# wangkenpu/rsrgan

Hardware: AMD Instinct MI355X
Metric: GAN train frames/sec (G+D step), 257-dim LPS->40-dim MFCC (higher is better)
Workload: dtype f32

## Files before the change

include/rsrgan.h:

```cpp
#ifndef RSRGAN_H_
#define RSRGAN_H_

#include <stddef.h>
#include <stdint.h>

#ifdef __cplusplus
extern "C" {
#endif

typedef enum rsrgan_status {
  RSRGAN_OK = 0,
  RSRGAN_ERR_INVALID = -1,
  RSRGAN_ERR_HIP = -2,
  RSRGAN_ERR_NO_DEVICE = -3,
  RSRGAN_ERR_STATE = -4
} rsrgan_status;

enum { RSRGAN_G_LSTM = 0, RSRGAN_G_RES_LSTM_L = 1, RSRGAN_G_RES_LSTM_BASE = 2,
       RSRGAN_G_DNN = 3,
       RSRGAN_G_RCED = 4,
       RSRGAN_G_BNLSTM = 5 ,
       RSRGAN_G_RES_LSTM_I = 6  };
enum { RSRGAN_D_LSTM = 0, RSRGAN_D_DNN = 1  };
enum { RSRGAN_NET_G = 0, RSRGAN_NET_D = 1 };
// ... 50 lines not shown
};

typedef struct rsrgan_handle_s* rsrgan_handle;

int rsrgan_default_cfg(int32_t g_type, rsrgan_cfg* cfg);

int rsrgan_create(const rsrgan_cfg* cfg, uint64_t seed, rsrgan_handle* out);
int rsrgan_destroy(rsrgan_handle h);
const char* rsrgan_last_error(void);

int rsrgan_set_scalar(rsrgan_handle h, int32_t which, double v);
int rsrgan_get_scalar(rsrgan_handle h, int32_t which, double* v);

int rsrgan_num_tensors(rsrgan_handle h, int32_t net);
int rsrgan_tensor_info(rsrgan_handle h, int32_t net, int32_t idx,
                       char* name, int32_t name_cap,
                       int32_t* rows, int32_t* cols, int64_t* dense_offset);
int64_t rsrgan_param_count(rsrgan_handle h, int32_t net);

int rsrgan_get_params(rsrgan_handle h, int32_t net, int32_t what, float* dense, void* stream);
int rsrgan_set_params(rsrgan_handle h, int32_t net, int32_t what, const float* dense, void* stream);
int rsrgan_get_grads(rsrgan_handle h, int32_t net, float* dense, void* stream);

int rsrgan_forward_g(rsrgan_handle h, const float* x, const int32_t* lengths, int32_t T,
                     float* y, void* stream);

int rsrgan_g_state_floats(rsrgan_handle h, int32_t* n);
int rsrgan_g_state_reset(rsrgan_handle h, const int32_t* row_mask, void* stream);
int rsrgan_g_state_get(rsrgan_handle h, float* dst, void* stream);
int rsrgan_g_state_set(rsrgan_handle h, const float* src, void* stream);
int rsrgan_forward_g_stream(rsrgan_handle h, const float* x, const int32_t* lengths, int32_t T,
                            float* y, void* stream);

int rsrgan_d_step(rsrgan_handle h, const float* x, const float* labels, const int32_t* lengths,
                  int32_t T, const float* noise_real, const float* noise_fake,
                  float* out_losses, int32_t train, void* stream);

int rsrgan_g_step(rsrgan_handle h, const float* x, const float* labels, const int32_t* lengths,
                  int32_t T, const float* noise_fake, float* out_losses,
                  int32_t train, int32_t reuse_g_forward, void* stream);

int rsrgan_d_backward(rsrgan_handle h, const float* x, const float* labels, const int32_t* lengths,
                      int32_t T, const float* noise_real, const float* noise_fake,
                      float* out_losses, void* stream);
int rsrgan_g_backward(rsrgan_handle h, const float* x, const float* labels, const int32_t* lengths,
                      int32_t T, const float* noise_fake, float* out_losses,
                      int32_t reuse_g_forward, void* stream);
int rsrgan_apply(rsrgan_handle h, int32_t net, void* stream);
int rsrgan_grad_buffer(rsrgan_handle h, int32_t net, float** ptr, int64_t* count);
int rsrgan_grad_bucket_count(rsrgan_handle h, int32_t net);
int rsrgan_grad_bucket_info(rsrgan_handle h, int32_t net, int32_t i, int64_t* offset, int64_t* count);
int rsrgan_grad_bucket_wait(rsrgan_handle h, int32_t net, int32_t i, void* stream);

int rsrgan_profile_begin(rsrgan_handle h);
int rsrgan_profile_read(rsrgan_handle h, int32_t* launches, double* total_us, double* alg_flops);
int rsrgan_profile_read_kind(rsrgan_handle h, int32_t kind, int32_t* launches, double* total_us, double* alg_flops);

int rsrgan_device_status(rsrgan_handle h, int32_t* code);

int rsrgan_device_bytes(rsrgan_handle h, int64_t* bytes);

int rsrgan_set_dropout(rsrgan_handle h, float keep_prob, uint64_t seed);

int rsrgan_profile_launches(rsrgan_handle h, int64_t* n);
int rsrgan_op_launch_floor(int32_t n, int32_t mode, double* us_per_launch, void* stream);

int rsrgan_op_gemm(const float* A, int32_t lda, int32_t a_kcontig,
                   const float* B, int32_t ldb, int32_t b_kcontig,
                   float* C, int32_t ldc, int32_t M, int32_t N, int32_t K,
                   const float* bias, int32_t act, float alpha, int32_t accumulate, void* stream);

int rsrgan_op_gemm2(const float* A, int32_t lda, int32_t a_kcontig, const float* A2, int32_t lda2, int32_t M1,
                    const float* B, int32_t ldb, int32_t b_kcontig, float* C, int32_t ldc, int32_t M, int32_t N, int32_t K,
                    const float* bias, int32_t act, float alpha, int32_t accumulate,
                    int32_t map_rows_per, int64_t map_outer, int64_t map_inner, int32_t workers, int32_t force_cfg, void* stream);
#define RSRGAN_OP_NOT_APPLICABLE 1
int rsrgan_op_gemm_batch(int32_t nb, const float* const* A, int32_t lda, const float* const* A2, int32_t lda2, int32_t M1,
                         const float* const* B, int32_t ldb, float* const* C, int32_t ldc, int32_t M, int32_t N, int32_t K,
                         int32_t accumulate, int32_t workers, void* stream);
int rsrgan_op_gemm16_batch(int32_t n, const float* const* A, int32_t lda, const float* const* A2, int32_t lda2, int32_t M1,
                           const float* const* B, int32_t ldb, float* const* C, int32_t ldc, int32_t M, int32_t N, int32_t K,
                           int32_t accumulate, void* stream);
int rsrgan_op_gemm_last_plan(int32_t out[8]);
int rsrgan_op_lstm_colsums(int32_t nb, const float* const* dz, const float* const* cprev, const float* const* ccur, float* const* db,
                           float* const* dwi, float* const* dwf, float* const* dwo, int32_t rows, int32_t H, void* stream);
int rsrgan_op_colsum(const float* a, int32_t lda, const float* b, int32_t ldb, float* out, int32_t rows, int32_t cols, int32_t tall,
                     void* stream);
int rsrgan_op_bnl_fold(const float* Wx, const float* Wh, const float* const bn[12], const float* bias, int32_t P, int32_t H, float* KxT,
                       int32_t ldI, float* KhT, int32_t ldP, float* bias_f, float* ca, float* cb, void* stream);

int rsrgan_op_conv_fwd(const float* in, int32_t ldc_in, int32_t C, const float* F, int32_t ldf, int32_t flip, const float* bias, int32_t relu,
                       const float* mask, float* out, int32_t ldc_out, int32_t N, int32_t R, int32_t S, int32_t W, int32_t fw, void* stream);
int rsrgan_op_conv_wgrad(const float* in, int32_t ldc_in, int32_t C, const float* d, int32_t ldc_d, int32_t N, float* dW, int32_t ldw, float* db,
                         float* ws, int64_t ws_floats, int32_t R_max, int32_t R, int32_t S, int32_t W, int32_t fw, void* stream);
int64_t rsrgan_op_conv_ws_floats(int32_t C, int32_t R_max, int32_t S, int32_t W, int32_t fw);
int rsrgan_op_conv_supported(int32_t C, int32_t N, int32_t S, int32_t W, int32_t fw);
int rsrgan_op_conv_last_plan(int32_t out[40]);

int rsrgan_op_bn_forward(const float* z, int32_t ldz, float* y, int32_t ldy, int32_t rows, int32_t cols, int32_t calls,
                         float* const* vars, float* stat, int32_t ldc, int32_t training, int32_t relu, float* scratch,
                         int64_t scratch_floats, void* stream);
int rsrgan_op_bn_backward(float* dy, int32_t ldd, const float* y, int32_t ldy, const float* z, int32_t ldz, int32_t rows, int32_t cols,
                          int32_t calls, const float* stat, int32_t ldc, float* dbeta, float* dgamma, int32_t accumulate, int32_t relu,
                          float* sums, float* scratch, int64_t scratch_floats, void* stream);
int rsrgan_op_bn_seq_forward(const float* z, int32_t ldz, float* y, int32_t ldy, int32_t rows, int32_t cols, float* const* vars,
                             float* stat, int32_t ldc, int32_t training, int32_t relu, float alpha, int32_t Bp, int32_t Bt,
                             float* scratch, int64_t scratch_floats, void* stream);
int rsrgan_op_bn_seq_backward(float* dy, int32_t ldd, const float* y, int32_t ldy, const float* z, int32_t ldz, int32_t rows,
                              int32_t cols, const float* stat, int32_t ldc, float* dbeta, float* dgamma, int32_t accumulate,
                              int32_t relu, float alpha, int32_t Bp, int32_t Bt, float* sums, float* scratch, int64_t scratch_floats,
                              void* stream);
int rsrgan_op_bn_commit(int32_t n, float* const* vars, const float* const* stat, const int32_t* dims, int32_t single, void* stream);
int rsrgan_op_bn_last_plan(int32_t out[16]);

int rsrgan_feat_batch(const float* raw, int64_t raw_rows, const int32_t* offsets, int32_t B, int32_t T, int32_t D, int32_t left,
                      int32_t right, const double* mean, const double* stddev, float* out, int32_t* lengths, void* stream);
int rsrgan_feat_frames(const float* pool, int64_t pool_rows, const int32_t* picks, int32_t N, int32_t D, int32_t left, int32_t right,
                       const double* mean, const double* stddev, float* out, void* stream);
int rsrgan_feat_stream(const float* fresh, int64_t fresh_rows, const int32_t* table, float* hist, int32_t B, int32_t H, int32_t T, int32_t D,
                       int32_t left, int32_t right, const double* mean, const double* stddev, float* out, int32_t* lengths, void* stream);
int rsrgan_feat_denorm(const float* y, const int32_t* lengths, int32_t B, int32_t T, int32_t D, const double* mean, const double* stddev,
                       double* out, void* stream);
int rsrgan_feat_decode(const uint8_t* blob, int64_t blob_bytes, const int64_t* seg, const float* scale, const int32_t* offsets, int32_t B,
                       int32_t D, const double* mean, const double* stddev, float* out, int64_t out_rows, void* stream);
int rsrgan_feat_wave(const void* pcm, int32_t kind, int64_t n_samples, const int64_t* seg, const int32_t* offsets, int32_t B, int32_t N,
                     int32_t S, int32_t P, float preemph, const float* window, const float* twiddle, float* out, int64_t out_rows,
                     void* stream);
int rsrgan_feat_mfcc(const void* pcm, int32_t kind, int64_t n_samples, const int64_t* seg, const int32_t* offsets, int32_t B, int32_t N,
                     int32_t S, int32_t P, float preemph, const float* window, const float* twiddle, const int32_t* mel_seg,
                     const float* mel_w, int32_t nnz, int32_t M, const float* dct, int32_t C, float* out, int64_t out_rows, void* stream);
int rsrgan_feat_wave_frames(int32_t P);
int rsrgan_wave_reverb(const void* pcm, int32_t kind, int64_t n_samples, const int64_t* seg, const float* rir, int64_t n_taps,
                       const int64_t* rir_seg, const float* noise, int64_t n_noise, const int64_t* noise_seg, const float* noise_pow,
                       const int32_t* sel, const float* snr, int32_t B, int32_t R, int32_t V, int32_t C, const float* twiddle, int32_t flags,
                       float* out, int64_t out_samples, const int64_t* out_seg, float* gains, void* work, int64_t work_bytes, void* stream);
int64_t rsrgan_wave_reverb_work(int32_t B, int64_t n_max, int64_t L_max, int32_t C);

int rsrgan_hist(int32_t n, const float* const* x, const int64_t* dims, double* out, void* stream);
int rsrgan_hist_limits(double* out, int32_t* n);
int rsrgan_d_logits(rsrgan_handle h, float* real, float* fake, int32_t* T, void* stream);
int rsrgan_d_logits_hist(rsrgan_handle h, double* out, void* stream);

int rsrgan_op_segan_sizes(int32_t kind, const int64_t* dims, int64_t out[12]);
int rsrgan_op_segan_conv2(int32_t op, const void* const* ptrs, const int64_t* dims, const float* fl, void* stream);
int rsrgan_op_segan_conv1(int32_t op, const void* const* ptrs, const int64_t* dims, const float* fl, void* stream);
int rsrgan_op_segan_colred(int32_t mode, const void* const* ptrs, const int64_t* dims, const float* fl, void* stream);
int rsrgan_op_segan_last_plan(int32_t out[8]);
int rsrgan_op_segan_vbn(int32_t op, const void* const* ptrs, const int64_t* dims, const float* fl, void* stream);
int rsrgan_op_segan_elem(int32_t op, const void* const* ptrs, const int64_t* dims, const float* fl, void* stream);
int rsrgan_op_segan_dhead(int32_t op, const void* const* ptrs, const int64_t* dims, const float* fl, void* stream);

int rsrgan_op_chunks(const int64_t* tensors, int32_t n_tensors, int32_t* out, int64_t out_ints, int32_t* n_chunks);
int rsrgan_op_update(int32_t op, const void* const* ptrs, const int64_t* dims, const float* fl, void* stream);
int rsrgan_op_step_elem(int32_t op, const void* const* ptrs, const int64_t* dims, const float* fl, void* stream);
int rsrgan_op_layout(int32_t op, const void* const* ptrs, const int64_t* dims, const float* fl, void* stream);

typedef struct rsrgan_segan_cfg {
  int32_t batch_size;
  int32_t input_len;
  int32_t output_dim;
  int32_t n_layers;
  int32_t g_depths[16];
  int32_t d_depths[16];
  int32_t g_kwidth;
  int32_t d_kwidth;
  int32_t g_prelu;
  float   lrelu_alpha;
  float   vbn_eps;
  float   rms_decay;
  float   rms_eps;
} rsrgan_segan_cfg;
typedef struct rsrgan_segan_handle_s* rsrgan_segan_handle;
enum { RSRGAN_SEGAN_G_LR = 0, RSRGAN_SEGAN_D_LR = 1, RSRGAN_SEGAN_L1_LAMBDA = 2 };
int rsrgan_segan_default_cfg(rsrgan_segan_cfg* cfg);
int rsrgan_segan_create(const rsrgan_segan_cfg* cfg, uint64_t seed, rsrgan_segan_handle* out);
int rsrgan_segan_destroy(rsrgan_segan_handle h);
int rsrgan_segan_set_scalar(rsrgan_segan_handle h, int32_t which, double v);
int rsrgan_segan_num_tensors(rsrgan_segan_handle h, int32_t net);
int rsrgan_segan_tensor_info(rsrgan_segan_handle h, int32_t net, int32_t idx, char* name, int32_t name_cap, int32_t* rows, int32_t* cols,
                             int64_t* dense_offset);
int64_t rsrgan_segan_param_count(rsrgan_segan_handle h, int32_t net);
int rsrgan_segan_get_params(rsrgan_segan_handle h, int32_t net, int32_t what, float* dense, void* stream);
int rsrgan_segan_set_params(rsrgan_segan_handle h, int32_t net, int32_t what, const float* dense, void* stream);
int rsrgan_segan_forward_g(rsrgan_segan_handle h, const float* x, const float* z, float* y, void* stream);
int rsrgan_segan_d_backward(rsrgan_segan_handle h, const float* x, const float* labels, const float* z, const float* noise_ref,
                            const float* noise_real, const float* noise_fake, float* out_losses, int32_t train, void* stream);
int rsrgan_segan_g_backward(rsrgan_segan_handle h, const float* x, const float* labels, const float* z, const float* noise_ref,
                            const float* noise_fake, float* out_losses, int32_t train, void* stream);
int rsrgan_segan_grad_buffer(rsrgan_segan_handle h, int32_t net, float** ptr, int64_t* count);
int rsrgan_segan_apply(rsrgan_segan_handle h, int32_t net, void* stream);

int rsrgan_version(void);

#ifdef __cplusplus
}
#endif
#endif
```

rsrgan_amd/_lib.py:

```python
from __future__ import annotations

import ctypes as C
import os

_HERE = os.path.dirname(os.path.abspath(__file__))
LIB_PATH = os.path.join(_HERE, "lib", "librsrgan_hip.so")

G_TYPES = {"lstm": 0, "res_lstm_l": 1, "res_lstm_base": 2, "dnn": 3, "rced": 4, "bnlstm": 5, "res_lstm_i": 6}
FLAG_BATCH_NORM = 32
FLAG_INFER = 64
D_TYPES = {"lstm": 0, "dnn": 1}
NET_G, NET_D = 0, 1
SCALARS = {"g_learning_rate": 0, "d_learning_rate": 1, "mse_lambda": 2, "d_real": 3, "d_fake": 4,
           "l2_scale": 5, "clip_norm": 6, "adam_step": 7, "adam_step_d": 8}
WHAT = {"variables": 0, "adam_m": 1, "adam_v": 2, "ema": 3}

SYMBOLS = ["rsrgan_default_cfg", "rsrgan_create", "rsrgan_destroy", "rsrgan_last_error", "rsrgan_set_scalar",
           "rsrgan_get_scalar", "rsrgan_num_tensors", "rsrgan_tensor_info", "rsrgan_param_count",
           "rsrgan_get_params", "rsrgan_set_params", "rsrgan_get_grads", "rsrgan_forward_g",
           "rsrgan_g_state_floats", "rsrgan_g_state_reset", "rsrgan_g_state_get", "rsrgan_g_state_set", "rsrgan_forward_g_stream",
           "rsrgan_d_step",
           "rsrgan_g_step", "rsrgan_d_backward", "rsrgan_g_backward", "rsrgan_apply", "rsrgan_grad_buffer",
           "rsrgan_grad_bucket_count", "rsrgan_grad_bucket_info", "rsrgan_grad_bucket_wait",
           "rsrgan_profile_begin", "rsrgan_profile_read", "rsrgan_profile_read_kind", "rsrgan_profile_launches", "rsrgan_op_launch_floor", "rsrgan_device_status", "rsrgan_device_bytes", "rsrgan_set_dropout",
           "rsrgan_op_gemm", "rsrgan_op_gemm2", "rsrgan_op_gemm_batch", "rsrgan_op_gemm16_batch", "rsrgan_op_gemm_last_plan",
           "rsrgan_op_lstm_colsums", "rsrgan_op_colsum", "rsrgan_op_bnl_fold", "rsrgan_version",
           "rsrgan_op_conv_fwd", "rsrgan_op_conv_wgrad", "rsrgan_op_conv_ws_floats", "rsrgan_op_conv_supported", "rsrgan_op_conv_last_plan",
           "rsrgan_op_bn_forward", "rsrgan_op_bn_backward", "rsrgan_op_bn_commit", "rsrgan_op_bn_last_plan",
           "rsrgan_op_bn_seq_forward", "rsrgan_op_bn_seq_backward", "rsrgan_feat_batch", "rsrgan_feat_frames",
           "rsrgan_feat_stream", "rsrgan_feat_denorm", "rsrgan_feat_decode", "rsrgan_feat_wave", "rsrgan_feat_mfcc", "rsrgan_feat_wave_frames",
           "rsrgan_wave_reverb", "rsrgan_wave_reverb_work",
           "rsrgan_hist", "rsrgan_hist_limits", "rsrgan_d_logits", "rsrgan_d_logits_hist",
           "rsrgan_op_segan_sizes", "rsrgan_op_segan_conv2", "rsrgan_op_segan_conv1", "rsrgan_op_segan_colred", "rsrgan_op_segan_last_plan",
           "rsrgan_op_segan_vbn", "rsrgan_op_segan_elem", "rsrgan_op_segan_dhead",
           "rsrgan_op_chunks", "rsrgan_op_update", "rsrgan_op_step_elem", "rsrgan_op_layout",
           "rsrgan_segan_default_cfg", "rsrgan_segan_create", "rsrgan_segan_destroy", "rsrgan_segan_set_scalar",
           "rsrgan_segan_num_tensors", "rsrgan_segan_tensor_info", "rsrgan_segan_param_count", "rsrgan_segan_get_params",
           "rsrgan_segan_set_params", "rsrgan_segan_forward_g", "rsrgan_segan_d_backward", "rsrgan_segan_g_backward",
           "rsrgan_segan_grad_buffer", "rsrgan_segan_apply"]


class RsrganCfg(C.Structure):
    _fields_ = [("batch_size", C.c_int32), ("max_frames", C.c_int32), ("input_dim", C.c_int32),
                ("output_dim", C.c_int32), ("g_type", C.c_int32), ("g_layers", C.c_int32), ("g_cells", C.c_int32),
                ("g_proj", C.c_int32), ("d_type", C.c_int32), ("d_layers", C.c_int32), ("d_cells", C.c_int32),
                ("d_proj", C.c_int32), ("l2_scale", C.c_float), ("clip_norm", C.c_float), ("adam_beta1", C.c_float),
                ("adam_beta2", C.c_float), ("adam_eps", C.c_float), ("ema_decay", C.c_float),
                ("lrelu_alpha", C.c_float), ("forget_bias", C.c_float), ("cross_validation", C.c_int32),
                ("flags", C.c_int32), ("d_joint_off", C.c_int32), ("d_joint_dim", C.c_int32), ("g_splice", C.c_int32)]


class SeganCfg(C.Structure):
    _fields_ = [("batch_size", C.c_int32), ("input_len", C.c_int32), ("output_dim", C.c_int32), ("n_layers", C.c_int32),
                ("g_depths", C.c_int32 * 16), ("d_depths", C.c_int32 * 16), ("g_kwidth", C.c_int32), ("d_kwidth", C.c_int32),
                ("g_prelu", C.c_int32), ("lrelu_alpha", C.c_float), ("vbn_eps", C.c_float), ("rms_decay", C.c_float),
                ("rms_eps", C.c_float)]


class RsrganError(RuntimeError):
    pass


_lib = None


def load():
    global _lib
    if _lib is not None:
        return _lib
    if not os.path.exists(LIB_PATH):
        raise ImportError("%s is missing: build it with `python -c 'import __graft_entry__ as g; g.build()'` "
                          "(hipcc --offload-arch=gfx950); rsrgan_amd has no CPU fallback" % LIB_PATH)
    lib = C.CDLL(LIB_PATH)
    p, i32, i64, f32, vp = C.c_void_p, C.c_int32, C.c_int64, C.c_float, C.c_void_p
    lib.rsrgan_last_error.restype = C.c_char_p
    lib.rsrgan_default_cfg.argtypes = [i32, C.POINTER(RsrganCfg)]
    lib.rsrgan_create.argtypes = [C.POINTER(RsrganCfg), C.c_uint64, C.POINTER(vp)]
    lib.rsrgan_destroy.argtypes = [vp]
    lib.rsrgan_set_scalar.argtypes = [vp, i32, C.c_double]
    lib.rsrgan_get_scalar.argtypes = [vp, i32, C.POINTER(C.c_double)]
    lib.rsrgan_num_tensors.argtypes = [vp, i32]
    lib.rsrgan_tensor_info.argtypes = [vp, i32, i32, C.c_char_p, i32, C.POINTER(i32), C.POINTER(i32), C.POINTER(i64)]
    lib.rsrgan_param_count.argtypes = [vp, i32]
    lib.rsrgan_param_count.restype = i64
    lib.rsrgan_get_params.argtypes = [vp, i32, i32, p, vp]
    lib.rsrgan_set_params.argtypes = [vp, i32, i32, p, vp]
    lib.rsrgan_get_grads.argtypes = [vp, i32, p, vp]
    lib.rsrgan_forward_g.argtypes = [vp, p, p, i32, p, vp]
    lib.rsrgan_g_state_floats.argtypes = [vp, C.POINTER(i32)]
    lib.rsrgan_g_state_reset.argtypes = [vp, p, vp]
    lib.rsrgan_g_state_get.argtypes = [vp, p, vp]
    lib.rsrgan_g_state_set.argtypes = [vp, p, vp]
    lib.rsrgan_forward_g_stream.argtypes = [vp, p, p, i32, p, vp]
    lib.rsrgan_d_step.argtypes = [vp, p, p, p, i32, p, p, p, i32, vp]
    lib.rsrgan_g_step.argtypes = [vp, p, p, p, i32, p, p, i32, i32, vp]
    lib.rsrgan_d_backward.argtypes = [vp, p, p, p, i32, p, p, p, vp]
    lib.rsrgan_g_backward.argtypes = [vp, p, p, p, i32, p, p, i32, vp]
    lib.rsrgan_apply.argtypes = [vp, i32, vp]
    lib.rsrgan_grad_buffer.argtypes = [vp, i32, C.POINTER(p), C.POINTER(i64)]
    lib.rsrgan_grad_bucket_count.argtypes = [vp, i32]
    lib.rsrgan_grad_bucket_info.argtypes = [vp, i32, i32, C.POINTER(i64), C.POINTER(i64)]
    lib.rsrgan_grad_bucket_wait.argtypes = [vp, i32, i32, vp]
    lib.rsrgan_profile_begin.argtypes = [vp]
    lib.rsrgan_profile_read.argtypes = [vp, C.POINTER(i32), C.POINTER(C.c_double), C.POINTER(C.c_double)]
    lib.rsrgan_profile_read_kind.argtypes = [vp, i32, C.POINTER(i32), C.POINTER(C.c_double), C.POINTER(C.c_double)]
    lib.rsrgan_device_status.argtypes = [vp, C.POINTER(i32)]
    lib.rsrgan_device_bytes.argtypes = [vp, C.POINTER(i64)]
    lib.rsrgan_set_dropout.argtypes = [vp, f32, C.c_uint64]
    lib.rsrgan_profile_launches.argtypes = [vp, C.POINTER(i64)]
    lib.rsrgan_op_launch_floor.argtypes = [i32, i32, C.POINTER(C.c_double), vp]
    lib.rsrgan_op_gemm.argtypes = [p, i32, i32, p, i32, i32, p, i32, i32, i32, i32, p, i32, f32, i32, vp]
    pp = C.POINTER(C.c_void_p)
    lib.rsrgan_op_gemm2.argtypes = [p, i32, i32, p, i32, i32, p, i32, i32, p, i32, i32, i32, i32, p, i32, f32, i32, i32, i64, i64, i32, i32, vp]
    lib.rsrgan_op_gemm_batch.argtypes = [i32, pp, i32, pp, i32, i32, pp, i32, pp, i32, i32, i32, i32, i32, i32, vp]
    lib.rsrgan_op_gemm16_batch.argtypes = [i32, pp, i32, pp, i32, i32, pp, i32, pp, i32, i32, i32, i32, i32, vp]
    lib.rsrgan_op_gemm_last_plan.argtypes = [C.POINTER(i32)]
    lib.rsrgan_op_lstm_colsums.argtypes = [i32, pp, pp, pp, pp, pp, pp, pp, i32, i32, vp]
    lib.rsrgan_op_colsum.argtypes = [p, i32, p, i32, p, i32, i32, i32, vp]
    lib.rsrgan_op_bnl_fold.argtypes = [p, p, pp, p, i32, i32, p, i32, p, i32, p, p, p, vp]
    lib.rsrgan_op_conv_fwd.argtypes = [p, i32, i32, p, i32, i32, p, i32, p, p, i32, i32, i32, i32, i32, i32, vp]
    lib.rsrgan_op_conv_wgrad.argtypes = [p, i32, i32, p, i32, i32, p, i32, p, p, i64, i32, i32, i32, i32, i32, vp]
    lib.rsrgan_op_conv_ws_floats.argtypes = [i32, i32, i32, i32, i32]
    lib.rsrgan_op_conv_ws_floats.restype = i64
    lib.rsrgan_op_conv_supported.argtypes = [i32, i32, i32, i32, i32]
    lib.rsrgan_op_conv_last_plan.argtypes = [C.POINTER(i32)]
    lib.rsrgan_op_bn_forward.argtypes = [p, i32, p, i32, i32, i32, i32, pp, p, i32, i32, i32, p, i64, vp]
    lib.rsrgan_op_bn_backward.argtypes = [p, i32, p, i32, p, i32, i32, i32, i32, p, i32, p, p, i32, i32, p, p, i64, vp]
    lib.rsrgan_op_bn_seq_forward.argtypes = [p, i32, p, i32, i32, i32, pp, p, i32, i32, i32, f32, i32, i32, p, i64, vp]
    lib.rsrgan_op_bn_seq_backward.argtypes = [p, i32, p, i32, p, i32, i32, i32, p, i32, p, p, i32, i32, f32, i32, i32, p, p, i64, vp]
    lib.rsrgan_feat_batch.argtypes = [p, i64, p, i32, i32, i32, i32, i32, p, p, p, p, vp]
    lib.rsrgan_feat_frames.argtypes = [p, i64, p, i32, i32, i32, i32, p, p, p, vp]
    lib.rsrgan_feat_stream.argtypes = [p, i64, p, p, i32, i32, i32, i32, i32, i32, p, p, p, p, vp]
    lib.rsrgan_feat_denorm.argtypes = [p, p, i32, i32, i32, p, p, p, vp]
    lib.rsrgan_feat_decode.argtypes = [p, i64, p, p, p, i32, i32, p, p, p, i64, vp]
    lib.rsrgan_feat_wave.argtypes = [p, i32, i64, p, p, i32, i32, i32, i32, f32, p, p, p, i64, vp]
    lib.rsrgan_feat_mfcc.argtypes = [p, i32, i64, p, p, i32, i32, i32, i32, f32, p, p, p, p, i32, i32, p, i32, p, i64, vp]
    lib.rsrgan_feat_wave_frames.argtypes = [i32]
    lib.rsrgan_wave_reverb.argtypes = [p, i32, i64, p, p, i64, p, p, i64, p, p, p, p, i32, i32, i32, i32, p, i32, p, i64, p, p, p, i64, vp]
    lib.rsrgan_wave_reverb_work.argtypes = [i32, i64, i64, i32]
    lib.rsrgan_wave_reverb_work.restype = i64
    lib.rsrgan_hist.argtypes = [i32, pp, C.POINTER(i64), p, vp]
    lib.rsrgan_hist_limits.argtypes = [C.POINTER(C.c_double), C.POINTER(i32)]
    lib.rsrgan_d_logits.argtypes = [vp, p, p, C.POINTER(i32), vp]
    lib.rsrgan_d_logits_hist.argtypes = [vp, p, vp]
    lib.rsrgan_op_bn_commit.argtypes =[i32, pp, pp, C.POINTER(i32), i32, vp]
    lib.rsrgan_op_bn_last_plan.argtypes = [C.POINTER(i32)]
    lib.rsrgan_op_segan_sizes.argtypes = [i32, C.POINTER(i64), C.POINTER(i64)]
    for f in (lib.rsrgan_op_segan_conv2, lib.rsrgan_op_segan_conv1, lib.rsrgan_op_segan_colred, lib.rsrgan_op_segan_vbn, lib.rsrgan_op_segan_elem,
              lib.rsrgan_op_segan_dhead, lib.rsrgan_op_update, lib.rsrgan_op_step_elem, lib.rsrgan_op_layout):
        f.argtypes = [i32, C.POINTER(vp), C.POINTER(i64), C.POINTER(C.c_float), vp]
    lib.rsrgan_op_segan_last_plan.argtypes = [C.POINTER(i32)]
    lib.rsrgan_op_chunks.argtypes = [C.POINTER(i64), i32, C.POINTER(i32), i64, C.POINTER(i32)]
    lib.rsrgan_segan_default_cfg.argtypes = [C.POINTER(SeganCfg)]
    lib.rsrgan_segan_create.argtypes = [C.POINTER(SeganCfg), C.c_uint64, C.POINTER(vp)]
    lib.rsrgan_segan_destroy.argtypes = [vp]
    lib.rsrgan_segan_set_scalar.argtypes = [vp, i32, C.c_double]
    lib.rsrgan_segan_num_tensors.argtypes = [vp, i32]
    lib.rsrgan_segan_tensor_info.argtypes = [vp, i32, i32, C.c_char_p, i32, C.POINTER(i32), C.POINTER(i32), C.POINTER(i64)]
    lib.rsrgan_segan_param_count.argtypes = [vp, i32]
    lib.rsrgan_segan_param_count.restype = i64
    lib.rsrgan_segan_get_params.argtypes = [vp, i32, i32, p, vp]
    lib.rsrgan_segan_set_params.argtypes = [vp, i32, i32, p, vp]
    lib.rsrgan_segan_forward_g.argtypes = [vp, p, p, p, vp]
    lib.rsrgan_segan_d_backward.argtypes = [vp, p, p, p, p, p, p, p, i32, vp]
    lib.rsrgan_segan_g_backward.argtypes = [vp, p, p, p, p, p, p, i32, vp]
    lib.rsrgan_segan_grad_buffer.argtypes = [vp, i32, C.POINTER(p), C.POINTER(i64)]
    lib.rsrgan_segan_apply.argtypes = [vp, i32, vp]
    _lib = lib
    return lib


OP_NOT_APPLICABLE = 1
GEMM_CLASSES = {0: "none", 1: "gemm16", 2: "n32", 3: "k_gemm", 4: "k_gemm_s", 5: "gemm16_batch", 6: "k_gemm_batch", 7: "k_gemm_s_batch"}
GEMM_PLAN_FIELDS = ("cls", "bm", "bn", "W", "n_dp", "fixup", "splits", "Ur")
GEMM_FORMS = [("k_gemm", 128, 128), ("k_gemm", 96, 128), ("k_gemm", 128, 96), ("k_gemm", 256, 64), ("k_gemm", 256, 32),
              ("k_gemm_s", 256, 256), ("k_gemm_s", 128, 256), ("k_gemm_s", 256, 128)]
CONV_FAMILIES = {0: "none", 1: "fwd", 2: "fwd4", 3: "wgrad", 4: "wgrad4"}
CONV_FWD_BRANCHES = {1: "whole", 2: "main", 3: "rem"}
CONV_WGRAD_BRANCHES = {1: "k2", 2: "rows", 3: "search"}
CONV_PLAN_FIELDS = ("family", "a0", "a1", "a2", "branch", "TW", "FB", "gx", "gy", "gz", "lds", "DH", "fpg", "groups", "nstrips", "nkg",
                    "PS", "waves", "gmax")
BN_ROUTES = {0: "none", 1: "small", 2: "sliced", 3: "narrow"}
BN_PLAN_FIELDS = ("route", "backward", "calls", "launches", "slices", "per", "pgx", "pgy", "egrid", "q", "R")
SEGAN_OPS = {"conv2": ("conv2_fwd", "conv2_wgrad", "tconv2"), "conv1": ("conv1_fwd", "conv1_wgrad", "tconv1"),
             "colred": ("sum", "dalpha", "moments", "vbn_bwd"), "vbn": ("coef", "apply", "bwd_coef", "bwd_apply"),
             "elem": ("pad_rows", "prep_tconv", "prep_tconv_many", "interleave", "act_fwd", "act_bwd", "copy_cols", "build_joint1", "sum_all",
                      "lsgan", "l1", "rmsprop"),
             "dhead": ("fwd", "bwd")}
UPDATE_OPS = ("sumsq", "dw_reduce", "l2", "apply_sgd", "apply_adam")
STEP_ELEM_OPS = ("lsgan", "dhead", "mse", "g_total", "l2_total", "adam_tick", "dropout_fwd", "dropout_bwd", "lrelu_bwd")
LAYOUT_OPS = ("pack_tm", "unpack_bm", "stage_inputs", "build_d_input", "add_noise_rows", "transpose", "transpose_many", "swizzle_many", "im2col",
              "col2im", "expand_c4", "gstate", "window_len", "zero_many", "fill", "build_joint", "slice_cols", "pad_copy", "copy_f")
DYN_SLOTS = {"g_lr": 0, "d_lr": 1, "lambda": 2, "d_real": 3, "d_fake": 4, "l2": 5, "clip": 6, "beta1": 7, "beta2": 8, "eps": 9, "ema": 10,
             "adam_lrt": 11, "adam_lrt_d": 12}
DYN_COUNT = 16
SEGAN_PLAN_FIELDS = ("vec", "mode", "chunk", "chunks_per", "grid")
BN_VARS = ("beta", "gamma", "moving_mean", "moving_variance", "renorm_mean", "renorm_mean_weight", "renorm_stddev", "renorm_stddev_weight")


def ptr_table(ptrs):
    return (C.c_void_p * max(len(ptrs), 1))(*[None if q is None else q for q in ptrs])


_hist_limits = None


def hist_limits():
    global _hist_limits
    if _hist_limits is None:
        import numpy as np
        lib = load()
        n = C.c_int32()
        check(lib.rsrgan_hist_limits(None, C.byref(n)))
        buf = (C.c_double * n.value)()
        check(lib.rsrgan_hist_limits(buf, C.byref(n)))
        _hist_limits = np.frombuffer(buf, np.float64).copy()
        _hist_limits.setflags(write=False)
    return _hist_limits


def check(rc):
    if rc != 0:
        raise RsrganError("librsrgan_hip error %d: %s" % (rc, load().rsrgan_last_error().decode()))
```

rsrgan_amd/csrc/capi_ops.cpp:

```cpp
#include "capi_common.h"

extern "C" {

int rsrgan_op_launch_floor(int32_t n, int32_t mode, double* us_per_launch, void* stream) {
  if (n <= 0 || !us_per_launch) { set_error("op_launch_floor: bad argument"); return RSRGAN_ERR_INVALID; }
  static float* buf = nullptr;
  if (!buf && hipMalloc((void**)&buf, 2 * 65536 * 4 * sizeof(float)) != hipSuccess) { set_error("hipMalloc failed"); return RSRGAN_ERR_HIP; }
  hipStream_t s = nullptr;
  hipGraph_t g = nullptr; hipGraphExec_t ge = nullptr;
  hipEvent_t e0 = nullptr, e1 = nullptr;
  int rc = RSRGAN_ERR_HIP;
  do {
    if (hipStreamCreateWithFlags(&s, hipStreamNonBlocking) != hipSuccess) break;
    if (hipMemsetAsync(buf, 0, 2 * 65536 * 4 * sizeof(float), s) != hipSuccess) break;
    if (hipStreamBeginCapture(s, hipStreamCaptureModeThreadLocal) != hipSuccess) break;
    launch_floor_chain(buf, buf + 65536 * 4, n, mode, s);
    if (hipStreamEndCapture(s, &g) != hipSuccess) break;
    if (hipGraphInstantiate(&ge, g, nullptr, nullptr, 0) != hipSuccess) break;
    if (hipEventCreate(&e0) != hipSuccess || hipEventCreate(&e1) != hipSuccess) break;
    if (hipGraphLaunch(ge, s) != hipSuccess) break;
    if (hipEventRecord(e0, s) != hipSuccess || hipGraphLaunch(ge, s) != hipSuccess || hipEventRecord(e1, s) != hipSuccess) break;
    if (hipEventSynchronize(e1) != hipSuccess) break;
    float ms = 0.f;
    if (hipEventElapsedTime(&ms, e0, e1) != hipSuccess) break;
// ... 568 lines not shown
      }
      if (op == 1) launch_prep_tconv(FP(0), (int)d[1], (int)d[2], (int)d[3], (int)d[4], (int)d[5], FP(1), (int)d[6], s);
      else {
        PrepTconvBatch pb(s);
        for (int j = 0; j < n; ++j) { const int64_t* q = d + 1 + 6 * j; pb.add(FP(2 * j), (int)q[0], (int)q[1], (int)q[2], (int)q[3], (int)q[4], FP(2 * j + 1), (int)q[5]); }
        pb.flush();
      }
      break;
    }
    case 3: {
      OP_DIM("Q0", d[0], 1); OP_DIM("Q1", d[1], 1); OP_DIM("pl", d[4], 0); OP_DIM("B", d[5], 1); OP_DIM("Lt", d[6], 1); OP_DIM("C", d[7], 1); OP_MUL4("C", d[7]);
      for (int e = 0; e < 2; ++e) {
        const int64_t i0 = (((e - d[4]) % 2) + 2) % 2, cnt = d[6] > i0 ? (d[6] - i0 + 1) / 2 : 0;
        OP_REFUSE(d[2 + e] != i0, WHO ": i0%d = %lld is not the first position of parity class %d under pl = %lld", e, (long long)d[2 + e], e, (long long)d[4]);
        OP_REFUSE(d[e] < cnt, WHO ": Q%d = %lld below the %lld positions of its class", e, (long long)d[e], (long long)cnt);
      }
      OP_REFUSE(d[5] * d[6] * d[7] > ((int64_t)1 << 30), WHO ": B x Lt x C above the entry's 2^30");
      OP_PTR("T0", ptrs[0], 16); OP_PTR("T1", ptrs[1], 16); OP_OPT("bias", ptrs[2], 16); OP_PTR("T", ptrs[3], 16);
      launch_interleave(FP(0), FP(1), (int)d[0], (int)d[1], (int)d[2], (int)d[3], (int)d[4], FP(2), FP(3), (int)d[5], (int)d[6], (int)d[7], s);
      break;
    }
    case 4: {
      OP_DIM("C", d[0], 1); OP_DIM("coff", d[2], 0); OP_DIM("rows", d[3], 1); OP_LD("ldo", d[1], d[2] + d[0]);
      OP_REFUSE(d[3] * d[1] > ((int64_t)1 << 30), WHO ": rows x ldo above the entry's 2^30");
      OP_PTR("z", ptrs[0], 4); OP_OPT("alpha", ptrs[1], 4); OP_PTR("out", ptrs[2], 4);
      launch_act_fwd(FP(0), (int)d[0], FP(1), fl[0], FP(2), (int)d[1], (int)d[2], (size_t)d[3], s);
      break;
    }
    case 5: {
      OP_DIM("C", d[2], 1); OP_DIM("coff", d[1], 0); OP_DIM("rows", d[3], 1); OP_LD("ldy", d[0], d[1] + d[2]);
      OP_REFUSE(d[3] * d[0] > ((int64_t)1 << 30), WHO ": rows x ldy above the entry's 2^30");
      OP_PTR("dy", ptrs[0], 4); OP_PTR("z", ptrs[1], 4); OP_OPT("alpha", ptrs[2], 4); OP_OPT("extra", ptrs[3], 4); OP_PTR("dz", ptrs[4], 4);
      launch_act_bwd(FP(0), (int)d[0], (int)d[1], FP(1), (int)d[2], FP(2), fl[0], FP(3), FP(4), (size_t)d[3], s);
      break;
    }
    case 6: {
      OP_DIM("C", d[4], 1); OP_DIM("rows", d[5], 1); OP_DIM("soff", d[1], 0); OP_DIM("doff", d[3], 0); OP_FLAG("accumulate", d[6]);
      OP_LD("lds", d[0], d[1] + d[4]); OP_LD("ldd", d[2], d[3] + d[4]);
      OP_REFUSE(d[5] * std::max(d[0], d[2]) > ((int64_t)1 << 30), WHO ": rows x ld above the entry's 2^30");
      OP_PTR("src", ptrs[0], 4); OP_PTR("dst", ptrs[1], 4);
      launch_copy_cols(FP(0), (int)d[0], (int)d[1], FP(1), (int)d[2], (int)d[3], (int)d[4], (size_t)d[5], d[6] != 0, s);
      break;
    }
    case 7: {
      OP_DIM("Lx", d[0], 1); OP_DIM("U", d[1], 1); OP_DIM("B", d[2], 1);
      OP_REFUSE(d[2] * (d[0] + d[1]) > ((int64_t)1 << 30), WHO ": B x (Lx + U) above the entry's 2^30");
      OP_PTR("x", ptrs[0], 4); OP_PTR("tail", ptrs[1], 4); OP_OPT("noise", ptrs[2], 4); OP_PTR("joint", ptrs[3], 4);
      launch_build_joint1(FP(0), (int)d[0], FP(1), (int)d[1], FP(2), FP(3), (int)d[2], s);
      break;
    }
    case 8: {
      OP_DIM("rows", d[0], 1); OP_DIM("cols", d[1], 1); OP_LD("ld", d[2], d[1]);
      OP_REFUSE(d[0] * d[2] > ((int64_t)1 << 30), WHO ": rows x ld above the entry's 2^30");
      OP_PTR("src", ptrs[0], 4); OP_PTR("out", ptrs[1], 4); OP_PTR("scratch", ptrs[2], 4);
      launch_sum_all(FP(0), (int)d[0], (int)d[1], (int)d[2], FP(1), FP(2), s);
      break;
    }
    case 9: {
      OP_DIM("B", d[0], 1); OP_DIM("P", d[3], 1);
      OP_REFUSE(d[1] < 0 || d[1] > 1, WHO ": mode = %lld outside 0 (D-run) .. 1 (G-run)", (long long)d[1]);
      OP_REFUSE(d[2] < 0 || d[2] >= d[3], WHO ": fake_pass = %lld outside [0, P = %lld)", (long long)d[2], (long long)d[3]);
      OP_REFUSE(d[0] * d[3] > (1 << 24), WHO ": P x B above the entry's 2^24");
      OP_PTR("logits", ptrs[0], 4); OP_OPT("dlogits", ptrs[1], 4); OP_PTR("loss3", ptrs[2], 4);
      launch_segan_lsgan(FP(0), (int)d[0], (int)d[1], (int)d[2], (int)d[3], FP(1), FP(2), s);
      break;
    }
    case 10: {
      OP_DIM("n", d[0], 1); OP_FLAG("accumulate", d[1]);
      OP_PTR("G", ptrs[0], 4); OP_PTR("labels", ptrs[1], 4); OP_PTR("lambda", ptrs[2], 4); OP_OPT("dG", ptrs[3], 4); OP_PTR("loss3", ptrs[4], 4);
      launch_segan_l1(FP(0), FP(1), (int)d[0], FP(2), FP(3), d[1] != 0, FP(4), s);
      break;
    }
    default: {
      OP_DIM("n", d[0], 1);
      OP_PTR("w", ptrs[0], 4); OP_PTR("g", ptrs[1], 4); OP_PTR("ms", ptrs[2], 4); OP_PTR("lr", ptrs[3], 4);
      launch_rmsprop(FP(0), FP(1), FP(2), FP(3), fl[0], fl[1], (size_t)d[0], s);
      break;
    }
  }
  OP_LAUNCHED(WHO);
}
#undef WHO

#define WHO "op_segan_dhead"
int rsrgan_op_segan_dhead(int32_t op, const void* const* ptrs, const int64_t* dims, const float* fl, void* stream) {
  (void)fl;
  OP_TABLES(0);
  OP_REFUSE(op < 0 || op > 1, WHO ": op = %d outside 0 (dhead_fwd), 1 (dhead_bwd)", op);
  const int64_t* d = dims;
  OP_DIM("R", d[0], 1); OP_DIM("Ld", d[1], 1); OP_DIM("C", d[2], 1); OP_DIM("k", d[3], 1); OP_DIM("ldfc", d[4], 1);
  OP_REFUSE(d[0] * d[1] * d[2] > ((int64_t)1 << 28) || d[3] * d[2] > (1 << 24), WHO ": R x Ld x C above the entry's 2^28");
  if (op == 0) {
    const char* names[6] = {"h", "W", "wfc", "bfc", "conv_out", "logits"};
    for (int i = 0; i < 6; ++i) OP_PTR(names[i], ptrs[i], 4);
    launch_dhead_fwd(FP(0), (int)d[0], (int)d[1], (int)d[2], (int)d[3], FP(1), FP(2), (int)d[4], FP(3), FP(4), FP(5), (hipStream_t)stream);
  } else {
    const char* names[9] = {"dlogit", "h", "conv_out", "W", "wfc", "dW", "dwfc", "dbfc", "dh"};
    for (int i = 0; i < 9; ++i) { if (i >= 5 && i <= 7) OP_OPT(names[i], ptrs[i], 4); else OP_PTR(names[i], ptrs[i], 4); }
    OP_REFUSE((!ptrs[5]) != (!ptrs[6]) || (!ptrs[5]) != (!ptrs[7]), WHO ": dW, dwfc and dbfc must all be given or all be null");
    launch_dhead_bwd(FP(0), (int)d[0], (int)d[1], (int)d[2], (int)d[3], FP(1), FP(2), FP(3), FP(4), (int)d[4], FP(5), FP(6), FP(7), FP(8), (hipStream_t)stream);
  }
  OP_LAUNCHED(WHO);
}
#undef WHO

#define OP_BP(rows_name, rows, Bp, Bt) do { \
    OP_REFUSE((Bp) < 0 || (Bp) > (1 << 20), WHO ": Bp = %lld outside 0 .. 2^20", (long long)(Bp)); \
    if ((Bp) > 0) { \
      OP_REFUSE((Bt) < 1 || (Bt) > (Bp), WHO ": Bt = %lld outside 1 .. Bp = %lld", (long long)(Bt), (long long)(Bp)); \
      OP_REFUSE((rows) % (Bp), WHO ": %s = %lld is not divisible by Bp = %lld", rows_name, (long long)(rows), (long long)(Bp)); \
    } } while (0)
static const int64_t g_up_max_tensors = 4096;

static int up_tensors_ok(const char* who, const int64_t* tensors, int64_t n, int64_t buf_floats) {
  OP_REFUSE(!tensors, "%s: null pointer (tensors)", who);
  OP_REFUSE(n < 1 || n > g_up_max_tensors, "%s: n_tensors = %lld outside 1 .. %lld", who, (long long)n, (long long)g_up_max_tensors);
  for (int64_t i = 0; i < n; ++i) {
    const int64_t off = tensors[3 * i], fl = tensors[3 * i + 1], l2 = tensors[3 * i + 2];
    OP_REFUSE(off < 0 || (off & 3), "%s: offset %lld of tensor %lld is negative or not a multiple of 4", who, (long long)off, (long long)i);
    OP_REFUSE(fl < 1 || (fl & 3), "%s: length %lld of tensor %lld is below 1 or not a multiple of 4", who, (long long)fl, (long long)i);
    OP_REFUSE(off > ((int64_t)1 << 30) || fl > ((int64_t)1 << 30), "%s: tensor %lld reaches beyond 2^30 floats", who, (long long)i);
    OP_REFUSE(l2 < 0 || l2 > 1, "%s: l2 flag %lld of tensor %lld is neither 0 nor 1", who, (long long)l2, (long long)i);
    OP_REFUSE(buf_floats >= 0 && off + fl > buf_floats, "%s: tensor %lld ends at %lld, beyond the buffer's %lld floats", who, (long long)i,
              (long long)(off + fl), (long long)buf_floats);
  }
  return RSRGAN_OK;
}
static void up_table(const int64_t* tensors, int n, ChunkTableHost& h) {
  std::vector<int64_t> off(n), fl(n);
  std::vector<int> l2(n);
  for (int i = 0; i < n; ++i) { off[i] = tensors[3 * i]; fl[i] = tensors[3 * i + 1]; l2[i] = (int)tensors[3 * i + 2]; }
  chunk_table_host(off.data(), fl.data(), l2.data(), n, h);
}

#define WHO "op_chunks"
int rsrgan_op_chunks(const int64_t* tensors, int32_t n_tensors, int32_t* out, int64_t out_ints, int32_t* n_chunks) {
  return guard(WHO, [&]() -> int {
    OP_REFUSE(!n_chunks, WHO ": null pointer (n_chunks)");
    if (int rc = up_tensors_ok(WHO, tensors, n_tensors, -1)) return rc;
    ChunkTableHost h;
    up_table(tensors, n_tensors, h);
    *n_chunks = (int32_t)h.tensor.size();
    if (!out) return RSRGAN_OK;
    const int64_t need = 3 * (int64_t)h.tensor.size() + 3 * (int64_t)n_tensors;
    OP_REFUSE(out_ints < need, WHO ": out of %lld ints below the table's %lld", (long long)out_ints, (long long)need);
    for (const std::vector<int>* v : {&h.tensor, &h.off, &h.len, &h.t_first, &h.t_count, &h.t_l2})
      for (int x : *v) *out++ = x;
    return RSRGAN_OK;
  });
}
#undef WHO

#define WHO "op_update"
int rsrgan_op_update(int32_t op, const void* const* ptrs, const int64_t* dims, const float* fl, void* stream) {
  (void)fl;
  return guard(WHO, [&]() -> int {
    OP_TABLES(0);
    OP_REFUSE(op < 0 || op > 4, WHO ": op = %d outside 0 (sumsq), 1 (dw_reduce), 2 (l2), 3 (apply_sgd), 4 (apply_adam)", op);
    const int64_t* d = dims;
    const int64_t nt = d[0], buf_floats = d[1], partial_floats = d[2];
    OP_DIM("buf_floats", buf_floats, 4);
    if (int rc = up_tensors_ok(WHO, d + 6, nt, buf_floats)) return rc;
    ChunkTableHost h;
    up_table(d + 6, (int)nt, h);
    const int nc = (int)h.tensor.size();
    OP_REFUSE(partial_floats < nc, WHO ": partial of %lld floats below the table's %d chunks", (long long)partial_floats, nc);
    static const char* const names[5][7] = {{"g", "partial"}, {"ws", "g", "partial"}, {"w", "g", "l2_scale", "partial"},
                                            {"w", "g", "ema", "partial", "dyn"}, {"w", "g", "m", "v", "ema", "partial", "dyn"}};
    static const int align[5][7] = {{16, 4}, {16, 16, 4}, {16, 16, 4, 4}, {16, 16, -16, 4, 4}, {16, 16, 16, 16, -16, 4, 4}};
    static const int np[5] = {2, 3, 4, 5, 7};
    for (int i = 0; i < np[op]; ++i) {
      if (align[op][i] < 0) OP_OPT(names[op][i], ptrs[i], -align[op][i]); else OP_PTR(names[op][i], ptrs[i], align[op][i]);
    }
    std::vector<long long> src;
    if (op == 1) {
      const int64_t stride = d[3], ntiles = d[4], ws_floats = d[5];
      OP_DIM("stride", stride, 4); OP_MUL4("stride", stride); OP_DIM("ws_floats", ws_floats, 4);
      OP_REFUSE(ntiles < 1 || ntiles > 64, WHO ": ntiles = %lld outside 1 .. 64", (long long)ntiles);
      for (int64_t i = 0; i < nt; ++i) {
        const int64_t so = d[6 + 3 * nt + i], n = d[6 + 3 * i + 1];
        OP_REFUSE(so < -1 || (so >= 0 && (so & 3)), WHO ": src %lld of tensor %lld is neither -1 nor a non-negative multiple of 4", (long long)so, (long long)i);
        OP_REFUSE(so >= 0 && so + n > stride, WHO ": tensor %lld at src %lld does not fit a record of stride %lld", (long long)i, (long long)so, (long long)stride);
        OP_REFUSE(so >= 0 && (ntiles - 1) * stride + so + n > ws_floats, WHO ": ws of %lld floats below tensor %lld's last record", (long long)ws_floats, (long long)i);
        src.push_back(so);
      }
    }
    if (op == 4) OP_REFUSE(d[3] != DYN_ADAM_LRT && d[3] != DYN_ADAM_LRT_D, WHO ": lrt_slot = %lld is neither %d (G) nor %d (D)", (long long)d[3], (int)DYN_ADAM_LRT, (int)DYN_ADAM_LRT_D);
    hipStream_t s = (hipStream_t)stream;
    std::vector<int> host;
    for (const std::vector<int>* v : {&h.tensor, &h.off, &h.len, &h.t_first, &h.t_count, &h.t_l2}) host.insert(host.end(), v->begin(), v->end());
    int* dev = nullptr;
    long long* dsrc = nullptr;
    HIPC(hipMalloc((void**)&dev, host.size() * sizeof(int)));
    struct Free { int*& a; long long*& b; ~Free() { if (a) (void)hipFree(a); if (b) (void)hipFree(b); } } fr{dev, dsrc};
    HIPC(hipMemcpy(dev, host.data(), host.size() * sizeof(int), hipMemcpyHostToDevice));
    if (op == 1) {
      HIPC(hipMalloc((void**)&dsrc, src.size() * sizeof(long long)));
      HIPC(hipMemcpy(dsrc, src.data(), src.size() * sizeof(long long), hipMemcpyHostToDevice));
    }
    ChunkTable ct{};
    ct.tensor = dev; ct.off = dev + nc; ct.len = dev + 2 * nc;
    ct.t_first = dev + 3 * nc; ct.t_count = dev + 3 * nc + nt; ct.t_l2 = dev + 3 * nc + 2 * nt;
    ct.n_chunks = nc; ct.n_tensors = (int)nt;
    switch (op) {
      case 0: launch_sumsq(FP(0), ct, FP(1), s); break;
      case 1: launch_dw_reduce(FP(0), (size_t)d[3], (int)d[4], dsrc, FP(1), ct, FP(2), s); break;
      case 2: launch_l2(FP(0), FP(1), ct, FP(2), FP(3), s); break;
      case 3: launch_apply_sgd(FP(0), FP(1), FP(2), ct, FP(3), FP(4), s); break;
      default: launch_apply_adam(FP(0), FP(1), FP(2), FP(3), FP(4), ct, FP(5), FP(6), s, (int)d[3]); break;
    }
    OP_LAUNCH_OK(WHO);
    HIPC(hipStreamSynchronize(s));
    return RSRGAN_OK;
  });
}
#undef WHO

#define WHO "op_step_elem"
int rsrgan_op_step_elem(int32_t op, const void* const* ptrs, const int64_t* dims, const float* fl, void* stream) {
  OP_REFUSE(!ptrs, WHO ": null table (ptrs)");
  OP_REFUSE(op < 0 || op > 8, WHO ": op = %d outside 0 .. 8", op);
  OP_REFUSE(op != 3 && !dims, WHO ": null table (dims)");
  OP_REFUSE((op == 0 || op >= 5) && !fl, WHO ": null table (fl: the clip bounds, the betas, keep or alpha)");
  const int64_t* d = dims;
  hipStream_t s = (hipStream_t)stream;
  switch (op) {
    case 0: {
      OP_DIM("T", d[0], 1); OP_DIM("Nd", d[1], 1); OP_LD("ldl", d[3], 1); OP_FLAG("clip_on", d[4]);
      OP_REFUSE(d[2] < 0 || d[2] > d[1], WHO ": n_real = %lld outside 0 .. Nd = %lld", (long long)d[2], (long long)d[1]);
      OP_REFUSE(d[0] * d[1] > (1 << 24), WHO ": T x Nd above the entry's 2^24");
      OP_BP("Nd", d[1], d[5], d[6]); OP_BP("n_real", d[2], d[5], d[6]);
      OP_PTR("logits", ptrs[0], 4); OP_OPT("dlogits", ptrs[1], 4); OP_PTR("t_real", ptrs[2], 4); OP_PTR("t_fake", ptrs[3], 4); OP_PTR("loss3", ptrs[4], 4);
      launch_lsgan(FP(0), (int)d[3], FP(1), (int)d[0], (int)d[1], (int)d[2], FP(2), FP(3), FP(4), s, d[4] != 0, fl[0], fl[1], (int)d[5], (int)d[6]);
      break;
    }
    case 1: {
      OP_DIM("T", d[0], 1); OP_DIM("Nd", d[1], 1); OP_DIM("dR", d[3], 1); OP_MUL4("dR", d[3]);
      OP_REFUSE(d[3] + 3 > 64, WHO ": dR = %lld above 60 (k_dhead2 sums 3 + dR <= 64 quantities)", (long long)d[3]);
      OP_REFUSE(d[2] < 0 || d[2] > d[1], WHO ": n_real = %lld outside 0 .. Nd = %lld", (long long)d[2], (long long)d[1]);
      OP_REFUSE(d[0] * d[1] > (1 << 24), WHO ": T x Nd above the entry's 2^24");
      OP_FLAG("want_grads", d[8]); OP_FLAG("want_wgrads", d[9]);
      OP_LD("ldt", d[4], d[3]); OP_MUL4("ldt", d[4]); OP_LD("ldw", d[5], 1); OP_LD("ldl", d[6], 1);
      if (d[8]) { OP_LD("ldo", d[7], d[3]); OP_MUL4("ldo", d[7]); }
      OP_BP("Nd", d[1], d[10], d[11]); OP_BP("n_real", d[2], d[10], d[11]);
      static const char* const names[12] = {"top", "w", "b", "logits", "dlogits", "dout", "gw", "gb", "t_real", "t_fake", "loss3", "part"};
      for (int i = 0; i < 12; ++i) {
        const bool wanted = i < 4 || i > 7 || (i < 6 ? d[8] != 0 : d[9] != 0);
        const int align = (i == 0 || i == 5) ? 16 : 4;
        if (wanted) OP_PTR(names[i], ptrs[i], align); else OP_OPT(names[i], ptrs[i], align);
      }
      const int64_t need = (d[0] * d[1] + 63) / 64 * (DH_MAXR + 3);
      OP_REFUSE(d[12] < need, WHO ": part of %lld floats below ceil(T x Nd / 64) x %d = %lld", (long long)d[12], DH_MAXR + 3, (long long)need);
      DHeadArgs a{};
      a.top = FP(0); a.ldt = (int)d[4]; a.w = FP(1); a.ldw = (int)d[5]; a.b = FP(2);
      a.logits = FP(3); a.ldl = (int)d[6]; a.dlogits = FP(4); a.dout = FP(5); a.ldo = (int)d[7]; a.gw = FP(6); a.gb = FP(7);
      a.T = (int)d[0]; a.Nd = (int)d[1]; a.n_real = (int)d[2]; a.dR = (int)d[3]; a.t_real = FP(8); a.t_fake = FP(9); a.loss3 = FP(10); a.part = FP(11);
      a.want_grads = (int)d[8]; a.want_wgrads = (int)d[9]; a.Bp = (int)d[10]; a.Bt = (int)d[11];
      launch_dhead(a, s);
      break;
    }
    case 2: {
      OP_DIM("rows", d[0], 1); OP_DIM("D", d[1], 1); OP_LD("ld", d[2], d[1]); OP_FLAG("accumulate", d[3]);
      OP_REFUSE(d[0] * d[2] > ((int64_t)1 << 30), WHO ": rows x ld above the entry's 2^30");
      OP_BP("rows", d[0], d[4], d[5]);
      OP_REFUSE(d[6] < 1024, WHO ": scratch of %lld floats below launch_mse's 1024", (long long)d[6]);
      OP_PTR("y", ptrs[0], 4); OP_PTR("lab", ptrs[1], 4); OP_OPT("dy", ptrs[2], 4); OP_PTR("lambda", ptrs[3], 4); OP_PTR("loss", ptrs[4], 4); OP_PTR("scratch", ptrs[5], 4);
      launch_mse(FP(0), FP(1), (int)d[2], FP(2), (int)d[0], (int)d[1], FP(3), d[3] != 0, FP(4), FP(5), s, (int)d[4], (int)d[5]);
      break;
    }
    case 3:
      OP_PTR("l4", ptrs[0], 4); OP_PTR("lambda", ptrs[1], 4);
      launch_g_total(FP(0), FP(1), s);
      break;
    case 4:
      OP_DIM("n", d[0], 1);
      OP_PTR("partial", ptrs[0], 4); OP_PTR("l2_scale", ptrs[1], 4); OP_PTR("out", ptrs[2], 4);
      launch_l2_total(FP(0), (int)d[0], FP(1), FP(2), s);
      break;
    case 5: {
      const bool g = d[0] == DYN_G_LR && d[1] == DYN_ADAM_LRT, dd = d[0] == DYN_D_LR && d[1] == DYN_ADAM_LRT_D;
      OP_REFUSE(!g && !dd, WHO ": slots (%lld, %lld) are neither (%d, %d) (G) nor (%d, %d) (D)", (long long)d[0], (long long)d[1], (int)DYN_G_LR,
                (int)DYN_ADAM_LRT, (int)DYN_D_LR, (int)DYN_ADAM_LRT_D);
      OP_REFUSE(!(fl[0] >= 0.f && fl[0] < 1.f) || !(fl[1] >= 0.f && fl[1] < 1.f), WHO ": beta1 = %g or beta2 = %g outside [0, 1)", (double)fl[0], (double)fl[1]);
      OP_PTR("dyn", ptrs[0], 4); OP_PTR("t", ptrs[1], 4);
      launch_adam_tick(FP(0), (int*)ptrs[1], (double)fl[0], (double)fl[1], s, (int)d[0], (int)d[1]);
      break;
    }
    case 6: case 7: case 8: {
      OP_DIM("rows", d[0], 1); OP_DIM("cols", d[1], 1); OP_LD("ld", d[2], d[1]);
      OP_REFUSE(d[0] * d[2] > ((int64_t)1 << 30), WHO ": rows x ld above the entry's 2^30");
      if (op != 8) OP_REFUSE(!(fl[0] > 0.f && fl[0] <= 1.f), WHO ": keep = %g outside (0, 1]", (double)fl[0]);
      if (op == 6) OP_REFUSE(d[4] < 0 || d[4] > (1 << 24), WHO ": thr = %lld outside 0 .. 2^24", (long long)d[4]);
      OP_PTR(op == 8 ? "h" : "y", ptrs[0], 4);
      if (op != 6) OP_PTR("d", ptrs[1], 4);
      if (op == 6) launch_dropout_fwd(FP(0), (size_t)d[0], (int)d[1], (int)d[2], (unsigned long long)d[3], (unsigned)d[4], fl[0], s);
      else if (op == 7) launch_dropout_bwd(FP(0), FP(1), (size_t)d[0], (int)d[1], (int)d[2], fl[0], s);
      else launch_lrelu_bwd(FP(0), FP(1), (size_t)d[0], (int)d[1], (int)d[2], fl[0], s);
      break;
    }
  }
  OP_LAUNCHED(WHO);
}
#undef WHO

#define OP_JOB_NAME(buf, name, j) char buf[48]; snprintf(buf, sizeof(buf), "%s of job %d", name, (int)(j))
#define WHO "op_layout"
int rsrgan_op_layout(int32_t op, const void* const* ptrs, const int64_t* dims, const float* fl, void* stream) {
  OP_REFUSE(!ptrs || !dims, WHO ": null table (ptrs or dims)");
  OP_REFUSE(op < 0 || op > 18, WHO ": op = %d outside 0 .. 18", op);
  OP_REFUSE(op == 14 && !fl, WHO ": null table (fl: the fill value)");
  const int64_t* d = dims;
  const int64_t lim = (int64_t)1 << 30;
  hipStream_t s = (hipStream_t)stream;
  switch (op) {
    case 0: case 1: {
      OP_DIM("B", d[0], 1); OP_DIM("T", d[1], 1); OP_DIM("D", d[2], 1); OP_LD("ld", d[3], d[2]);
      OP_REFUSE(d[0] * d[1] * d[3] > lim || d[0] > 65535, WHO ": B x T x ld above the entry's 2^30, or B above the grid's 65535");
      if (op == 1) OP_REFUSE(d[4] < 0 || d[4] > d[0], WHO ": Bt = %lld outside 0 (all rows) .. B = %lld", (long long)d[4], (long long)d[0]);
      OP_PTR("src", ptrs[0], 4); OP_PTR("dst", ptrs[1], 4);
      if (op == 0) launch_pack_tm(FP(0), FP(1), (int)d[0], (int)d[1], (int)d[2], (int)d[3], s);
      else launch_unpack_bm(FP(0), (int)d[3], FP(1), (int)d[0], (int)d[1], (int)d[2], s, (int)d[4]);
      break;
    }
    case 2: {
      OP_DIM("B", d[0], 1); OP_DIM("T", d[1], 1);
      OP_REFUSE(d[0] > 65535, WHO ": B = %lld above the grid's 65535", (long long)d[0]);
      OP_REFUSE(d[2] < 0 || d[2] > d[0], WHO ": Bt = %lld outside 0 (all rows) .. B = %lld", (long long)d[2], (long long)d[0]);
      StageJobs j{};
      j.B = (int)d[0]; j.T = (int)d[1]; j.Bt = (int)d[2];
      for (int k = 0; k < 2; ++k) {
        if (!ptrs[2 * k]) continue;
        OP_JOB_NAME(ns, "src", k); OP_JOB_NAME(nd, "dst", k); OP_JOB_NAME(nD, "D", k); OP_JOB_NAME(nl, "ld", k);
        OP_PTR(ns, ptrs[2 * k], 4); OP_PTR(nd, ptrs[2 * k + 1], 4);
        OP_DIM(nD, d[3 + 2 * k], 1); OP_LD(nl, d[4 + 2 * k], d[3 + 2 * k]);
        OP_REFUSE(d[0] * d[1] * d[4 + 2 * k] > lim, WHO ": B x T x ld of pack %d above the entry's 2^30", k);
        j.pack[k] = StagePack{FP(2 * k), FP(2 * k + 1), (int)d[3 + 2 * k], (int)d[4 + 2 * k]};
      }
      for (int k = 0; k < 4; ++k) {
        if (!ptrs[4 + 2 * k]) continue;
        OP_JOB_NAME(ns, "copy src", k); OP_JOB_NAME(nd, "copy dst", k); OP_JOB_NAME(nn, "n", k);
        OP_PTR(ns, ptrs[4 + 2 * k], 4); OP_PTR(nd, ptrs[5 + 2 * k], 4); OP_DIM(nn, d[7 + k], 1);
        j.copy[k] = StageCopy{ptrs[4 + 2 * k], (void*)ptrs[5 + 2 * k], (int)d[7 + k]};
      }
      launch_stage_inputs(j, s);
      break;
    }
    case 3: {
      OP_DIM("B", d[0], 1); OP_DIM("T", d[1], 1); OP_DIM("D", d[2], 1); OP_LD("ld", d[3], d[2]); OP_FLAG("with_real", d[4]);
      OP_REFUSE(2 * d[0] * d[1] * d[3] > lim, WHO ": 2 B x T x ld above the entry's 2^30");
      if (d[4]) OP_PTR("lab", ptrs[0], 4); else OP_OPT("lab", ptrs[0], 4);
      OP_PTR("y", ptrs[1], 4); OP_OPT("nr", ptrs[2], 4); OP_OPT("nf", ptrs[3], 4); OP_PTR("xd", ptrs[4], 4);
      launch_build_d_input(FP(0), FP(1), FP(2), FP(3), FP(4), (int)d[0], (int)d[1], (int)d[2], (int)d[3], d[4] != 0, s);
      break;
    }
    case 4: {
      OP_DIM("B", d[0], 1); OP_DIM("T", d[1], 1); OP_DIM("D", d[2], 1); OP_LD("ld", d[3], d[2]); OP_DIM("Ns", d[4], 1); OP_DIM("row0", d[5], 0);
      OP_REFUSE(d[5] + d[0] > d[4], WHO ": rows [row0 = %lld, row0 + B = %lld) outside Ns = %lld", (long long)d[5], (long long)(d[5] + d[0]), (long long)d[4]);
      OP_REFUSE(d[4] * d[1] * d[3] > lim, WHO ": Ns x T x ld above the entry's 2^30");
      OP_PTR("src", ptrs[0], 4); OP_OPT("noise", ptrs[1], 4); OP_PTR("dst", ptrs[2], 4);
      launch_add_noise_rows(FP(0), FP(1), FP(2), (int)d[0], (int)d[1], (int)d[2], (int)d[3], (int)d[4], (int)d[5], s);
      break;
    }
    case 5: {
      OP_DIM("R", d[2], 1); OP_DIM("C", d[3], 1); OP_LD("lds", d[0], d[3]); OP_LD("ldd", d[1], d[2]);
      OP_REFUSE(d[2] * d[0] > lim || d[3] * d[1] > lim || d[2] > (65535 << 5), WHO ": R x lds or C x ldd above the entry's 2^30, or R above the grid's 65535 tiles");
      OP_PTR("src", ptrs[0], 4); OP_PTR("dst", ptrs[1], 4);
// ... 159 lines not shown
```

rsrgan_amd/csrc/kernels.h:

```cpp
#pragma once
#include <hip/hip_runtime.h>
#include <stdint.h>

#include <vector>

#include "switches.h"

namespace rsr {

constexpr int MAXJ = 8;

struct Place { int x0, nx, sb, se, nb, w; };
constexpr int JOBMAP_MAX = 768;
struct JobMap { int valid; unsigned char job[JOBMAP_MAX]; };
struct PlanItem { int ncol, nrow; double cost; int mult; };
int plan_places(int n, const PlanItem* items, Place* out);

enum { DYN_G_LR = 0, DYN_D_LR = 1, DYN_LAMBDA = 2, DYN_D_REAL = 3, DYN_D_FAKE = 4, DYN_L2 = 5, DYN_CLIP = 6,
       DYN_B1 = 7, DYN_B2 = 8, DYN_EPS = 9, DYN_EMA = 10, DYN_ADAM_LRT = 11, DYN_ADAM_LRT_D = 12, DYN_COUNT = 16 };

struct FwdGateJob {
  const float* x;
  const float* KxT;
  const float* m;
// ... 211 lines not shown
                         hipStream_t s, float* ws, size_t ws_floats);
void launch_gemm2(const float* A, int lda, const float* A2, int lda2, int M1, bool a_kc, const float* B, int ldb, bool b_kc,
                  float* C, int ldc, int M, int N, int K, const float* bias, int act, float alpha, bool accumulate,
                  hipStream_t s, float* ws, size_t ws_floats);
constexpr int GEMM_MAXB = 4;
bool launch_gemm_batch(int nb, const float* const* A, int lda, const float* const* A2, int lda2, int M1, const float* const* B, int ldb,
                       float* const* C, int ldc, int M, int N, int K, bool accumulate, hipStream_t s, float* ws, size_t ws_floats);
void launch_gemm(const float* A, int lda, bool a_kc, const float* B, int ldb, bool b_kc,
                 float* C, int ldc, int M, int N, int K,
                 const float* bias, int act, float alpha, bool accumulate, hipStream_t s,
                 float* splitk_ws = nullptr, size_t splitk_ws_floats = 0);

struct StagePack { const float* src; float* dst; int D, ld; };
struct StageCopy { const void* src; void* dst; int n; };
struct StageJobs { StagePack pack[2]; StageCopy copy[4]; int B, T; int Bt; };
void launch_stage_inputs(const StageJobs& j, hipStream_t s);
void launch_pack_tm(const float* src_bm, float* dst_tm, int B, int T, int D, int ld, hipStream_t s);
void launch_unpack_bm(const float* src_tm, int ld, float* dst_bm, int B, int T, int D, hipStream_t s, int Bt = 0);
void launch_build_d_input(const float* lab_tm, const float* y_tm, const float* noise_r, const float* noise_f,
                          float* xd, int B, int T, int D, int ld, bool with_real, hipStream_t s);
void launch_add_noise_rows(const float* src_tm, const float* noise, float* dst, int B, int T, int D, int ld,
                           int Ns, int row0, hipStream_t s);
void launch_transpose(const float* src, int lds, float* dst, int ldd, int R, int C, hipStream_t s);
void launch_fill(float* p, size_t n, float v, hipStream_t s);
struct SwizzleJob { const float* src; float* dst; int ld, gates, H, C, c0, K1, I, P, kx, nct, nkb, blk_base; };
struct SwizzleList { int n; SwizzleJob j[24]; };
void launch_swizzle_many(SwizzleList& sl, hipStream_t s);
inline size_t swizzle_floats(int nct, int nkb) { return (size_t)nct * nkb * 256; }
struct TransposeJob { const float* src; float* dst; int lds, ldd, R, C, blk_base; };
struct TransposeList { int n; TransposeJob j[16]; };
void launch_transpose_many(TransposeList& tl, hipStream_t s);
size_t conv_prep_floats(int S, int fw, int C);
void launch_conv_prep(const float* F, int ldf_src, int S, int fw, int Cin, int Cout, bool flip, float* Ft, hipStream_t s);
bool conv_fwd_supported(int C, int N, int S, int W, int fw);
void launch_conv_fwd(const float* in, int ldc_in, int C, const float* Ft, const float* bias, bool relu, float* out, int ldc_out, int N,
                     int R, int S, int W, int fw, hipStream_t s,
                     const float* mask = nullptr );
bool conv_wgrad_supported(int C, int N, int S, int W, int fw);
size_t conv_wgrad_ws_floats(int C, int R, int S, int W, int fw);
void launch_conv_wgrad(const float* in, int ldc_in, int C, const float* d, int ldc_d, int N, float* dW, int ldw, float* ws, int R, int S,
                       int W, int fw, hipStream_t s,
                       float* db = nullptr );
enum { CONV_FAM_NONE = 0, CONV_FAM_FWD = 1 , CONV_FAM_FWD4 = 2 ,
       CONV_FAM_WGRAD = 3 , CONV_FAM_WGRAD4 = 4  };
enum { CONV_BR_WHOLE = 1, CONV_BR_MAIN = 2, CONV_BR_REM = 3, CONV_BR_WG_K2 = 1, CONV_BR_WG_ROWS = 2, CONV_BR_WG_SEARCH = 3 };
struct ConvLaunchRecord {
  int family, a0, a1, a2;
  int branch, TW, FB, gx, gy, gz, lds;
  int DH, fpg, groups, nstrips, nkg, PS, waves, gmax;
};
struct ConvPlanRecord { int n; ConvLaunchRecord l[2]; };
extern thread_local ConvPlanRecord g_conv_last_plan;
void launch_im2col(const float* src, size_t row_stride, int ldc, int C, int S, int W, int kh, int kw, float* col, int ldk, size_t M,
                   hipStream_t s);
void launch_expand_c4(const float* src, int ld_src, int n, float* dst, size_t rows, hipStream_t s);
void launch_col2im(const float* dcol, int ldk, int C, int S, int W, int kh, int kw, float* dst, int ldc, size_t M, hipStream_t s);
struct GStateLayer { float *c, *mst; int H, P, ldP, off; };
struct GStateArgs { GStateLayer L[GP_MAXL]; int nl, SF, rows, dir; float* state; size_t slot; const int* mask; };
void launch_gstate(const GStateArgs& a, hipStream_t s);
void launch_window_len(const int* len, int* dst, int n, int t0, int Tw, hipStream_t s);
struct ZeroList { int n; float* p[32]; unsigned len[32]; };
void launch_zero_many(const ZeroList& zl, hipStream_t s);
struct ColsumsBatch { const float* dz[4]; const float* cprev[4]; const float* ccur[4]; float* db[4]; float* dwi[4]; float* dwf[4]; float* dwo[4]; int n; };
void launch_lstm_colsums_batch(const ColsumsBatch& bt, int rows, int H, float* scratch, hipStream_t s);
void launch_lstm_colsums(const float* dz, const float* cprev, const float* ccur, float* db, float* dwi, float* dwf, float* dwo,
                         int rows, int H, float* scratch , hipStream_t s);
void launch_lrelu_bwd(const float* hval, float* d, size_t rows, int cols, int ld, float alpha, hipStream_t s);
void launch_dropout_fwd(float* y, size_t rows, int cols, int ld, unsigned long long key, unsigned thr, float keep, hipStream_t s);
void launch_dropout_bwd(const float* y, float* d, size_t rows, int cols, int ld, float keep, hipStream_t s);
void launch_colsum_tall(const float* a, int lda, float* out, int rows, int cols, float* scratch, size_t scratch_floats, hipStream_t s);

struct BnVars {
  float *beta, *gamma;
  float *mm, *mv, *rm, *rmw, *rs, *rsw;
};
constexpr int BN_STAT_ROWS = 6;
void launch_bn_forward(const float* z, int ldz, float* y, int ldy, int rows, int cols, const BnVars& v, float* stat, int ldc, bool training,
                       bool relu, float* scratch, size_t scratch_floats, hipStream_t s, int calls = 1);
void launch_bn_backward(float* dy, int ldd, const float* y, int ldy, const float* z, int ldz, int rows, int cols, const float* stat, int ldc,
                        float* dbeta, float* dgamma, bool accumulate, bool relu, float* sums, float* scratch, size_t scratch_floats,
                        hipStream_t s, int calls = 1);
void launch_bn_commit(int cols, const BnVars& v, const float* stat, int ldc, int times, hipStream_t s);
struct BnCommit { BnVars v; const float* stat; int cols, ldc, times0, times1; };
struct BnCommitList { int n; BnCommit e[24]; };
void launch_bn_commit_many(const BnCommitList& cl, hipStream_t s);
enum { BN_ROUTE_NONE = 0, BN_ROUTE_SMALL = 1, BN_ROUTE_SLICED = 2, BN_ROUTE_NARROW = 3 };
struct BnPlanRecord { int route, backward, calls, launches, slices, per, pgx, pgy, egrid, q, R; };
extern thread_local BnPlanRecord g_bn_last_plan;
int bn_seq_count(int rows, int Bp, int Bt);
void launch_bn_seq_forward(const float* z, int ldz, float* y, int ldy, int rows, int cols, const BnVars& v, float* stat, int ldc, bool training,
                           bool act, float alpha, int Bp, int Bt, float* scratch, size_t scratch_floats, hipStream_t s);
void launch_bn_seq_backward(float* dy, int ldd, const float* y, int ldy, const float* z, int ldz, int rows, int cols, const float* stat, int ldc,
                            float* dbeta, float* dgamma, bool accumulate, bool act, float alpha, int Bp, int Bt, float* sums, float* scratch,
                            size_t scratch_floats, hipStream_t s);
void launch_bn_seq_fold(float* W, int ldw, int K, int cols, const BnVars& v, float* bias, hipStream_t s);
void launch_feat_batch(const float* raw, long long raw_rows, const int* offsets, int B, int T, int D, int left, int right, const double* mean,
                       const double* stddev, float* out, int* lengths, hipStream_t s);
void launch_feat_frames(const float* pool, long long pool_rows, const int* picks, int N, int D, int left, int right, const double* mean,
                        const double* stddev, float* out, hipStream_t s);
void launch_feat_stream(const float* fresh, long long fresh_rows, const int* table, float* hist, int B, int H, int T, int D, int left, int right,
                        const double* mean, const double* stddev, float* out, int* lengths, hipStream_t s);
void launch_feat_denorm(const float* y, const int* lengths, int B, int T, int D, const double* mean, const double* stddev, double* out,
                        hipStream_t s);
void launch_feat_decode(const uint8_t* blob, long long blob_bytes, const long long* seg, const float* scale, const int* offsets, int B, int D,
                        const double* mean, const double* stddev, float* out, long long out_rows, hipStream_t s);
int wave_frames(int P);
void launch_feat_wave(const void* pcm, int kind, long long n_samples, const long long* seg, const int* offsets, int B, int N, int S, int P,
                      float preemph, const float* window, const float* twiddle, float* out, long long out_rows, hipStream_t s);
size_t mfcc_lds_bytes(int N, int S, int P, int M, int C, int nnz);
void launch_feat_mfcc(const void* pcm, int kind, long long n_samples, const long long* seg, const int* offsets, int B, int N, int S, int P,
                      float preemph, const float* window, const float* twiddle, const int* mel_seg, const float* mel_w, int nnz, int M,
                      const float* dct, int C, float* out, long long out_rows, hipStream_t s);
struct RevArgs {
  const void* pcm; int kind; long long n_samples; const long long* seg;
  const float* rir; long long n_taps; const long long* rir_seg;
  const float* noise; long long n_noise; const long long* noise_seg; const float* noise_pow;
  const int* sel; const float* snr; int B, R, V; uint32_t C; const float* twiddle; int flags;
  float* out; long long out_samples; const long long* out_seg; float* gains;
  unsigned char* work; unsigned long long slot;
};
size_t reverb_work_bytes(int B, long long n_max, long long L_max, int C);
void launch_wave_reverb(const RevArgs& a, size_t work_bytes, hipStream_t s);
constexpr int HIST_MAX_TENSORS = 16;
constexpr int hist_nl() {
  int k = 0;
  for (double v = 1e-12; v < 1e20; v *= 1.1) ++k;
  return 2 * (k + 1) + 1;
}
constexpr int HIST_NL = hist_nl();
constexpr int HIST_REC = 5 + HIST_NL;
struct HistView { const float* x; long long ld, cs; unsigned rows, cols; int clip; };
const std::vector<double>& hist_limits();
bool launch_hist(int n, const HistView* views, float clip_lo, float clip_hi, double* out, hipStream_t s);
void launch_logits_dense(const float* logits, int frame_rows, int B, int T, float* out, bool clip, float clip_lo, float clip_hi, hipStream_t s);
void launch_colsum(const float* a, int lda, const float* b, int ldb, float* out, int rows, int cols,
                   float* scratch , hipStream_t s);

constexpr int DH_MAXR = 64;
struct DHeadArgs {
  const float* top; int ldt; const float* w; int ldw; const float* b;
  float* logits; int ldl; float* dlogits; float* dout; int ldo; float* gw; float* gb;
  int T, Nd, n_real, dR; const float* t_real; const float* t_fake; float* loss3; float* part; int want_grads, want_wgrads;
  int Bp, Bt;
};
void launch_dhead(const DHeadArgs& a, hipStream_t s);
void launch_lsgan(const float* logits, int ldl, float* dlogits, int T, int Nd, int n_real,
                  const float* target_real, const float* target_fake, float* loss3, hipStream_t s,
                  bool clip_on = false, float clip_lo = 0.f, float clip_hi = 0.f, int Bp = 0, int Bt = 0);
void launch_build_joint(const float* x, int ldx, int off, int dim, const float* tail, int ldt, int Dt, float* joint, int ldj,
                        int row0, int R, hipStream_t s);
void launch_slice_cols(const float* src, int lds, int off, float* dst, int ldd, int R, int C, hipStream_t s);
void launch_mse(const float* y, const float* lab, int ld, float* dy, int rows, int D, const float* lambda,
                bool accumulate, float* loss_out, float* scratch , hipStream_t s, int Bp = 0, int Bt = 0);
void launch_g_total(float* l4 , const float* lambda, hipStream_t s);
void launch_copy_f(const float* src, float* dst, int n, hipStream_t s);

struct ChunkTable {
  const int* tensor;
  const int* off;
  const int* len;
  const int* t_first;
  const int* t_count;
  const int* t_l2;
  int n_chunks, n_tensors;
};
void launch_sumsq(const float* g, const ChunkTable& ct, float* partial, hipStream_t s);
void launch_dw_reduce(const float* ws, size_t stride, int ntiles, const long long* src, float* g, const ChunkTable& ct, float* partial, hipStream_t s);
void launch_l2(const float* w, float* g, const ChunkTable& ct, const float* l2_scale, float* partial, hipStream_t s);
void launch_l2_total(const float* partial, int n_chunks, const float* l2_scale, float* out, hipStream_t s);
void launch_apply_sgd(float* w, const float* g, float* ema, const ChunkTable& ct, const float* partial,
                      const float* dyn, hipStream_t s);
void launch_apply_adam(float* w, const float* g, float* m, float* v, float* ema, const ChunkTable& ct,
                       const float* partial, const float* dyn, hipStream_t s, int lrt_slot = DYN_ADAM_LRT);
void launch_adam_tick(float* dyn, int* t, double b1, double b2, hipStream_t s, int lr_slot = DYN_G_LR, int lrt_slot = DYN_ADAM_LRT);
void launch_pad_copy(const float* dense, float* padded, int rows, int cols, int ld, bool to_padded, hipStream_t s);

}
```

rsrgan_amd/csrc/kernels.hip:

```cpp
#include <algorithm>
#include <cstdlib>

#include "kernels.h"

namespace rsr {

typedef float f32x4 __attribute__((ext_vector_type(4)));

__device__ __forceinline__ float sigmoid_(float x) { return 1.0f / (1.0f + expf(-x)); }

#ifdef RSR_TRACE
__device__ unsigned long long g_trace[8192 * 16];
#define TR_BEGIN() do { if (threadIdx.x == 0 && blockIdx.x < 8192) { unsigned long long* t_ = g_trace + (size_t)blockIdx.x * 16; \
    t_[0] = __builtin_amdgcn_s_memrealtime(); t_[1] = __builtin_amdgcn_s_memtime(); \
    t_[14] = __builtin_amdgcn_s_getreg(4 | (0 << 6) | (31 << 11)); t_[15] = __builtin_amdgcn_s_getreg(20 | (0 << 6) | (3 << 11)); \
    for (int i_ = 2; i_ < 14; ++i_) t_[i_] = 0; } } while (0)
#define TR_ID(ptr) do { if (threadIdx.x == 0 && blockIdx.x < 8192) g_trace[(size_t)blockIdx.x * 16 + 12] = (unsigned long long)(size_t)(ptr); } while (0)
#define TR(i) do { if (threadIdx.x == 0 && blockIdx.x < 8192) g_trace[(size_t)blockIdx.x * 16 + (i)] = __builtin_amdgcn_s_memtime(); } while (0)
#define TR_END() do { if (threadIdx.x == 0 && blockIdx.x < 8192) { g_trace[(size_t)blockIdx.x * 16 + 9] = __builtin_amdgcn_s_memtime(); \
    g_trace[(size_t)blockIdx.x * 16 + 13] = __builtin_amdgcn_s_memrealtime(); } } while (0)
#else
#define TR_BEGIN() do { } while (0)
#define TR_ID(ptr) do { } while (0)
#define TR(i) do { } while (0)
// ... 1496 lines not shown
    const float lr_ = n_real > 0 ? sr / cr : 0.f;
    const float lf_ = (Nd - n_real) > 0 ? sf / cf : 0.f;
    loss3[0] = lr_; loss3[1] = lf_; loss3[2] = lr_ + lf_;
  }
}
void launch_lsgan(const float* logits, int ldl, float* dlogits, int T, int Nd, int n_real,
                  const float* t_real, const float* t_fake, float* loss3, hipStream_t s, bool clip_on, float clip_lo, float clip_hi,
                  int Bp, int Bt) {
  hipLaunchKernelGGL(k_lsgan, dim3(1), dim3(1024), 0, s, logits, ldl, dlogits, T, Nd, n_real, t_real, t_fake, loss3,
                     clip_on ? 1 : 0, clip_lo, clip_hi, Bp, Bt);
}

__global__ __launch_bounds__(64) void k_dhead1(const DHeadArgs a) {
  __shared__ float wsh[DH_MAXR + 1];
  const int lane = threadIdx.x;
  const int rows = a.T * a.Nd, dR = a.dR;
  if (lane < dR) wsh[lane] = a.w[(size_t)lane * a.ldw];
  if (lane == 0) wsh[DH_MAXR] = a.b[0];
  __syncthreads();
  const int r = blockIdx.x * 64 + lane;
  const bool on = r < rows;
  const float tr = *a.t_real, tf = *a.t_fake;
  const int nr_ = a.Bp > 0 ? a.n_real / a.Bp * a.Bt : a.n_real, nf_ = a.Bp > 0 ? (a.Nd - a.n_real) / a.Bp * a.Bt : a.Nd - a.n_real;
  const float cr = (float)a.T * (float)nr_, cf = (float)a.T * (float)nf_;
  float x[DH_MAXR];
  float logit = wsh[DH_MAXR];
  const float* xr = a.top + (size_t)(on ? r : 0) * a.ldt;
#pragma unroll
  for (int c = 0; c < DH_MAXR; c += 4) {
    float4 v = make_float4(0.f, 0.f, 0.f, 0.f);
    if (c < dR) v = *reinterpret_cast<const float4*>(xr + c);
    x[c] = v.x; x[c + 1] = v.y; x[c + 2] = v.z; x[c + 3] = v.w;
  }
#pragma unroll
  for (int c = 0; c < DH_MAXR; ++c) if (c < dR) logit += x[c] * wsh[c];
  const bool real = on && (r % a.Nd) < a.n_real;
  const bool valid = a.Bp <= 0 || ((r % a.Nd) % a.Bp) < a.Bt;
  const float d = valid ? logit - (real ? tr : tf) : 0.f;
  float sr = (on && real) ? d * d : 0.f, sf = (on && !real) ? d * d : 0.f;
  const float dl = on ? 2.f * d / (real ? cr : cf) : 0.f;
  if (on) {
    a.logits[(size_t)r * a.ldl] = logit;
    if (a.want_grads) {
      a.dlogits[(size_t)r * a.ldl] = dl;
      float* o = a.dout + (size_t)r * a.ldo;
#pragma unroll
      for (int c = 0; c < DH_MAXR; c += 4)
        if (c < dR) *reinterpret_cast<float4*>(o + c) = make_float4(dl * wsh[c], dl * wsh[c + 1], dl * wsh[c + 2], dl * wsh[c + 3]);
    }
  }
  auto wsum = [&](float v) { for (int o = 32; o > 0; o >>= 1) v += __shfl_down(v, o, 64); return v; };
  float* part = a.part + (size_t)blockIdx.x * (DH_MAXR + 3);
  sr = wsum(sr); sf = wsum(sf);
  if (lane == 0) { part[0] = sr; part[1] = sf; }
  if (a.want_wgrads) {
    const float sd = wsum(dl);
    if (lane == 0) part[2] = sd;
#pragma unroll
    for (int c = 0; c < DH_MAXR; ++c)
      if (c < dR) { const float v = wsum(x[c] * dl); if (lane == 0) part[3 + c] = v; }
  }
}
__global__ __launch_bounds__(1024) void k_dhead2(const DHeadArgs a, int nblocks) {
  __shared__ float tot[DH_MAXR + 3];
  const int q = threadIdx.x >> 4, j = threadIdx.x & 15;
  const int nq = a.want_wgrads ? 3 + a.dR : 2;
  float s = 0.f;
  if (q < nq)
    for (int b = j; b < nblocks; b += 16) s += a.part[(size_t)b * (DH_MAXR + 3) + q];
  s += __shfl_xor(s, 8); s += __shfl_xor(s, 4); s += __shfl_xor(s, 2); s += __shfl_xor(s, 1);
  if (q < nq && j == 0) {
    tot[q] = s;
    if (a.want_wgrads) {
      if (q == 2) a.gb[0] = s;
      if (q >= 3) a.gw[(size_t)(q - 3) * a.ldw] = s;
    }
  }
  __syncthreads();
  if (threadIdx.x == 0) {
    const int nr_ = a.Bp > 0 ? a.n_real / a.Bp * a.Bt : a.n_real, nf_ = a.Bp > 0 ? (a.Nd - a.n_real) / a.Bp * a.Bt : a.Nd - a.n_real;
    const float cr = (float)a.T * (float)nr_, cf = (float)a.T * (float)nf_;
    const float lr_ = a.n_real > 0 ? tot[0] / cr : 0.f;
    const float lf_ = (a.Nd - a.n_real) > 0 ? tot[1] / cf : 0.f;
    a.loss3[0] = lr_; a.loss3[1] = lf_; a.loss3[2] = lr_ + lf_;
  }
}
void launch_dhead(const DHeadArgs& a, hipStream_t s) {
  const int rows = a.T * a.Nd, nb = (rows + 63) / 64;
  hipLaunchKernelGGL(k_dhead1, dim3(nb), dim3(64), 0, s, a);
  hipLaunchKernelGGL(k_dhead2, dim3(1), dim3(1024), 0, s, a, nb);
}

__global__ void k_build_joint(const float* __restrict__ x, int ldx, int off, int dim, const float* __restrict__ tail, int ldt, int Dt,
                              float* __restrict__ joint, int ldj, int row0, int R) {
  const int W = dim + Dt;
  const size_t total = (size_t)R * W;
  for (size_t i = (size_t)blockIdx.x * blockDim.x + threadIdx.x; i < total; i += (size_t)gridDim.x * blockDim.x) {
    const int r = (int)(i / W), c = (int)(i % W);
    joint[(size_t)(row0 + r) * ldj + c] = c < dim ? x[(size_t)r * ldx + off + c] : tail[(size_t)r * ldt + (c - dim)];
  }
}
void launch_build_joint(const float* x, int ldx, int off, int dim, const float* tail, int ldt, int Dt, float* joint, int ldj,
                        int row0, int R, hipStream_t s) {
  const size_t total = (size_t)R * (dim + Dt);
  const int blocks = (int)min((size_t)2048, (total + 255) / 256);
  hipLaunchKernelGGL(k_build_joint, dim3(blocks), dim3(256), 0, s, x, ldx, off, dim, tail, ldt, Dt, joint, ldj, row0, R);
}
__global__ void k_slice_cols(const float* __restrict__ src, int lds_, int off, float* __restrict__ dst, int ldd, int R, int C) {
  const size_t total = (size_t)R * C;
  for (size_t i = (size_t)blockIdx.x * blockDim.x + threadIdx.x; i < total; i += (size_t)gridDim.x * blockDim.x) {
    const int r = (int)(i / C), c = (int)(i % C);
    dst[(size_t)r * ldd + c] = src[(size_t)r * lds_ + off + c];
  }
}
void launch_slice_cols(const float* src, int lds_, int off, float* dst, int ldd, int R, int C, hipStream_t s) {
  const size_t total = (size_t)R * C;
  const int blocks = (int)min((size_t)2048, (total + 255) / 256);
  hipLaunchKernelGGL(k_slice_cols, dim3(blocks), dim3(256), 0, s, src, lds_, off, dst, ldd, R, C);
}

constexpr int MSE_BLOCKS = 256;
__global__ __launch_bounds__(256) void k_mse1(const float* __restrict__ y, const float* __restrict__ lab, int ld,
                                              float* __restrict__ dy, int rows, int D, const float* __restrict__ lambda,
                                              int accumulate, float* __restrict__ scratch, int Bp, int Bt) {
  __shared__ float red[16];
  const size_t total = (size_t)rows * D;
  const int rows_eff = Bp > 0 ? rows / Bp * Bt : rows;
  const float scale = dy ? (*lambda) / (float)rows_eff : 0.f;
  float s = 0.f;
  for (size_t i = (size_t)blockIdx.x * blockDim.x + threadIdx.x; i < total; i += (size_t)gridDim.x * blockDim.x) {
    const size_t r = i / D; const int c = (int)(i % D);
    const size_t o = r * ld + c;
    const bool valid = Bp <= 0 || (int)(r % Bp) < Bt;
    const float d = valid ? y[o] - lab[o] : 0.f;
    s += d * d;
    if (dy) dy[o] = (accumulate ? dy[o] : 0.f) + scale * d;
  }
  s = block_sum_1024(s, red);
  if (threadIdx.x == 0) scratch[blockIdx.x] = s;
}
__global__ void k_mse2(const float* __restrict__ scratch, int rows, float* __restrict__ out) {
  if (threadIdx.x == 0) {
    float s = 0.f;
    for (int i = 0; i < MSE_BLOCKS; ++i) s += scratch[i];
    *out = 0.5f * s / (float)rows;
  }
}
void launch_mse(const float* y, const float* lab, int ld, float* dy, int rows, int D, const float* lambda,
                bool accumulate, float* loss_out, float* scratch, hipStream_t s, int Bp, int Bt) {
  hipLaunchKernelGGL(k_mse1, dim3(MSE_BLOCKS), dim3(256), 0, s, y, lab, ld, dy, rows, D, lambda, accumulate ? 1 : 0, scratch, Bp, Bt);
  hipLaunchKernelGGL(k_mse2, dim3(1), dim3(64), 0, s, scratch, Bp > 0 ? rows / Bp * Bt : rows, loss_out);
}

__global__ void k_g_total(float* l4, const float* lambda) {
  if (threadIdx.x == 0) l4[3] = l4[0] + (*lambda) * l4[1] + l4[2];
}
void launch_g_total(float* l4, const float* lambda, hipStream_t s) {
  hipLaunchKernelGGL(k_g_total, dim3(1), dim3(64), 0, s, l4, lambda);
}
__global__ void k_copy_f(const float* src, float* dst, int n) {
  const int i = blockIdx.x * blockDim.x + threadIdx.x;
  if (i < n) dst[i] = src[i];
}
void launch_copy_f(const float* src, float* dst, int n, hipStream_t s) {
  hipLaunchKernelGGL(k_copy_f, dim3((n + 255) / 256), dim3(256), 0, s, src, dst, n);
}


__global__ __launch_bounds__(256) void k_sumsq(const float* __restrict__ g, ChunkTable ct, float* __restrict__ partial) {
  __shared__ float red[16];
  const int c = blockIdx.x;
  const float* p = g + ct.off[c];
  const int n = ct.len[c];
  float s = 0.f;
  for (int i = threadIdx.x * 4; i < n; i += 1024) {
    const float4 v = *reinterpret_cast<const float4*>(p + i);
    s += (v.x * v.x + v.y * v.y) + (v.z * v.z + v.w * v.w);
  }
  s = block_sum_1024(s, red);
  if (threadIdx.x == 0) partial[c] = s;
}
void launch_sumsq(const float* g, const ChunkTable& ct, float* partial, hipStream_t s) {
  hipLaunchKernelGGL(k_sumsq, dim3(ct.n_chunks), dim3(256), 0, s, g, ct, partial);
}

__global__ __launch_bounds__(256) void k_dw_reduce(const float* __restrict__ ws, size_t stride, int ntiles, const long long* __restrict__ src,
                                                   float* __restrict__ g, ChunkTable ct, float* __restrict__ partial) {
  __shared__ float red[16];
  const int c = blockIdx.x;
  const int t = ct.tensor[c];
  const int off = ct.off[c], n = ct.len[c];
  const long long so = src[t];
  float s = 0.f;
  if (so < 0) {
    for (int i = threadIdx.x * 4; i < n; i += 1024) {
      const float4 v = *reinterpret_cast<const float4*>(g + off + i);
      s += (v.x * v.x + v.y * v.y) + (v.z * v.z + v.w * v.w);
    }
  } else {
    const float* p = ws + so + (off - ct.off[ct.t_first[t]]);
    for (int i = threadIdx.x * 4; i < n; i += 1024) {
      float4 a = *reinterpret_cast<const float4*>(p + i);
      for (int r = 1; r < ntiles; ++r) {
        const float4 b = *reinterpret_cast<const float4*>(p + (size_t)r * stride + i);
        a.x += b.x; a.y += b.y; a.z += b.z; a.w += b.w;
      }
      *reinterpret_cast<float4*>(g + off + i) = a;
      s += (a.x * a.x + a.y * a.y) + (a.z * a.z + a.w * a.w);
    }
  }
  s = block_sum_1024(s, red);
  if (threadIdx.x == 0) partial[c] = s;
}
void launch_dw_reduce(const float* ws, size_t stride, int ntiles, const long long* src, float* g, const ChunkTable& ct, float* partial, hipStream_t s) {
  hipLaunchKernelGGL(k_dw_reduce, dim3(ct.n_chunks), dim3(256), 0, s, ws, stride, ntiles, src, g, ct, partial);
}

__global__ __launch_bounds__(256) void k_l2(const float* __restrict__ w, float* __restrict__ g, ChunkTable ct,
                                            const float* __restrict__ l2_scale, float* __restrict__ partial) {
  __shared__ float red[16];
  const int c = blockIdx.x;
  const bool on = ct.t_l2[ct.tensor[c]] != 0;
  const int off = ct.off[c], n = ct.len[c];
  const float sc = *l2_scale;
  float s = 0.f;
  if (on) {
    for (int i = threadIdx.x; i < n; i += 256) {
      const float v = w[off + i];
      s += v * v;
      g[off + i] += sc * v;
    }
  }
  s = block_sum_1024(s, red);
  if (threadIdx.x == 0) partial[c] = s;
}
void launch_l2(const float* w, float* g, const ChunkTable& ct, const float* l2_scale, float* partial, hipStream_t s) {
  hipLaunchKernelGGL(k_l2, dim3(ct.n_chunks), dim3(256), 0, s, w, g, ct, l2_scale, partial);
}
__global__ __launch_bounds__(1024) void k_l2_total(const float* __restrict__ partial, int n, const float* __restrict__ l2_scale, float* out) {
  __shared__ float red[16];
  float s = 0.f;
  for (int i = threadIdx.x; i < n; i += blockDim.x) s += partial[i];
  s = block_sum_1024(s, red);
  if (threadIdx.x == 0) *out = 0.5f * (*l2_scale) * s;
}
void launch_l2_total(const float* partial, int n, const float* l2_scale, float* out, hipStream_t s) {
  hipLaunchKernelGGL(k_l2_total, dim3(1), dim3(1024), 0, s, partial, n, l2_scale, out);
}

__device__ __forceinline__ float tensor_clip_scale(const ChunkTable& ct, const float* partial, int c, float clip, float* red) {
  const int t = ct.tensor[c];
  const int first = ct.t_first[t], cnt = ct.t_count[t];
  float s = 0.f;
  for (int i = threadIdx.x; i < cnt; i += blockDim.x) s += partial[first + i];
  s = block_sum_1024(s, red);
  if (!(clip > 0.f)) return 1.0f;
  const float inv = s > 0.f ? 1.0f / sqrtf(s) : __builtin_inff();
  return clip * fminf(inv, 1.0f / clip);
}

__global__ __launch_bounds__(256) void k_apply_sgd(float* __restrict__ w, const float* __restrict__ g, float* __restrict__ ema,
                                                   ChunkTable ct, const float* __restrict__ partial, const float* __restrict__ dyn) {
  __shared__ float red[16];
  const int c = blockIdx.x;
  const float scale = tensor_clip_scale(ct, partial, c, dyn[DYN_CLIP], red);
  const float lr = dyn[DYN_D_LR], dec = dyn[DYN_EMA];
  const int off = ct.off[c], n = ct.len[c];
  for (int i = threadIdx.x; i < n; i += 256) {
    const float nw = w[off + i] - lr * (g[off + i] * scale);
    w[off + i] = nw;
    if (ema) ema[off + i] = dec * ema[off + i] + (1.f - dec) * nw;
  }
}
void launch_apply_sgd(float* w, const float* g, float* ema, const ChunkTable& ct, const float* partial, const float* dyn, hipStream_t s) {
  hipLaunchKernelGGL(k_apply_sgd, dim3(ct.n_chunks), dim3(256), 0, s, w, g, ema, ct, partial, dyn);
}

__global__ __launch_bounds__(256) void k_apply_adam(float* __restrict__ w, const float* __restrict__ g, float* __restrict__ m,
                                                    float* __restrict__ v, float* __restrict__ ema, ChunkTable ct,
                                                    const float* __restrict__ partial, const float* __restrict__ dyn, int lrt_slot) {
  __shared__ float red[16];
  const int c = blockIdx.x;
  const float scale = tensor_clip_scale(ct, partial, c, dyn[DYN_CLIP], red);
  const float b1 = dyn[DYN_B1], b2 = dyn[DYN_B2], eps = dyn[DYN_EPS], lrt = dyn[lrt_slot], dec = dyn[DYN_EMA];
  const int off = ct.off[c], n = ct.len[c];
  for (int i = threadIdx.x; i < n; i += 256) {
    const float gg = g[off + i] * scale;
    const float mm = b1 * m[off + i] + (1.f - b1) * gg;
    const float vv = b2 * v[off + i] + (1.f - b2) * gg * gg;
    m[off + i] = mm; v[off + i] = vv;
    const float nw = w[off + i] - lrt * mm / (sqrtf(vv) + eps);
    w[off + i] = nw;
    if (ema) ema[off + i] = dec * ema[off + i] + (1.f - dec) * nw;
  }
}
void launch_apply_adam(float* w, const float* g, float* m, float* v, float* ema, const ChunkTable& ct,
                       const float* partial, const float* dyn, hipStream_t s, int lrt_slot) {
  hipLaunchKernelGGL(k_apply_adam, dim3(ct.n_chunks), dim3(256), 0, s, w, g, m, v, ema, ct, partial, dyn, lrt_slot);
}

__global__ void k_adam_tick(float* dyn, int* t, double b1, double b2, int lr_slot, int lrt_slot) {
  if (threadIdx.x == 0) {
    const int tt = *t + 1;
    *t = tt;
    dyn[lrt_slot] = (float)((double)dyn[lr_slot] * sqrt(1.0 - pow(b2, (double)tt)) / (1.0 - pow(b1, (double)tt)));
  }
}
void launch_adam_tick(float* dyn, int* t, double b1, double b2, hipStream_t s, int lr_slot, int lrt_slot) {
  hipLaunchKernelGGL(k_adam_tick, dim3(1), dim3(64), 0, s, dyn, t, b1, b2, lr_slot, lrt_slot);
}

__global__ void k_pad_copy(const float* __restrict__ dense_c, float* __restrict__ dense_m, float* __restrict__ padded,
                           int rows, int cols, int ld, int to_padded) {
  const size_t total = (size_t)rows * cols;
  for (size_t i = (size_t)blockIdx.x * blockDim.x + threadIdx.x; i < total; i += (size_t)gridDim.x * blockDim.x) {
    const size_t r = i / cols; const int c = (int)(i % cols);
    if (to_padded) padded[r * ld + c] = dense_c[i];
    else dense_m[i] = padded[r * ld + c];
  }
}
void launch_pad_copy(const float* dense, float* padded, int rows, int cols, int ld, bool to_padded, hipStream_t s) {
  const size_t total = (size_t)rows * cols;
  const int blocks = (int)min((size_t)1024, (total + 255) / 256);
  hipLaunchKernelGGL(k_pad_copy, dim3(blocks), dim3(256), 0, s, dense, const_cast<float*>(dense), padded, rows, cols, ld, to_padded ? 1 : 0);
}

}
```

rsrgan_amd/csrc/model.cpp:

```cpp
#include "model.h"

#include <cmath>
#include <cstdarg>
#include <cstdio>
#include <cstdlib>
#include <cstring>

namespace rsr {

static thread_local char g_err[512] = "";
void set_error(const char* fmt, ...) {
  va_list ap;
  va_start(ap, fmt);
  vsnprintf(g_err, sizeof(g_err), fmt, ap);
  va_end(ap);
}
const char* get_error() { return g_err; }

void Model::refresh_transposes(int net, hipStream_t s) {
  const ParamSet& ps = net == RSRGAN_NET_G ? G : D;
  auto& layers = net == RSRGAN_NET_G ? gl : dl;
  TransposeList tl{};
  auto add = [&](const float* src, int lds_, float* dst, int ldd, int R, int C) {
    if (tl.n == 16) { launch_transpose_many(tl, s); tl.n = 0; }
    tl.j[tl.n++] = TransposeJob{src, dst, lds_, ldd, R, C, 0};
  };
  if (net == RSRGAN_NET_G && bnl_infer()) { bnl_refresh_fold(s); return; }
  if (net == RSRGAN_NET_G && seq_bn_infer()) seq_bn_fold(s);
  for (auto& L : layers) {
    const float* K = ps.W(L.tK);
    const int H4 = 4 * L.H;
    add(K, H4, L.KxT, L.ldI, L.I, H4);
    add(K + (size_t)L.I * H4, H4, L.KhT, L.ldP, L.P, H4);
    if (L.has_proj) add(ps.W(L.tWp), L.ldP, L.WpT, L.ldH, L.H, L.P);
  }
  if (net == RSRGAN_NET_G && g_fc_out_wT && g_fc_out_w >= 0)
    add(G.W(g_fc_out_w), ldDout, g_fc_out_wT, pad4(gR), gR, Dout);
  launch_transpose_many(tl, s);
  if (!lazy_sw) refresh_swizzles(net, s);
  if (net == RSRGAN_NET_G)
    for (size_t l = 0; l < gconv.size(); ++l) {
      const ConvLayer& L = gconv[l];
      if (rc_ft_fwd[l]) launch_conv_prep(G.W(L.tW), L.ldCout, rcS, L.fw, L.Cin, L.Cout, false, rc_ft_fwd[l], s);
      if (rc_ft_bwd[l]) launch_conv_prep(G.W(L.tW), L.ldCout, rcS, L.fw, L.Cin, L.Cout, true, rc_ft_bwd[l], s);
    }
}

void Model::refresh_swizzles(int net, hipStream_t s) {
  if (net == RSRGAN_NET_G && bnl_infer()) return;
  const ParamSet& ps = net == RSRGAN_NET_G ? G : D;
  auto& layers = net == RSRGAN_NET_G ? gl : dl;
  {
    SwizzleList sl{};
    auto addz = [&](const SwizzleJob& j) {
      if (!j.dst) return;
      if (sl.n == 24) { launch_swizzle_many(sl, s); sl.n = 0; }
      sl.j[sl.n++] = j;
    };
    for (auto& L : layers) {
      const float* K = ps.W(L.tK);
      const int H4 = 4 * L.H, ncb = (L.H + 15) / 16, kbI = (L.ldI + L.ldP + 15) / 16, kbP = (L.ldP + 15) / 16, kbH = (L.ldH + 15) / 16, kb4 = (H4 + 15) / 16;
      addz(SwizzleJob{K, L.Wg_full, H4,    4,    L.H, 0,         0,   0,  L.I, L.P, L.ldI, 4 * ncb,            kbI, 0});
      addz(SwizzleJob{K, L.Wg_h,    H4,    4,    L.H, 0,         0,   0,  L.I, L.P, 0,     4 * ncb,            kbP, 0});
      addz(SwizzleJob{K, L.Kb_full, H4,    0,    0,   L.I + L.P, 0,   H4, 0,   0,   0,     (L.I + L.P + 15) / 16, kb4, 0});
      addz(SwizzleJob{K, L.Kb_rec,  H4,    0,    0,   L.P,       L.I, H4, 0,   0,   0,     (L.P + 15) / 16,    kb4, 0});
      if (L.has_proj) {
        const float* Wp = ps.W(L.tWp);
        addz(SwizzleJob{Wp, L.WpT_sw, L.ldP, 1,  L.P, 0,         0,   0,  L.H, 0,   16 * kbH, (L.P + 15) / 16, kbH, 0});
        addz(SwizzleJob{Wp, L.Wp_sw,  L.ldP, 0,  0,   L.H,       0,   L.P, 0,  0,   0,     ncb,                kbP, 0});
      }
    }
    launch_swizzle_many(sl, s);
  }
}

static inline int kb16(int ld) { return (ld + 15) >> 4; }

bool Model::bwd_b_splitk_ok(const BwdBJobs& jobs) const {
  if (!bwdb_ws || (cfg.flags & RSRGAN_FLAG_NO_SPLITK_B)) return false;
  BwdBJobs tmp = jobs;
  const size_t need = bwd_b_plan(tmp, nullptr);
  if (need > bwdb_ws_floats) return false;
  int blocks = 0;
  for (int i = 0; i < tmp.n; ++i) {
    if ((tmp.j[i].kpg + 1) / 2 > 12) return false;
    blocks += tmp.j[i].KG * tmp.j[i].ncg * tmp.j[i].nrg;
  }
  return blocks >= 96;
}

void Model::gemm(const float* A, int lda, bool a_kc, const float* B_, int ldb, bool b_kc, float* C, int ldc, int M, int N,
                 int K, const float* bias, int act, float alpha, bool accumulate, hipStream_t s) {
  launch_gemm(A, lda, a_kc, B_, ldb, b_kc, C, ldc, M, N, K, bias, act, alpha, accumulate, s,
              (side && s == side) ? gemm_ws2 : gemm_ws, gemm_ws_floats);
}

static void fill_gate(FwdGateJob& a, const LayerRun& R, int t, bool zx) {
  const LstmLayer& L = *R.L; const LstmStash& S = *R.S; const ParamSet& ps = *R.ps;
  const int H = L.H, H4 = 4 * H;
  const size_t r = (size_t)t * R.Ns + R.row0, rn = (size_t)(t + 1) * R.Ns + R.row0;
  a.x = zx ? nullptr : R.in + r * L.ldI;
  a.KxT = L.KxT; a.ldx = L.ldI; a.Wsw = zx ? L.Wg_h : L.Wg_full;
  a.m = S.mst + r * L.ldP; a.KhT = L.KhT; a.ldm = L.ldP;
  a.zx = zx ? S.gates + r * H4 : nullptr; a.bias = ps.W(L.tb);
  a.wf = ps.W(L.twf); a.wi = ps.W(L.twi); a.wo = ps.W(L.two);
  a.c_prev = S.c + r * H; a.c_out = S.c + rn * H;
  a.gates = S.gates + r * H4;
  a.h = S.h + r * L.ldH; a.ldh = L.ldH;
  a.len = R.len; a.t = t; a.N = R.N; a.H = H;
  a.nblk_c = (H + 15) / 16;
  if (L.has_proj) { a.np_m_out = nullptr; a.np_out = nullptr; a.np_res_in = nullptr; a.np_res_out = nullptr; }
  else {
    a.np_m_out = S.mst + rn * L.ldP; a.np_out = S.out ? S.out + r * L.ldP : nullptr;
    a.np_res_in = R.res_in ? R.res_in + r * L.ldP : nullptr;
    a.np_res_out = R.res_out ? R.res_out + r * L.ldP : nullptr;
  }
}
static void fill_proj(FwdProjJob& p, const LayerRun& R, int t) {
  const LstmLayer& L = *R.L; const LstmStash& S = *R.S;
  const size_t r = (size_t)t * R.Ns + R.row0, rn = (size_t)(t + 1) * R.Ns + R.row0;
  p.h = S.h + r * L.ldH; p.WpT = L.WpT; p.WpT_sw = L.WpT_sw; p.ldh = L.ldH;
  p.m_prev = S.mst + r * L.ldP; p.m_out = S.mst + rn * L.ldP; p.out = S.out + r * L.ldP;
  p.res_in = R.res_in ? R.res_in + r * L.ldP : nullptr;
  p.res_out = R.res_out ? R.res_out + r * L.ldP : nullptr;
  p.len = R.len; p.bias = nullptr; p.noise = nullptr;
  p.ldm = L.ldP; p.ldo = L.ldP; p.P = L.P; p.t = t; p.N = R.N;
  p.nblk_c = (L.P + 15) / 16;
  p.drop = R.drop; p.drop.tag += (unsigned long long)t;
}
static void fill_fc_fwd(FwdProjJob& p, const FcStage& F, int t) {
  p.h = F.in + (size_t)t * F.N * F.ld_in; p.WpT = F.WT; p.WpT_sw = nullptr; p.ldh = F.ld_in;
  p.m_prev = nullptr; p.m_out = F.y + (size_t)t * F.N * F.ldy; p.ldm = F.ldy;
  p.out = F.out2 + ((size_t)t * F.Ns2 + F.row02) * F.ld2; p.ldo = F.ld2;
  p.res_in = nullptr; p.res_out = nullptr; p.len = nullptr; p.bias = F.bias; p.noise = F.noise;
  p.P = F.D; p.t = t; p.N = F.N;
  p.nblk_c = (F.D + 15) / 16;
  p.drop = DropSpec{};
}
static void fill_fc_bwd(BwdBJob& b, const FcStage& F, int t) {
  b.dz = F.in + (size_t)t * F.N * F.ld_in; b.K = F.WT; b.Ksw = nullptr; b.H4 = F.ld_in;
  b.dx = F.y + (size_t)t * F.N * F.ldy; b.lddx = F.ldy; b.dmst = nullptr; b.len = nullptr;
  b.I = F.D; b.n_begin = 0; b.n_end = F.D; b.ldm = 0; b.t = t; b.N = F.N;
  b.dx_accumulate = F.accumulate ? 1 : 0;
  b.nblk_c = (F.D + 15) / 16;
}
static void fill_bwd_a(BwdAJob& a, const LayerRun& R, int t) {
  const LstmLayer& L = *R.L; const LstmStash& S = *R.S; const ParamSet& ps = *R.ps;
  const int H = L.H, H4 = 4 * H;
  const size_t r = (size_t)t * R.Ns + R.row0, rn = (size_t)(t + 1) * R.Ns + R.row0;
  a.dout = R.dout ? R.dout + r * L.ldP : nullptr;
  a.dmst = S.dmst + (size_t)R.row0 * L.ldP; a.Wp = L.has_proj ? ps.W(L.tWp) : nullptr; a.Wp_sw = L.has_proj ? L.Wp_sw : nullptr;
  a.dmt = S.dmt + r * L.ldP;
  a.gates = S.gates + r * H4;
  a.c_prev = S.c + r * H; a.c_cur = S.c + rn * H;
  a.wf = ps.W(L.twf); a.wi = ps.W(L.twi); a.wo = ps.W(L.two);
  a.dc = S.dc + (size_t)R.row0 * H; a.len = R.len; a.ldm = L.ldP; a.P = L.P; a.t = t; a.N = R.N; a.H = H;
  a.nblk_c = (H + bwd_a_cells() - 1) / bwd_a_cells();
  a.drop = R.drop; a.drop.tag += (unsigned long long)t;
}
static void fill_bwd_b(BwdBJob& b, const LayerRun& R, int t, bool with_dx) {
  const LstmLayer& L = *R.L; const LstmStash& S = *R.S; const ParamSet& ps = *R.ps;
  const int H4 = 4 * L.H;
  const size_t r = (size_t)t * R.Ns + R.row0;
  b.dz = S.gates + r * H4; b.K = ps.W(L.tK); b.Ksw = with_dx ? L.Kb_full : L.Kb_rec;
  b.dx = with_dx ? R.din + r * L.ldI : nullptr;
  b.dmst = S.dmst + (size_t)R.row0 * L.ldP; b.len = R.len;
  b.I = L.I; b.n_begin = with_dx ? 0 : L.I; b.n_end = L.I + L.P; b.lddx = L.ldI; b.ldm = L.ldP; b.t = t; b.N = R.N; b.H4 = H4;
  b.dx_accumulate = R.din_accumulate ? 1 : 0;
  b.nblk_c = (b.n_end - b.n_begin + 15) / 16;
}

int Model::gates_blocks(int H, int N) const { return job_blocks((H + 15) / 16, N, fwd_gates_rows()); }
int Model::proj_blocks(int P, int N) const { return job_blocks((P + 15) / 16, N); }
int Model::bwd_a_blocks(int H, int N) const { return job_blocks((H + bwd_a_cells() - 1) / bwd_a_cells(), N); }
static void run_gates(const FwdGateJobs& gj, int blocks, int kb, hipStream_t s) { launch_fwd_gates(gj, blocks, kb, s); }
static void run_proj(const FwdProjJobs& pj, int blocks, int kb, hipStream_t s) { launch_fwd_proj(pj, blocks, kb, s); }
static void run_bwd_a(const BwdAJobs& aj, int blocks, int kb, hipStream_t s) { launch_bwd_a(aj, blocks, kb, s); }
void Model::run_bwd_b_splitk(BwdBJobs& bj, hipStream_t s) { bwd_b_plan(bj, bwdb_ws); launch_bwd_b_splitk(bj, s); }

static void prof_ring_room(std::vector<hipEvent_t>& ev, int n, size_t step) {
  if ((size_t)(2 * n + 2) <= ev.size()) return;
  const size_t old = ev.size();
  ev.resize(old + step, nullptr);
  for (size_t i = old; i < ev.size(); ++i) (void)hipEventCreate(&ev[i]);
}
void Model::gates_launch(const FwdGateJobs& gj, int blocks, int kb, hipStream_t s) {
  if (!prof_on) { run_gates(gj, blocks, kb, s); return; }
  prof_ring_room(prof_ev, prof_n, 128);
  for (int i = 0; i < gj.n; ++i) {
    const FwdGateJob& J = gj.j[i];
    prof_flops += 2.0 * J.N * ((J.x ? J.ldx : 0) + J.ldm) * 4.0 * J.H;
// ... 711 lines not shown
```

rsrgan_amd/csrc/model.h:

```cpp
#pragma once
#include <hip/hip_runtime.h>
#include <stdint.h>
#include <string>
#include <unordered_map>
#include <functional>
#include <vector>

#include "../../include/rsrgan.h"
#include "kernels.h"

namespace rsr {

inline int pad4(int x) { return (x + 3) & ~3; }

struct TensorDesc {
  std::string name;
  int rows, cols, ld;
  int64_t off;
  int64_t dense_off;
  bool l2;
  bool trainable = true;
  bool is_vector;
  int xavier_fan_out = 0;
  float bias_init = 0.f;
// ... 214 lines not shown
  void persist_disable(int which);
  bool gp_fwd_on() const { return gp_gran1 && (gp_live & 1); }
  bool gpersist_shape(GPersistArgs& a, int T) const;
  int gp_np_nt = 0;
  bool gp_noproj = false;
  bool gpersist_args(GPersistArgs& a, int T) const;
  void gpersist_rearm();
  bool persist_forward_g(int T, hipStream_t s);
  float* g_state = nullptr;
  int g_state_sf = 0;
  bool g_carry = false;
  void gstate_xfer(int dir, int T, int rows, const int* mask, hipStream_t s);
  typedef std::function<void(hipStream_t)> StreamFn;
  bool persist_backward_g(const Chain& ch, int T, hipStream_t s, bool check_only = false, const StreamFn& pre = nullptr, const StreamFn& post = nullptr);
  std::vector<FcLayer> gfc, dfc;
  std::vector<float*> g_act, d_act;
  float *fc_dA = nullptr, *fc_dB = nullptr, *joint = nullptr, *dy_buf = nullptr;
  int ldJ = 0;
  int *adam_t_dev_d = nullptr;
  bool g_dnn() const { return cfg.g_type == RSRGAN_G_DNN || cfg.g_type == RSRGAN_G_RCED; }
  bool g_rced() const { return cfg.g_type == RSRGAN_G_RCED; }
  bool g_resi() const { return cfg.g_type == RSRGAN_G_RES_LSTM_I; }
  std::vector<BnlCell> bnl;
  bool g_bnl() const { return cfg.g_type == RSRGAN_G_BNLSTM; }
  int bnl_check(const rsrgan_cfg& c) const;
  void bnl_params();
  void bnl_alloc();
  void bnl_init(std::vector<float>& host, uint64_t seed) const;
  BnlLayer bnl_args(int l, bool train) const;
  void bnl_forward(int T, bool train, hipStream_t s);
  void bnl_backward(int T, float* dy, hipStream_t s);
  int bnl_step(const float* x, const float* labels, const int32_t* lengths, int T, float* out_losses, bool want_grads, hipStream_t s);
  bool bnl_infer() const { return g_bnl() && infer(); }
  void bnl_infer_layers();
  void bnl_refresh_fold(hipStream_t s);
  std::vector<ConvLayer> gconv;
  FcLayer rc_fc{};
  std::vector<float*> rc_act;
  float *rc_col = nullptr, *rc_dcol = nullptr, *rc_dA = nullptr, *rc_dB = nullptr;
  std::vector<float*> rc_cols;
  std::vector<float*> rc_ft_fwd, rc_ft_bwd;
  std::vector<char> rc_wgrad_implicit;
  float* rc_wg_ws = nullptr;
  float* rc_x4 = nullptr;
  bool rc_keep_cols = false;
  size_t scratch_floats = 0;
  int rcS = 0, rcW = 0;
  void g_frame_forward(int rows, hipStream_t s);
  void g_frame_backward(int rows, float* dy, hipStream_t s);
  void rced_forward(int rows, hipStream_t s);
  void rced_backward(int rows, float* dy, hipStream_t s);
  bool d_dnn() const { return cfg.d_type == RSRGAN_D_DNN && !(cfg.flags & RSRGAN_FLAG_INFER); }
  bool d_adam() const { return g_dnn(); }
  void fc_forward(const ParamSet& ps, const std::vector<FcLayer>& L, const std::vector<float*>& act, int rows, hipStream_t s, int calls = 1,
                  int call0 = 0);
  float keep_prob = 1.f;
  uint64_t drop_seed = 0, drop_run = 0;
  bool drop_training() const {
    return g_dnn() && keep_prob < 1.f && !cfg.cross_validation && !bn_eval_call && scal[RSRGAN_L2_SCALE] > 0.0;
  }
  uint64_t drop_key(int net, int layer, int call) const;
  unsigned long long* drop_ctr = nullptr;
  bool seq_drop_on() const { return !g_dnn() && keep_prob < 1.f && !cfg.cross_validation && !bn_eval_call; }
  unsigned drop_thr() const { return (unsigned)((double)keep_prob * 16777216.0); }
  float* fc_backward(const ParamSet& ps, const std::vector<FcLayer>& L, const std::vector<float*>& act, int rows, float* dtop,
                     bool want_wgrads, bool want_din, hipStream_t s, int calls = 1, int row0 = 0, int call0 = 0);
  bool bn_on() const { return (cfg.flags & RSRGAN_FLAG_BATCH_NORM) != 0; }
  bool bn_eval_call = false;
  bool bn_training() const { return bn_on() && !cfg.cross_validation && !bn_eval_call; }
  BnVars bn_vars(const ParamSet& ps, const FcLayer& F) const;
  BnVars bn_vars(const ParamSet& ps, const int (&tbn)[8]) const;
  void bn_commit_stack(const ParamSet& ps, const std::vector<FcLayer>& L, int times0, int times1, BnCommitList& cl);
  float* bn_sums = nullptr;
  bool seq_bn() const { return bn_on() && cfg.g_type == RSRGAN_G_LSTM; }
  int g_bn_t[8] = {-1, -1, -1, -1, -1, -1, -1, -1};
  float* g_z0 = nullptr;
  float* g_bn_stat = nullptr;
  float* g_bn_sums = nullptr;
  float* g_bn_scr = nullptr;
  bool g_fwd_bn_train = false;
  void g_fc_in_backward(float* d, int R, float* colsum_scratch, hipStream_t q);
  void seq_bn_commit(int times, hipStream_t s);
  bool seq_bn_infer() const { return seq_bn() && infer(); }
  float* g_bn_fold_b = nullptr;
  std::vector<float> g_w0_host;
  bool g_fc_in_unfolded = false;
  void seq_bn_fold(hipStream_t s);
  void d_dnn_forward_loss(int T, int Nd, int n_real, bool want_grads, float* loss3, hipStream_t s, int calls = 1, int call0 = 0);
  void bn_commit_run(bool with_d, hipStream_t s);
  int dnn_d_backward(const float* x, const float* labels, int T, float* out_losses, bool want_grads, hipStream_t s);
  int dnn_g_backward(const float* x, const float* labels, int T, float* out_losses, bool want_grads, bool reuse, hipStream_t s);

  float *dyn = nullptr;
  int *adam_t_dev = nullptr;
  float *losses = nullptr;
  float *tmp3 = nullptr;
  float *scratch = nullptr;
  double scal[RSRGAN_SCALAR_COUNT_] = {0};
  bool g_fwd_valid = false;
  int cur_T = 0;
  bool d_grads_ready = false, g_grads_ready = false;
  std::vector<void*> allocs;
  size_t alloc_bytes = 0;

  int init(const rsrgan_cfg& c, uint64_t seed);
  int check_cfg() const;
  void build_tables();
  void plan_rows();
  int alloc_params();
  int alloc_generator();
  void alloc_rced();
  int alloc_discriminator();
  int alloc_shared();
  int plan_persistent();
  int plan_dpersist();
  int plan_gpersist();
  int init_values(uint64_t seed);
  size_t frame_rows() const { return (size_t)Tmax * B; }
  int g_ldP() const { return g_dnn() ? 4 : pad4(gR); }
  int d_ldP() const { return d_dnn() ? 4 : pad4(dR); }
  bool res_sums() const { return cfg.g_type == RSRGAN_G_RES_LSTM_L || cfg.g_type == RSRGAN_G_RES_LSTM_I; }
  bool ema_on() const { return cfg.ema_decay > 0.f && !infer(); }
  template <typename T> T* alloc(size_t n);
  template <typename T> T* alloc_opt(size_t n);
  void* alloc_raw(size_t bytes, bool required);
  int alloc_status(const char* stage) const;
  bool alloc_fail = false;
  size_t alloc_fail_bytes = 0;
  void destroy();

  int prepare_batch(const float* x, const float* labels, const int32_t* lengths, int T, hipStream_t s, const float** nr = nullptr,
                    const float** nf = nullptr, hipStream_t early = nullptr);
  void g_forward(int T, hipStream_t s, Chain* extra = nullptr);
  void g_forward_head(int T, hipStream_t s);
  void g_forward_tail(int T, hipStream_t s);
  void d_logits(int N, int T, hipStream_t s);
  void d_backward_pass(int N, int T, bool want_wgrads, bool need_dx0, const float* dlog, hipStream_t s, bool head_done = false);
  bool d_head(int N, int T, int n_real, const float* t_real, const float* t_fake, float* loss3, bool want_grads, bool want_wgrads, hipStream_t s);
  void g_backward_pass(int T, float* dy, hipStream_t s);
  void g_fc_out_wgrads(const float* dy, int R, hipStream_t q);
  float* wire_g_bptt(Chain& ch, float* a, float* b);
  float* wire_d_bptt(Chain& ch, bool want_wgrads, float* din0, bool accumulate0);
  FcStage g_out_fc_stage(const float* nf, int Ns2, int row02);
  bool d_head_or_logits(int N, int T, int n_real, const float* t_fake, float* loss3, bool want_grads, bool want_wgrads, hipStream_t s);
  void g_loss_tail(bool l2, hipStream_t s);
  GRunPlan plan_g_run(int T, const float* nf, bool want_grads, bool reuse, hipStream_t s);
  void g_fc_side_pair(const GRunPlan& p, StreamFn& pre, StreamFn& post);
  bool g_run_forward(const GRunPlan& p, hipStream_t s);
  void g_run_d_forward(const GRunPlan& p, hipStream_t s);
  bool g_run_loss_head(const GRunPlan& p, hipStream_t s);
  bool g_run_backward(const GRunPlan& p, bool g_head, hipStream_t s);
  bool g_run_bptt_fused(const GRunPlan& p, hipStream_t s);
  void g_run_bwd_rest(const GRunPlan& p, hipStream_t s);
  void g_run_tail(const GRunPlan& p, hipStream_t s);
  int g_supervised_step(const float* x, const float* labels, const int32_t* lengths, int T, float* out_losses, bool want_grads, hipStream_t s);
  DRunPlan plan_d_run(int T, const float* nr, const float* nf, bool want_grads, hipStream_t s);
  void d_run_forward(const DRunPlan& p, hipStream_t s);
  void d_run_head_backward(const DRunPlan& p, hipStream_t s);
  bool g_forward_persist(int T, hipStream_t s);
  int d_backward(const float* x, const float* labels, const int32_t* lengths, int T, const float* nr, const float* nf,
                 float* out_losses, bool want_grads, hipStream_t s);
  int g_backward(const float* x, const float* labels, const int32_t* lengths, int T, const float* nf,
                 float* out_losses, bool want_grads, bool reuse, hipStream_t s);
  int apply(int net, hipStream_t s);
  void apply_body(int net, hipStream_t s);
  int apply_inlined = 0;
  void refresh_transposes(int net, hipStream_t s);
  void refresh_swizzles(int net, hipStream_t s);
  bool lazy_sw = false;

  void rnn_forward(std::vector<Chain>& chains, int T, hipStream_t s, const std::vector<int>* offsets = nullptr,
                   const std::vector<FcStage>* fcs = nullptr);
  void rnn_backward(std::vector<Chain>& chains, int T, hipStream_t s, const std::vector<int>* offsets = nullptr,
                    const std::vector<FcStage>* fcs = nullptr);
  void layer_wgrads(const LayerRun& R, int T, hipStream_t s);
  void chain_wgrads(const Chain& ch, int T, hipStream_t s, const StreamFn& between, const StreamFn& pre = nullptr, const StreamFn& post = nullptr);
  void layer_wgrads_gemms(const LayerRun& R, int t0, int t1, bool accumulate, hipStream_t s, bool do_dK = true, bool do_dWp = true);
  int trail_nrt() const;
  bool batch_wgrads(const Chain& ch, int T, hipStream_t s, bool dK_too, bool* dK_done, bool check_only = false);
  void layer_wgrads_colsums(const LayerRun& R, int T, hipStream_t s, float* scr);
  hipStream_t side = nullptr;
  struct GradBucket { int64_t off = 0, count = 0; hipEvent_t ev = nullptr; bool marked = false; };
  std::vector<GradBucket> gbk[2];
  bool fused_apply = false;
  bool defer_wgrads = false;
  int build_buckets();
  void mark_bucket(int net, int i, hipStream_t s);
  void finish_buckets(int net, hipStream_t s);
  bool prof_on = false;
  std::vector<hipEvent_t> prof_ev;
  int prof_n = 0;
  double prof_flops = 0.0;
  std::vector<hipEvent_t> prof_gp_ev;
  int prof_gp_n = 0;
  double prof_gp_flops = 0.0;
  std::vector<hipEvent_t> prof_gb_ev;
  int prof_gb_n = 0;
  int prof_fdt_n = 0;
  int prof_cnt[9] = {};
  double prof_gb_flops = 0.0;
  void gates_launch(const FwdGateJobs& gj, int blocks, int kb, hipStream_t s);
  int gates_blocks(int H, int N) const;
  int proj_blocks(int P, int N) const;
  int bwd_a_blocks(int H, int N) const;
  void run_bwd_b_splitk(BwdBJobs& bj, hipStream_t s);
  hipEvent_t ev_pool[16] = {};
  int ev_next = 0;
  float* gemm_ws2 = nullptr;
  float* dk_tmp = nullptr;
  size_t dk_tmp_per = 0;
  float* scratch2 = nullptr;
  bool overlap() const { return side != nullptr && (cfg.flags & RSRGAN_FLAG_OVERLAP) != 0; }
  Chain g_chain(int T);
  Chain d_chain(int N, int Ns, int row0);
  void gemm(const float* A, int lda, bool a_kc, const float* B, int ldb, bool b_kc, float* C, int ldc, int M, int N,
            int K, const float* bias, int act, float alpha, bool accumulate, hipStream_t s);
  bool supervised() const { return (cfg.flags & RSRGAN_FLAG_SUPERVISED) != 0; }
  bool infer() const { return (cfg.flags & RSRGAN_FLAG_INFER) != 0; }
  static constexpr int INFER_WINDOW = 64;
  int inf_W = 0;
  int* len_win = nullptr;
  int inf_t0 = 0, inf_slot = 0;
  bool inf_failed = false;
  bool infer_fallback_stash();
  void infer_forward(int T, hipStream_t s);
  void infer_window_launches(int t0, int Tw, hipStream_t s);
  void infer_state_to_slot0(hipStream_t s);
  bool wavefront() const { return (cfg.flags & RSRGAN_FLAG_WAVEFRONT) != 0; }
  float* g_fc_out_wT = nullptr;
  float* bwdb_ws = nullptr;
  size_t bwdb_ws_floats = 0;
  bool bwd_b_splitk_ok(const BwdBJobs& jobs) const;
  float* gemm_ws = nullptr;
  size_t gemm_ws_floats = 0;

  struct GraphSlot { int uses = 0; hipGraphExec_t exec = nullptr; };
  std::unordered_map<uint64_t, GraphSlot> graphs;
  hipStream_t main_s = nullptr;
  hipEvent_t ev_in = nullptr, ev_out = nullptr;
  hipEvent_t ev_last = nullptr; bool ev_last_set = false;
  float *noise_r_buf = nullptr, *noise_f_buf = nullptr;
  bool graphs_on() const { return (cfg.flags & RSRGAN_FLAG_GRAPH) != 0 && wavefront() && !overlap() && !prof_on && !g_dnn() && sw.graphs; }
  template <class F> void run_seg(uint64_t key, hipStream_t s, F&& body);
  void drop_graphs();
  hipStream_t enter(hipStream_t caller);
  void leave(hipStream_t caller, hipStream_t work);
  const float* stage_noise(const float* src, float* buf, hipStream_t s);
};

void set_error(const char* fmt, ...);
const char* get_error();

#define HIPC(expr)                                                                   \
  do {                                                                               \
    hipError_t e_ = (expr);                                                          \
    if (e_ != hipSuccess) {                                                          \
      rsr::set_error("%s failed: %s (%s:%d)", #expr, hipGetErrorString(e_), __FILE__, __LINE__); \
      return RSRGAN_ERR_HIP;                                                         \
    }                                                                                \
  } while (0)

}
```

rsrgan_amd/csrc/model_init.cpp:

```cpp
#include "model.h"

#include <algorithm>
#include <cmath>
#include <random>

namespace rsr {

int ParamSet::add(const std::string& name, int rows, int cols, bool is_vector) {
  TensorDesc d;
  d.name = name;
  d.rows = rows; d.cols = cols; d.ld = pad4(cols);
  d.off = padded; d.dense_off = dense;
  d.l2 = name.find("bias") == std::string::npos;
  d.is_vector = is_vector;
  padded += ((int64_t)rows * d.ld + 63) / 64 * 64;
  dense += (int64_t)rows * cols;
  t.push_back(d);
  return (int)t.size() - 1;
}

void* Model::alloc_raw(size_t bytes, bool required) {
  void* p = nullptr;
  if (hipMalloc(&p, bytes) != hipSuccess) {
    if (required && !alloc_fail) { alloc_fail = true; alloc_fail_bytes = bytes; }
// ... 494 lines not shown
  }
  if (!inf && switches().dk_pad && !gl.empty() && gl[0].has_proj && gl[0].I % 4 != 0 && gl[0].ldI % 4 == 0 && gl.size() <= (size_t)GEMM_MAXB) {
    dk_tmp_per = (size_t)(gl[0].ldI + gl[0].P) * 4 * gl[0].H;
    dk_tmp = alloc_opt<float>(dk_tmp_per * gl.size());
    if (!dk_tmp) dk_tmp_per = 0;
  }
  if (!gemm_ws2) side = nullptr;
  if (int rc = alloc_status("shared work space")) return rc;
  HIPC(hipMemset(drop_ctr, 0, 16));
  return RSRGAN_OK;
}

int Model::plan_persistent() {
  if (int rc = plan_dpersist()) return rc;
  if (int rc = plan_gpersist()) return rc;
  if (bnl_infer() && !gp_fwd_on()) {
    set_error("g_type bnlstm with RSRGAN_FLAG_INFER: no persistent forward plan for this configuration (batch_size=%d padded to %d rows, %d x %d / p%d; "
              "gpersist_plan's shapes, every workgroup of a row group resident at once, RSRGAN_GPERSIST / RSRGAN_PAD_ROWS not switched off), "
              "and a launch-per-phase forward of the folded cell is not built", Bt, B, cfg.g_layers, cfg.g_cells, cfg.g_proj);
    return RSRGAN_ERR_INVALID;
  }
  GPersistArgs ga{};
  if (sw.trail && dp_gran && (dp_live & 2) && gp_gran1 && gp_gran3 && !gp_noproj && (gp_live & 2) && B % 32 == 0 && gpersist_args(ga, gp_Tcap))
    trail_fits = resident_probe(gpersist_grid(ga) + ((dpersist_trail_grid((int)dl.size(), B) + 7) & ~7), GP_THREADS,
                                std::max(gpersist_lds_bytes(), dpersist_trail_lds_bytes()));
  lazy_sw = switches().lazy_swizzle && wavefront() && gp_gran1 && gp_gran3 && (gp_live & 3) == 3 && dp_gran && (dp_live & 3) == 3;
  if (sw.dpipe > 0 && trail_fits && side && !d_dnn() && dp_max_grid >= dpersist_grid((int)dl.size(), B)) {
    const size_t gb = dpersist_granule_bytes((int)dl.size(), B, Tmax) / 2;
    dp_gran2 = (unsigned long long*)alloc_opt<float>(gb / sizeof(float));
    dp_ctl2 = (unsigned*)alloc_opt<float>(16);
    if (dp_gran2 && dp_ctl2 && hipEventCreateWithFlags(&ev_dfree, hipEventDisableTiming) == hipSuccess &&
        hipEventCreateWithFlags(&ev_real, hipEventDisableTiming) == hipSuccess) {
      HIPC(ctl_reset(dp_ctl2));
      dpipe = true;
    }
  }
  return RSRGAN_OK;
}

int Model::plan_dpersist() {
  if (dp_live && !dl.empty() && dl.size() <= (size_t)DP_MAXL && B % 16 == 0) {
    const int nl_ = (int)dl.size();
    for (int rows : {2 * B, B}) {
      const int g_ = dpersist_grid(nl_, rows);
      if (g_ <= 128 && resident_probe(g_, 512, dpersist_lds_bytes())) { dp_max_grid = g_; break; }
    }
  }
  if (dp_max_grid <= 0) return RSRGAN_OK;
  dp_gran_bytes = dpersist_granule_bytes((int)dl.size(), 2 * B, Tmax);
  dp_gran = (unsigned long long*)alloc<float>(dp_gran_bytes / sizeof(float));
  dp_ctl = (unsigned*)alloc<float>(16);
  if (int rc = alloc_status("persistent discriminator rings")) return rc;
  HIPC(ctl_reset(dp_ctl));
  DPersistArgs pa{};
  pa.nl = (int)dl.size(); pa.N = 2 * B; pa.H = dl[0].H;
  for (size_t l = 0; l < dl.size(); ++l) { pa.L[l].I = dl[l].I; pa.L[l].P = dl[l].P; pa.L[l].ldP = dl[l].ldP; pa.L[l].ldI = dl[l].ldI; }
  bool shapes = switches().dw_inkernel && (dp_live & 2) && dpersist_dw_supported(pa) && !d_adam();
  for (auto& L : dl) shapes = shapes && L.has_proj && L.H == dl[0].H && L.ldH == dl[0].ldH;
  if (shapes && dpersist_grid(pa.nl, pa.N) == dp_max_grid) {
    const int nt = pa.N / 16;
    dw_stride = dpersist_dw_stride(pa);
    dw_ws = alloc_opt<float>((size_t)pa.nl * nt * dw_stride);
    dw_flag = (unsigned*)alloc_opt<float>(dpersist_dw_flag_bytes(pa.nl, pa.N, Tmax) / sizeof(float));
    std::vector<long long> src(D.t.size(), -1);
    const int IP = dl[0].I + dl[0].P, H4 = 4 * dl[0].H, H_ = dl[0].H;
    for (size_t l = 0; l < dl.size(); ++l) {
      const long long base = (long long)l * nt * (long long)dw_stride;
      src[dl[l].tK] = base; src[dl[l].tb] = base + (long long)IP * H4;
      const long long pp = base + (long long)(IP + 1) * H4;
      src[dl[l].twi] = pp; src[dl[l].twf] = pp + H_; src[dl[l].two] = pp + 2 * H_; src[dl[l].tWp] = pp + 3 * H_;
    }
    dw_src = (long long*)alloc_opt<float>(src.size() * 2);
    if (dw_ws && dw_flag && dw_src) HIPC(hipMemcpy(dw_src, src.data(), src.size() * sizeof(long long), hipMemcpyHostToDevice));
    else dw_ws = nullptr;
  }
  return RSRGAN_OK;
}

int Model::plan_gpersist() {
  const bool inf = infer();
  if (!gp_live || g_dnn() || (g_bnl() && !inf)) return RSRGAN_OK;
  auto ring = [&](size_t bytes) { return (unsigned long long*)alloc_opt<float>(bytes / sizeof(float)); };
  GPersistArgs ga{};
  gp_Tcap = std::min(Tmax, (int)GP_TMAX);
  gp_noproj = !gl.empty() && !gl[0].has_proj;
  if (gp_noproj) {
    bool fits = false;
    for (int nt : {2, 4}) {
      gp_np_nt = nt;
      if (gpersist_shape(ga, gp_Tcap) && resident_probe(gpersist_grid(ga), GP_THREADS, gpersist_np_lds_bytes())) { fits = true; break; }
    }
    if (!fits) { gp_np_nt = 0; return RSRGAN_OK; }
    gp_gran2_bytes = gpersist_np_gran2_bytes(ga);
    gp_gran2 = ring(gp_gran2_bytes);
    gp_ctl = (unsigned*)alloc_opt<float>(16);
    if (gp_np_nt == 2 && (gp_live & 2) && switches().gp_np_bwd && !inf) {
      gp_gran1 = ring(gpersist_np_gran1_bytes(ga));
      gp_gran3 = ring(gpersist_np_gran3_bytes(ga));
      if (!gp_gran1 || !gp_gran3) { gp_gran1 = gp_gran3 = nullptr; }
    }
    if (!gp_gran1) gp_gran1 = gp_gran2;
    if (gp_gran2 && gp_ctl) {
      HIPC(ctl_reset(gp_ctl));
      gpersist_rearm();
    } else { gp_gran1 = gp_gran2 = gp_gran3 = nullptr; gp_ctl = nullptr; }
  } else if (gpersist_args(ga, gp_Tcap) && resident_probe(gpersist_grid(ga), GP_THREADS, gpersist_lds_bytes())) {
    gp_gran1 = ring(gpersist_gran1_bytes(ga));
    gp_gran2_bytes = gpersist_gran2_bytes(ga);
    gp_gran2 = ring(gp_gran2_bytes);
    gp_ctl = (unsigned*)alloc_opt<float>(16);
    bool bwd_ok = (gp_live & 2) != 0 && !inf;
    for (auto& L : gl) bwd_ok = bwd_ok && L.P > 16;
    if (bwd_ok) gp_gran3 = ring(gpersist_gran3_bytes(ga));
    if (gp_gran1 && gp_gran2 && gp_ctl) {
      HIPC(ctl_reset(gp_ctl));
      gpersist_rearm();
    } else { gp_gran1 = gp_gran2 = nullptr; gp_ctl = nullptr; }
  }
  return RSRGAN_OK;
}

int Model::init_values(uint64_t seed) {
  const rsrgan_cfg& c = cfg;
  const bool inf = infer();
  std::mt19937_64 rng(seed);
  for (ParamSet* ps : {&G, &D}) {
    if (ps == &D && inf) continue;
    std::vector<float> host((size_t)ps->padded, 0.f);
    if (ps == &G && g_bnl()) bnl_init(host, seed);
    else for (auto& t : ps->t) {
      if (!t.l2 || t.const_init) {
        if (t.bias_init != 0.f)
          for (int cc = 0; cc < t.cols; ++cc) host[(size_t)t.off + cc] = t.bias_init;
        continue;
      }
      const double fan_in = t.is_vector ? t.cols : t.rows, fan_out = t.xavier_fan_out > 0 ? t.xavier_fan_out : t.cols;
      const double lim = std::sqrt(6.0 / (fan_in + fan_out));
      std::uniform_real_distribution<double> u(-lim, lim);
      for (int r = 0; r < t.rows; ++r)
        for (int cc = 0; cc < t.cols; ++cc) host[(size_t)t.off + (size_t)r * t.ld + cc] = (float)u(rng);
    }
    HIPC(hipMemcpy(ps->w, host.data(), host.size() * sizeof(float), hipMemcpyHostToDevice));
    if (ps->ema) HIPC(hipMemcpy(ps->ema, host.data(), host.size() * sizeof(float), hipMemcpyHostToDevice));
  }
  scal[RSRGAN_G_LEARNING_RATE] = 8e-5; scal[RSRGAN_D_LEARNING_RATE] = 1e-3; scal[RSRGAN_MSE_LAMBDA] = 10.0;
  scal[RSRGAN_D_REAL] = 1.0; scal[RSRGAN_D_FAKE] = 0.0; scal[RSRGAN_L2_SCALE] = c.l2_scale;
  scal[RSRGAN_CLIP_NORM] = c.clip_norm; scal[RSRGAN_ADAM_STEP] = 0;
  float hdyn[DYN_COUNT] = {0};
  hdyn[DYN_G_LR] = 8e-5f; hdyn[DYN_D_LR] = 1e-3f; hdyn[DYN_LAMBDA] = 10.f; hdyn[DYN_D_REAL] = 1.f; hdyn[DYN_D_FAKE] = 0.f;
  hdyn[DYN_L2] = c.l2_scale; hdyn[DYN_CLIP] = c.clip_norm; hdyn[DYN_B1] = c.adam_beta1; hdyn[DYN_B2] = c.adam_beta2;
  hdyn[DYN_EPS] = c.adam_eps; hdyn[DYN_EMA] = c.ema_decay;
  HIPC(hipMemcpy(dyn, hdyn, sizeof(hdyn), hipMemcpyHostToDevice));
  g_fc_in_unfolded = true;
  refresh_transposes(RSRGAN_NET_G, nullptr);
  if (!inf) {
    refresh_transposes(RSRGAN_NET_D, nullptr);
    int rc = build_buckets(); if (rc) return rc;
  }
  HIPC(hipDeviceSynchronize());
  HIPC(hipGetLastError());
  return RSRGAN_OK;
}

void Model::destroy() {
  drop_graphs();
  if (main_s) {
    (void)hipStreamSynchronize(main_s);
    if (ev_in) (void)hipEventDestroy(ev_in);
    if (ev_out) (void)hipEventDestroy(ev_out);
    (void)hipStreamDestroy(main_s);
    main_s = nullptr;
  }
  if (side) {
    (void)hipStreamSynchronize(side);
    for (auto& e : ev_pool) if (e) (void)hipEventDestroy(e);
    (void)hipStreamDestroy(side);
    side = nullptr;
  }
  if (ev_last) { (void)hipEventDestroy(ev_last); ev_last = nullptr; ev_last_set = false; }
  if (ev_dfree) { (void)hipEventDestroy(ev_dfree); ev_dfree = nullptr; }
  if (ev_real) { (void)hipEventDestroy(ev_real); ev_real = nullptr; }
  dpipe = false;
  for (auto& v : gbk) { for (auto& b : v) if (b.ev) (void)hipEventDestroy(b.ev); v.clear(); }
  for (auto& e : prof_ev) if (e) (void)hipEventDestroy(e);
  prof_ev.clear();
  for (auto& e : prof_gp_ev) if (e) (void)hipEventDestroy(e);
  prof_gp_ev.clear();
  for (auto& e : prof_gb_ev) if (e) (void)hipEventDestroy(e);
  prof_gb_ev.clear();
  for (void* p : allocs) (void)hipFree(p);
  allocs.clear();
}

int Model::build_buckets() {
  auto range = [](const ParamSet& ps, int lo, int hi, GradBucket& b) {
    b.off = ps.t[lo].off;
    b.count = (hi + 1 < (int)ps.t.size() ? ps.t[hi + 1].off : ps.padded) - b.off;
  };
  auto whole = [](const ParamSet& ps, std::vector<GradBucket>& v) { GradBucket b; b.off = 0; b.count = ps.padded; v.assign(1, b); };
  whole(D, gbk[RSRGAN_NET_D]);
  whole(G, gbk[RSRGAN_NET_G]);
  if (!g_dnn() && wavefront()) {
    std::vector<GradBucket> v;
    bool ok = true;
    GradBucket b;
    range(G, g_fc_out_w, g_fc_out_b, b); ok = ok && g_fc_out_b == g_fc_out_w + 1; v.push_back(b);
    if (cfg.g_type == RSRGAN_G_LSTM) {
      const int hi = seq_bn() ? g_bn_t[7] : g_fc_in_b;
      range(G, g_fc_in_w, hi, b); ok = ok && hi == g_fc_in_w + (seq_bn() ? 8 : 1); v.push_back(b);
    }
    for (auto& L : gl) {
      const int lo = L.tK, hi = L.has_proj ? L.tWp : L.two;
      ok = ok && L.tb > lo && L.tb < hi && L.twf > lo && L.twi > lo && L.two <= hi && hi - lo == (L.has_proj ? 5 : 4);
      range(G, lo, hi, b); v.push_back(b);
    }
    int64_t covered = 0;
    for (auto& x : v) covered += x.count;
    if (ok && covered == G.padded) gbk[RSRGAN_NET_G] = v;
  }
  for (auto& v : gbk)
    for (auto& b : v)
      if (hipEventCreateWithFlags(&b.ev, hipEventDisableTiming) != hipSuccess) { set_error("hipEventCreate failed"); return RSRGAN_ERR_HIP; }
  return RSRGAN_OK;
}

}
```

rsrgan_amd/csrc/model_step.cpp:

```cpp
#include "model.h"

#include <cmath>
#include <cstdio>
#include <cstdlib>
#include <cstring>

namespace rsr {

static inline uint64_t seg_key(int seg, int T, unsigned bits) { return ((uint64_t)seg << 48) | ((uint64_t)(unsigned)T << 16) | (bits & 0xffffu); }
enum { SEG_D = 1, SEG_G_MAIN = 2, SEG_G_FCIN = 3, SEG_G_LAYER0 = 4 , SEG_G_L2 = 20, SEG_G_TAIL = 21, SEG_APPLY_D = 22, SEG_APPLY_G = 23, SEG_G_BATCH = 24, SEG_BNL = 25 };

template <class F>
void Model::run_seg(uint64_t key, hipStream_t s, F&& body) {
  if (!graphs_on() || s == nullptr) { body(); return; }
  if (graphs.size() > 96) drop_graphs();
  GraphSlot& g = graphs[key];
  if (g.exec) { if (hipGraphLaunch(g.exec, s) != hipSuccess) { (void)hipGetLastError(); g.exec = nullptr; g.uses = -1; body(); } return; }
  if (g.uses < 0) { body(); return; }
  if (g.uses++ == 0) { body(); return; }
  if (hipStreamBeginCapture(s, hipStreamCaptureModeThreadLocal) != hipSuccess) { (void)hipGetLastError(); g.uses = -1; body(); return; }
  body();
  hipGraph_t gr = nullptr;
  if (hipStreamEndCapture(s, &gr) != hipSuccess || !gr) {
    (void)hipGetLastError(); g.uses = -1;
// ... 150 lines not shown
void Model::g_forward_tail(int T, hipStream_t s) {
  const int P = gR, ldP = pad4(P);
  gemm(g_ins[gl.size()], ldP, true, G.W(g_fc_out_w), ldDout, false, y_tm, ldDout, T * B, Dout, P, G.W(g_fc_out_b), 0, 0.f, false, s);
  g_fwd_valid = true;
}
void Model::g_forward(int T, hipStream_t s, Chain* extra) {
  if (g_dnn()) { bn_eval_call = false; g_frame_forward(T * B, s); g_fwd_valid = true; return; }
  if (g_bnl() && !infer()) { bnl_forward(T, false, s); return; }
  g_forward_head(T, s);
  if (infer()) { infer_forward(T, s); g_forward_tail(T, s); return; }
  if (!extra && persist_forward_g(T, s)) { g_forward_tail(T, s); return; }
  std::vector<Chain> chains;
  chains.push_back(g_chain(T));
  if (extra) chains.push_back(*extra);
  rnn_forward(chains, T, s);
  g_forward_tail(T, s);
}

bool Model::infer_fallback_stash() {
  for (size_t l = 0; l < gl.size(); ++l) {
    LstmStash& S = g_st[l];
    if (!S.gates) S.gates = alloc_opt<float>((size_t)inf_W * B * 4 * gl[l].H);
    if (!S.h) S.h = alloc_opt<float>((size_t)inf_W * B * gl[l].ldH);
    if (!S.gates || !S.h) return false;
  }
  return true;
}
void Model::infer_window_launches(int t0, int Tw, hipStream_t s) {
  const bool res_l = cfg.g_type == RSRGAN_G_RES_LSTM_L, res_any = res_l || g_resi();
  const size_t top = gl.size() - 1;
  const float* x0 = g_ins[0] + (size_t)t0 * B * gl[0].ldI;
  std::vector<LstmStash> st(g_st);
  Chain ch;
  for (size_t l = 0; l < gl.size(); ++l) {
    const size_t o = l == top ? (size_t)t0 * B * gl[l].ldP : 0;
    if (!res_any) st[l].out += o;
    LayerRun R;
    R.ps = &G; R.L = &gl[l]; R.S = &st[l]; R.in = l == 0 ? x0 : g_ins[l];
    R.N = B; R.Ns = B; R.row0 = 0; R.len = len_win;
    R.zx_batched = (l == 0);
    R.carry = g_carry;
    if (res_l) { R.res_in = R.in; R.res_out = g_res[l] + o; }
    if (g_resi()) { R.res_in = x0; R.res_out = g_res[l] + o; }
    ch.push_back(R);
  }
  std::vector<Chain> chains{ch};
  rnn_forward(chains, Tw, s);
}
void Model::infer_forward(int T, hipStream_t s) {
  const bool carry_in = g_carry;
  bool persist = gp_fwd_on() && wavefront();
  for (int t0 = 0; t0 < T;) {
    const int Tw = std::min(T - t0, persist ? gp_Tcap : inf_W);
    g_carry = carry_in || t0 > 0;
    inf_t0 = t0;
    launch_window_len(len_dev, len_win, B, t0, Tw, s);
    if (persist && persist_forward_g(Tw, s)) {
      inf_slot = 1;
    } else if (bnl_infer()) {
      set_error("g_type bnlstm inference handle: the persistent forward is off after a reported device failure, and no other forward is built");
      inf_failed = true; break;
    } else if (persist) {
      persist = false;
      continue;
    } else {
      if (!infer_fallback_stash()) { set_error("hipMalloc failed (the launch path's stash of an inference handle)"); inf_failed = true; break; }
      infer_window_launches(t0, Tw, s);
      inf_slot = Tw;
    }
    t0 += Tw;
    if (t0 < T) infer_state_to_slot0(s);
  }
  g_carry = carry_in;
  inf_t0 = 0;
}
void Model::infer_state_to_slot0(hipStream_t s) {
  for (size_t l = 0; l < gl.size(); ++l) {
    const size_t nc = (size_t)B * gl[l].H, nm = (size_t)B * gl[l].ldP;
    (void)hipMemcpyAsync(g_st[l].c, g_st[l].c + (size_t)inf_slot * nc, nc * sizeof(float), hipMemcpyDeviceToDevice, s);
    (void)hipMemcpyAsync(g_st[l].mst, g_st[l].mst + (size_t)inf_slot * nm, nm * sizeof(float), hipMemcpyDeviceToDevice, s);
  }
}

void Model::d_logits(int N, int T, hipStream_t s) {
  const int ldPd = pad4(dR);
  gemm(d_st[dl.size() - 1].out, ldPd, true, D.W(d_fc_w), 4, false, logits, 4, T * N, 1, dR, D.W(d_fc_b), 0, 0.f, false, s);
}

bool Model::d_head(int N, int T, int n_real, const float* t_real, const float* t_fake, float* loss3, bool want_grads, bool want_wgrads,
                   hipStream_t s) {
  const int ldPd = pad4(dR), nb = (T * N + 63) / 64;
  if (!switches().dhead || d_dnn() || dl.empty() || dR % 4 != 0 || dR + 3 > 64 ||
      (size_t)nb * (DH_MAXR + 3) > scratch_floats) return false;
  DHeadArgs a{};
  a.top = d_st[dl.size() - 1].out; a.ldt = ldPd; a.w = D.W(d_fc_w); a.ldw = 4; a.b = D.W(d_fc_b);
  a.logits = logits; a.ldl = 4; a.dlogits = dlogits; a.dout = d_dB; a.ldo = ldPd; a.gw = D.Gd(d_fc_w); a.gb = D.Gd(d_fc_b);
  a.T = T; a.Nd = N; a.n_real = n_real; a.dR = dR; a.t_real = t_real; a.t_fake = t_fake; a.loss3 = loss3; a.part = scratch;
  a.want_grads = want_grads ? 1 : 0; a.want_wgrads = want_wgrads ? 1 : 0;
  a.Bp = pad_Bp(); a.Bt = Bt;
  launch_dhead(a, s);
  return true;
}

bool Model::d_head_or_logits(int N, int T, int n_real, const float* t_fake, float* loss3, bool want_grads, bool want_wgrads, hipStream_t s) {
  if (d_head(N, T, n_real, dyn + DYN_D_REAL, t_fake, loss3, want_grads, want_wgrads, s)) return true;
  d_logits(N, T, s);
  launch_lsgan(logits, 4, want_grads ? dlogits : nullptr, T, N, n_real, dyn + DYN_D_REAL, t_fake, loss3, s, false, 0.f, 0.f, pad_Bp(), Bt);
  return false;
}

float* Model::wire_d_bptt(Chain& ch, bool want_wgrads, float* din0, bool accumulate0) {
  float* cur = d_dB;
  float* other = d_dA;
  for (int l = (int)ch.size() - 1; l >= 0; --l) {
    ch[l].dout = cur; ch[l].want_wgrads = want_wgrads;
    if (l == 0) { ch[l].din = din0; ch[l].din_accumulate = accumulate0; }
    else { ch[l].din = other; ch[l].din_accumulate = false; std::swap(cur, other); }
  }
  return other;
}

float* Model::wire_g_bptt(Chain& ch, float* a, float* b) {
  for (int l = (int)ch.size() - 1; l >= 0; --l) {
    ch[l].want_wgrads = true;
    if (cfg.g_type == RSRGAN_G_RES_LSTM_L) {
      ch[l].dout = a; ch[l].din = l > 0 ? a : nullptr; ch[l].din_accumulate = true;
    } else {
      const bool need = cfg.g_type == RSRGAN_G_LSTM || l > 0;
      ch[l].dout = a; ch[l].din = need ? b : nullptr; ch[l].din_accumulate = false;
      std::swap(a, b);
    }
  }
  return a;
}

void Model::g_fc_out_wgrads(const float* dy, int R, hipStream_t q) {
  const int P = gR, ldP = pad4(P);
  gemm(g_ins[gl.size()], ldP, false, dy, ldDout, false, G.Gd(g_fc_out_w), ldDout, P, Dout, R, nullptr, 0, 0.f, false, q);
  launch_colsum(dy, ldDout, nullptr, 0, G.Gd(g_fc_out_b), R, Dout, (side && q == side) ? scratch2 : scratch, q);
}

FcStage Model::g_out_fc_stage(const float* nf, int Ns2, int row02) {
  FcStage F;
  F.offset = (int)gl.size(); F.N = B; F.K = gR; F.D = Dout;
  F.in = g_ins[gl.size()]; F.ld_in = pad4(gR); F.WT = g_fc_out_wT; F.bias = G.W(g_fc_out_b); F.noise = nf;
  F.y = y_tm; F.ldy = ldDout; F.out2 = xd; F.ld2 = ldDout; F.Ns2 = Ns2; F.row02 = row02;
  return F;
}

void Model::g_loss_tail(bool l2, hipStream_t s) {
  if (l2) {
    launch_l2(G.w, G.g, G.ct, dyn + DYN_L2, G.partial, s);
    launch_l2_total(G.partial, G.ct.n_chunks, dyn + DYN_L2, losses + 5, s);
  } else {
    (void)hipMemsetAsync(losses + 5, 0, sizeof(float), s);
  }
  launch_g_total(losses + 3, dyn + DYN_LAMBDA, s);
}

bool Model::g_forward_persist(int T, hipStream_t s) {
  if (!persist_forward_g(T, s)) return false;
  g_forward_tail(T, s);
  return true;
}

void Model::d_backward_pass(int N, int T, bool want_wgrads, bool need_dx0, const float* dlog, hipStream_t s, bool head_done) {
  const int R = T * N;
  const int ldPd = pad4(dR);
  const float* top = d_st[dl.size() - 1].out;
  if (want_wgrads && !head_done) {
    gemm(top, ldPd, false, dlog, 4, false, D.Gd(d_fc_w), 4, dR, 1, R, nullptr, 0, 0.f, false, s);
    launch_colsum(dlog, 4, nullptr, 0, D.Gd(d_fc_b), R, 1, scratch, s);
  }
  if (!head_done) gemm(dlog, 4, true, D.W(d_fc_w), 4, true, d_dB, ldPd, R, dR, 1, nullptr, 0, 0.f, false, s);
  std::vector<Chain> chains(1, d_chain(N, N, 0));
  Chain& ch = chains[0];
  last_dx0 = wire_d_bptt(ch, want_wgrads, nullptr, false);
  if (need_dx0) ch[0].din = last_dx0;
  if (!persist_backward(ch, T, s)) rnn_backward(chains, T, s);
}

void Model::g_backward_pass(int T, float* dy, hipStream_t s) {
  const int R = T * B;
  const int P = gR, ldP = pad4(P);
  g_fc_out_wgrads(dy, R, s);
  gemm(dy, ldDout, true, G.W(g_fc_out_w), ldDout, true, g_dA, ldP, R, P, Dout, nullptr, 0, 0.f, false, s);
  std::vector<Chain> chains(1, g_chain(T));
  float* dh0 = wire_g_bptt(chains[0], g_dA, g_dB);
  if (!persist_backward_g(chains[0], T, s)) rnn_backward(chains, T, s);
  if (cfg.g_type == RSRGAN_G_LSTM) g_fc_in_backward(dh0, R, scratch, s);
}

DRunPlan Model::plan_d_run(int T, const float* nr, const float* nf, bool want_grads, hipStream_t s) {
  DRunPlan p;
  p.T = T; p.want_grads = want_grads; p.nr = nr; p.nf = nf;
  if (dpipe && (!nr || sw.dpipe >= 2) && wavefront() && gp_fwd_on() && !d_dnn() && !seq_drop_on() && T > 0 && T <= Tmax) {
    Chain dchk = d_chain(B, 2 * B, B);
    p.dsplit = persist_forward_real(T, side, true) && persist_forward_g_trail(dchk, T, s, nf, true);
  }
  p.inl = fused_apply && switches().fused_seg && want_grads && !d_dnn() && graphs_on();
  return p;
}

void Model::d_run_forward(const DRunPlan& p, hipStream_t s) {
  const int T = p.T;
  if (p.dsplit) {
    g_forward_head(T, s);
    Chain dch = d_chain(B, 2 * B, B);
    if (persist_forward_g_trail(dch, T, s, p.nf)) return;
  }
  if (wavefront() && gp_fwd_on()) {
    g_forward_head(T, s);
    if (g_forward_persist(T, s)) {
      launch_add_noise_rows(y_tm, p.nf, xd, B, T, Dout, ldDout, 2 * B, B, s);
      if (!d_dnn()) {
        std::vector<Chain> chains(1, d_chain(2 * B, 2 * B, 0));
        if (!persist_forward(chains[0], T, s)) rnn_forward(chains, T, s);
      }
      return;
    }
  }
  if (wavefront()) {
    if (!gp_fwd_on()) g_forward_head(T, s);
    const int Lg = (int)gl.size();
    std::vector<Chain> chains{g_chain(T)};
    std::vector<int> offs{0};
    if (!d_dnn()) {
      chains.push_back(d_chain(B, 2 * B, 0)); offs.push_back(0);
      chains.push_back(d_chain(B, 2 * B, B)); offs.push_back(Lg + 1);
    }
    std::vector<FcStage> fcs{g_out_fc_stage(p.nf, 2 * B, B)};
    rnn_forward(chains, T, s, &offs, &fcs);
    return;
  }
  g_forward(T, s);
  launch_add_noise_rows(y_tm, p.nf, xd, B, T, Dout, ldDout, 2 * B, B, s);
  if (!d_dnn()) {
    std::vector<Chain> chains(1, d_chain(2 * B, 2 * B, 0));
    rnn_forward(chains, T, s);
  }
}

void Model::d_run_head_backward(const DRunPlan& p, hipStream_t s) {
  const int T = p.T;
  if (d_dnn()) {
    d_dnn_forward_loss(T, 2 * B, B, p.want_grads, losses, s);
    if (p.want_grads) fc_backward(D, dfc, d_act, T * 2 * B, dlogits, true, false, s);
    return;
  }
  const bool head = d_head_or_logits(2 * B, T, B, dyn + DYN_D_FAKE, losses, p.want_grads, p.want_grads, s);
  if (p.want_grads) d_backward_pass(2 * B, T, true, false, dlogits, s, head);
}

int Model::d_backward(const float* x, const float* labels, const int32_t* lengths, int T, const float* nr, const float* nf,
                      float* out_losses, bool want_grads, hipStream_t s) {
  if (!labels) { set_error("labels required"); return RSRGAN_ERR_INVALID; }
  if (supervised()) { set_error("RSRGAN_FLAG_SUPERVISED: the trainer graph has no discriminator step"); return RSRGAN_ERR_STATE; }
  if (g_dnn()) return dnn_d_backward(x, labels, T, out_losses, want_grads, s);
  if (d_dnn()) { nr = nullptr; nf = nullptr; }
  bn_eval_call = !want_grads;
  if (seq_bn()) g_fwd_bn_train = bn_training();
  dfree_current = false;
  DRunPlan p = plan_d_run(T, nr, nf, want_grads, s);
  int rc = prepare_batch(x, labels, lengths, T, s, &p.nr, &p.nf, p.dsplit ? side : nullptr);
  if (rc) return rc;
  p.kbits = (want_grads ? 1u : 0u) | (p.nr ? 2u : 0u) | (p.nf ? 4u : 0u) | (p.inl ? 8u : 0u) | (p.dsplit ? 16u : 0u);
  if (p.dsplit) {
    launch_add_noise_rows(lab_tm, p.nr, xd, B, T, Dout, ldDout, 2 * B, 0, side);
    (void)persist_forward_real(T, side);
    (void)hipEventRecord(ev_real, side);
    (void)hipStreamWaitEvent(s, ev_real, 0);
  }
  if (seq_drop_on()) launch_drop_tick(drop_ctr, s);
  run_seg(seg_key(SEG_D, T, p.kbits), s, [&]() {
    if (!p.dsplit) launch_add_noise_rows(lab_tm, p.nr, xd, B, T, Dout, ldDout, 2 * B, 0, s);
    d_run_forward(p, s);
    d_run_head_backward(p, s);
    if (p.inl) apply_body(RSRGAN_NET_D, s);
  });
  dlog_T = T; dlog_rows = 2 * B; dlog_fake0 = (size_t)B;
  d_partial_fresh = false;
  g_fwd_valid = true;
  if (p.inl) apply_inlined |= 2;
  if (want_grads) { finish_buckets(RSRGAN_NET_D, s); d_grads_ready = true; }
  if (out_losses) launch_copy_f(losses, out_losses, 3, s);
  HIPC(hipGetLastError());
  return RSRGAN_OK;
}

GRunPlan Model::plan_g_run(int T, const float* nf, bool want_grads, bool reuse, hipStream_t s) {
  GRunPlan p;
  p.T = T; p.R = T * B; p.want_grads = want_grads; p.reuse = reuse; p.nf = nf;
  p.l2_on = !cfg.cross_validation && scal[RSRGAN_L2_SCALE] > 0.0;
  p.wave_bwd = want_grads && !d_dnn() && wavefront();
  const bool fused_seg = switches().fused_seg;
  p.bucketed = p.wave_bwd && gbk[RSRGAN_NET_G].size() > 1 && !overlap() && !(fused_apply && fused_seg);
  p.dy = g_dB;
  if (p.wave_bwd) {
    p.dch = d_chain(B, B, 0);
    wire_d_bptt(p.dch, false, p.dy, true);
    p.gch = g_chain(T);
    p.dh0 = wire_g_bptt(p.gch, g_dA, g_dC);
    p.g_bptt_persist = dl[0].ldI == ldDout && persist_backward_g(p.gch, T, s, true);
  }
  const bool fc_side_env = switches().wgrad_streams >= 2 && switches().fc_side;
  p.fcs_inside = p.wave_bwd && !p.bucketed && side && fc_side_env && cfg.g_type == RSRGAN_G_LSTM && p.g_bptt_persist;
  p.inl = fused_apply && fused_seg && p.wave_bwd && !p.bucketed && graphs_on() && !(cfg.g_type == RSRGAN_G_LSTM && !p.fcs_inside);
  p.kbits = (want_grads ? 1u : 0u) | (nf ? 2u : 0u) | (reuse ? 4u : 0u) | (p.l2_on ? 8u : 0u) | (p.bucketed ? 16u : 0u) | (p.inl ? 32u : 0u);
  if (p.g_bptt_persist) {
    Chain dc0 = p.dch;
    dc0[0].din = nullptr;
    p.trail_plan = persist_backward_trail(dc0, T, s, p.dy, ldDout, g_dA, pad4(gR), true);
  }
  p.gsplit = dpipe && p.trail_plan;
  return p;
}

void Model::g_fc_side_pair(const GRunPlan& p, StreamFn& pre, StreamFn& post) {
  if (!p.fcs_inside) return;
  const float* dy = p.dy; float* dh0 = p.dh0; const int R = p.R;
  pre = [this, dy, R](hipStream_t q) { g_fc_out_wgrads(dy, R, q); };
  post = [this, dh0, R](hipStream_t q) { g_fc_in_backward(dh0, R, (side && q == side) ? scratch2 : scratch, q); };
}

bool Model::g_run_forward(const GRunPlan& p, hipStream_t s) {
  const int T = p.T;
  if (p.reuse) return false;
  if (!wavefront()) { g_forward(T, s); return false; }
  if (gp_fwd_on()) {
    g_forward_head(T, s);
    if (!d_dnn()) {
      Chain dch = d_chain(B, B, 0);
      if (persist_forward_g_trail(dch, T, s, p.nf)) return true;
    }
    if (g_forward_persist(T, s)) return false;
  }
  if (!gp_fwd_on()) g_forward_head(T, s);
  std::vector<Chain> chains{g_chain(T)};
  std::vector<int> offs{0};
  if (!d_dnn()) { chains.push_back(d_chain(B, B, 0)); offs.push_back((int)gl.size() + 1); }
  std::vector<FcStage> fcs{g_out_fc_stage(p.nf, B, 0)};
  rnn_forward(chains, T, s, &offs, &fcs);
  return true;
}

void Model::g_run_d_forward(const GRunPlan& p, hipStream_t s) {
  const int T = p.T;
  const bool direct = !p.nf && !d_dnn() && dl[0].ldI == ldDout;
  if (!direct) launch_add_noise_rows(y_tm, p.nf, xd, B, T, Dout, ldDout, B, 0, s);
  if (d_dnn()) return;
  std::vector<Chain> chains(1, d_chain(B, B, 0));
  if (direct) chains[0][0].in = y_tm;
  if (!persist_forward(chains[0], T, s) && !fold_forward(chains[0], T, s)) rnn_forward(chains, T, s);
}

bool Model::g_run_loss_head(const GRunPlan& p, hipStream_t s) {
  bool g_head = false;
  if (d_dnn()) d_dnn_forward_loss(p.T, B, 0, p.want_grads, tmp3, s);
  else g_head = d_head_or_logits(B, p.T, 0, dyn + DYN_D_REAL, tmp3, p.want_grads, false, s);
  launch_copy_f(tmp3 + 1, losses + 3, 1, s);
  return g_head;
}

bool Model::g_run_backward(const GRunPlan& p, bool g_head, hipStream_t s) {
  const int T = p.T, R = p.R;
  if (!p.want_grads) {
    launch_mse(y_tm, lab_tm, ldDout, nullptr, R, Dout, dyn + DYN_LAMBDA, false, losses + 4, scratch, s, pad_Bp(), Bt);
    return true;
  }
  if (d_dnn()) {
    float* dyd = fc_backward(D, dfc, d_act, R, dlogits, false, true, s);
    launch_mse(y_tm, lab_tm, ldDout, dyd, R, Dout, dyn + DYN_LAMBDA, true, losses + 4, scratch, s, pad_Bp(), Bt);
    g_backward_pass(T, dyd, s);
    return true;
  }
  if (!p.wave_bwd) {
    d_backward_pass(B, T, false, true, dlogits, s, g_head);
    float* dyd = last_dx0;
    launch_mse(y_tm, lab_tm, ldDout, dyd, R, Dout, dyn + DYN_LAMBDA, true, losses + 4, scratch, s, pad_Bp(), Bt);
    g_backward_pass(T, dyd, s);
    return true;
  }
  const int Ld = (int)dl.size(), ldPd = pad4(dR);
  if (!g_head) gemm(dlogits, 4, true, D.W(d_fc_w), 4, true, d_dB, ldPd, R, dR, 1, nullptr, 0, 0.f, false, s);
  launch_mse(y_tm, lab_tm, ldDout, p.dy, R, Dout, dyn + DYN_LAMBDA, false, losses + 4, scratch, s, pad_Bp(), Bt);
  if (p.g_bptt_persist) {
    if (!g_run_bptt_fused(p, s)) return false;
  } else {
    FcStage F;
    F.offset = Ld; F.N = B; F.K = Dout; F.D = gR;
    F.in = p.dy; F.ld_in = ldDout; F.WT = G.W(g_fc_out_w); F.y = g_dA; F.ldy = pad4(gR); F.accumulate = false;
    std::vector<int> offs{0, Ld + 1};
    std::vector<FcStage> fcs{F};
    std::vector<Chain> chains{p.dch, p.gch};
    ScopedSet<bool> defer(defer_wgrads, p.bucketed);
    rnn_backward(chains, T, s, &offs, &fcs);
  }
  if (!p.fcs_inside) g_fc_out_wgrads(p.dy, R, s);
  return true;
}

bool Model::g_run_bptt_fused(const GRunPlan& p, hipStream_t s) {
  const int T = p.T, R = p.R, ldP = pad4(gR);
  ScopedSet<bool> defer(defer_wgrads, p.bucketed);
  std::vector<Chain> dc1(1, p.dch);
  dc1[0][0].din = nullptr;
  const bool trailed = p.trail_plan && persist_backward_trail(dc1[0], T, s, p.dy, ldDout, g_dA, ldP);
  if (!trailed) {
    if (!persist_backward(dc1[0], T, s)) rnn_backward(dc1, T, s);
    const int H4d = 4 * dl[0].H;
    gemm(d_st[0].gates, H4d, true, D.W(dl[0].tK), H4d, true, p.dy, ldDout, R, dl[0].I, H4d, nullptr, 0, 0.f, true, s);
    gemm(p.dy, ldDout, true, G.W(g_fc_out_w), ldDout, true, g_dA, ldP, R, gR, Dout, nullptr, 0, 0.f, false, s);
  }
  ScopedSet<bool> trail(gp_trail_next, trailed);
  StreamFn pre, post;
  g_fc_side_pair(p, pre, post);
  ScopedSet<int> phase(gp_phase, p.gsplit ? 1 : 0);
  persist_backward_g(p.gch, T, s, false, pre, post);
  return !p.gsplit;
}

void Model::g_run_bwd_rest(const GRunPlan& p, hipStream_t s) {
  StreamFn pre, post;
  g_fc_side_pair(p, pre, post);
  {
    ScopedSet<int> workers(g_gemm_workers, std::min(g_gemm_workers, switches().dpipe_w));
    {
      ScopedSet<bool> defer(defer_wgrads, p.bucketed);
      ScopedSet<int> phase(gp_phase, 2);
      persist_backward_g(p.gch, p.T, s, false, pre, post);
    }
    if (!p.fcs_inside) g_fc_out_wgrads(p.dy, p.R, s);
  }
  if (p.inl) { g_run_tail(p, s); apply_body(RSRGAN_NET_G, s); }
}

void Model::g_run_tail(const GRunPlan& p, hipStream_t s) {
  g_loss_tail(p.want_grads && p.l2_on, s);
  if (seq_bn() && p.want_grads && bn_training()) seq_bn_commit(2, s);
}

int Model::g_backward(const float* x, const float* labels, const int32_t* lengths, int T, const float* nf,
                      float* out_losses, bool want_grads, bool reuse, hipStream_t s) {
  if (!labels) { set_error("labels required"); return RSRGAN_ERR_INVALID; }
  dlog_T = 0;
  if (g_dnn()) return dnn_g_backward(x, labels, T, out_losses, want_grads, reuse, s);
  if (g_bnl()) return bnl_step(x, labels, lengths, T, out_losses, want_grads, s);
  bn_eval_call = !want_grads;
  if (seq_bn() && want_grads && cfg.cross_validation) {
    set_error("RSRGAN_FLAG_BATCH_NORM: gradients of the cross_validation model (moving-statistics batch norm) are not built");
    return RSRGAN_ERR_INVALID;
  }
  if (seq_bn() && reuse && g_fwd_bn_train != bn_training()) reuse = false;
  if (seq_bn() && !reuse) g_fwd_bn_train = bn_training();
  dfree_current = false;
  if (seq_drop_on()) { reuse = false; launch_drop_tick(drop_ctr, s); }
  if (supervised()) return g_supervised_step(x, labels, lengths, T, out_losses, want_grads, s);
  if (d_dnn()) nf = nullptr;
  if (reuse) {
    if (!g_fwd_valid || T != cur_T) { set_error("reuse_g_forward without a valid generator forward"); return RSRGAN_ERR_STATE; }
  } else {
    int rc = prepare_batch(x, labels, lengths, T, s);
    if (rc) return rc;
  }
  nf = stage_noise(nf, noise_f_buf, s);
  const GRunPlan p = plan_g_run(T, nf, want_grads, reuse, s);

  run_seg(seg_key(SEG_G_MAIN, T, p.kbits | (p.trail_plan ? 64u : 0u) | (p.gsplit ? 128u : 0u)), s, [&]() {
    if (p.trail_plan) gpersist_arm_bytes(g_dA, (size_t)T * B * pad4(gR) * sizeof(float), s);
    if (!g_run_forward(p, s)) g_run_d_forward(p, s);
    const bool g_head = g_run_loss_head(p, s);
    if (!g_run_backward(p, g_head, s)) return;
    if (p.inl) { g_run_tail(p, s); apply_body(RSRGAN_NET_G, s); }
  });
  if (p.gsplit) {
    (void)hipEventRecord(ev_dfree, s);
    dfree_inside = true; dfree_current = true;
    run_seg(seg_key(SEG_G_MAIN, T, p.kbits | 64u | 256u), s, [&]() { g_run_bwd_rest(p, s); });
  }
  if (p.inl) apply_inlined |= 1;
  if (!reuse) g_fwd_valid = true;
  if (p.wave_bwd) {
    int bi = 0;
    if (p.bucketed) mark_bucket(RSRGAN_NET_G, bi++, s);
    if (cfg.g_type == RSRGAN_G_LSTM && !p.fcs_inside) {
      run_seg(seg_key(SEG_G_FCIN, T, p.kbits), s, [&]() { g_fc_in_backward(p.dh0, p.R, scratch, s); });
      if (p.bucketed) mark_bucket(RSRGAN_NET_G, bi++, s);
    }
    if (p.bucketed) {
      bool dkd = false;
      const bool gb = batch_wgrads(p.gch, T, s, false, &dkd, true);
      if (gb) run_seg(seg_key(SEG_G_BATCH, T, p.kbits), s, [&]() { bool d_ = false; (void)batch_wgrads(p.gch, T, s, false, &d_); });
      int li = 0;
      for (auto& Rr : p.gch) {
        run_seg(seg_key(SEG_G_LAYER0 + li, T, p.kbits), s, [&]() { if (gb) layer_wgrads_gemms(Rr, 0, T, false, s, true, false); else layer_wgrads(Rr, T, s); });
        mark_bucket(RSRGAN_NET_G, bi++, s);
        ++li;
      }
    }
  }
  if (!p.inl) run_seg(seg_key(SEG_G_TAIL, T, p.kbits), s, [&]() { g_run_tail(p, s); });
  if (want_grads) {
    if (p.l2_on) for (auto& bk : gbk[RSRGAN_NET_G]) bk.marked = false;
    finish_buckets(RSRGAN_NET_G, s);
    g_grads_ready = true;
  }
  if (out_losses) launch_copy_f(losses + 3, out_losses, 4, s);
  HIPC(hipGetLastError());
  return RSRGAN_OK;
}

int Model::g_supervised_step(const float* x, const float* labels, const int32_t* lengths, int T, float* out_losses, bool want_grads, hipStream_t s) {
  int rc = prepare_batch(x, labels, lengths, T, s);
  if (rc) return rc;
  g_forward(T, s);
  const bool l2s = !cfg.cross_validation && scal[RSRGAN_L2_SCALE] > 0.0;
  HIPC(hipMemsetAsync(losses + 3, 0, sizeof(float), s));
  if (want_grads) {
    float* dy = g_dC;
    launch_mse(y_tm, lab_tm, ldDout, dy, T * B, Dout, dyn + DYN_LAMBDA, false, losses + 4, scratch, s, pad_Bp(), Bt);
    g_backward_pass(T, dy, s);
    if (l2s) {
      launch_l2(G.w, G.g, G.ct, dyn + DYN_L2, G.partial, s);
      launch_l2_total(G.partial, G.ct.n_chunks, dyn + DYN_L2, losses + 5, s);
    }
    if (seq_bn() && bn_training()) seq_bn_commit(2, s);
    { finish_buckets(RSRGAN_NET_G, s); g_grads_ready = true; }
  } else {
    launch_mse(y_tm, lab_tm, ldDout, nullptr, T * B, Dout, dyn + DYN_LAMBDA, false, losses + 4, scratch, s, pad_Bp(), Bt);
  }
  if (!(want_grads && l2s)) HIPC(hipMemsetAsync(losses + 5, 0, sizeof(float), s));
  launch_g_total(losses + 3, dyn + DYN_LAMBDA, s);
  if (out_losses) launch_copy_f(losses + 3, out_losses, 4, s);
  HIPC(hipGetLastError());
  return RSRGAN_OK;
}

int Model::bnl_step(const float* x, const float* labels, const int32_t* lengths, int T, float* out_losses, bool want_grads, hipStream_t s) {
  if (want_grads && cfg.cross_validation) {
    set_error("g_type bnlstm: gradients of the cross_validation model (moving-statistics batch norm) are not built");
    return RSRGAN_ERR_INVALID;
  }
  int rc = prepare_batch(x, labels, lengths, T, s);
  if (rc) return rc;
  const bool l2s = want_grads && scal[RSRGAN_L2_SCALE] > 0.0;
  run_seg(seg_key(SEG_BNL, T, (want_grads ? 1u : 0u) | (l2s ? 2u : 0u)), s, [&]() {
    bnl_forward(T, want_grads, s);
    (void)hipMemsetAsync(losses + 3, 0, sizeof(float), s);
    float* dy = want_grads ? g_dC : nullptr;
    launch_mse(y_tm, lab_tm, ldDout, dy, T * B, Dout, dyn + DYN_LAMBDA, false, losses + 4, scratch, s, pad_Bp(), Bt);
    if (want_grads) bnl_backward(T, dy, s);
    g_loss_tail(l2s, s);
  });
  if (want_grads) { finish_buckets(RSRGAN_NET_G, s); g_grads_ready = true; }
  g_fwd_valid = false;
  if (out_losses) launch_copy_f(losses + 3, out_losses, 4, s);
  HIPC(hipGetLastError());
  return RSRGAN_OK;
}

void Model::apply_body(int net, hipStream_t s) {
  if (net == RSRGAN_NET_D) {
    if (!d_partial_fresh) launch_sumsq(D.g, D.ct, D.partial, s);
    d_partial_fresh = false;
    if (d_adam()) {
      launch_adam_tick(dyn, adam_t_dev_d, (double)cfg.adam_beta1, (double)cfg.adam_beta2, s, DYN_D_LR, DYN_ADAM_LRT_D);
      launch_apply_adam(D.w, D.g, D.m, D.v, D.ema, D.ct, D.partial, dyn, s, DYN_ADAM_LRT_D);
    } else {
      launch_apply_sgd(D.w, D.g, D.ema, D.ct, D.partial, dyn, s);
    }
    refresh_transposes(RSRGAN_NET_D, s);
  } else {
    launch_sumsq(G.g, G.ct, G.partial, s);
    launch_adam_tick(dyn, adam_t_dev, (double)cfg.adam_beta1, (double)cfg.adam_beta2, s);
    launch_apply_adam(G.w, G.g, G.m, G.v, G.ema, G.ct, G.partial, dyn, s);
    refresh_transposes(RSRGAN_NET_G, s);
  }
}

int Model::apply(int net, hipStream_t s) {
  if (net == RSRGAN_NET_D) {
    if (!d_grads_ready) { set_error("apply(D) without gradients"); return RSRGAN_ERR_STATE; }
    if (!(apply_inlined & 2)) run_seg(seg_key(SEG_APPLY_D, 0, 0), s, [&]() { apply_body(RSRGAN_NET_D, s); });
    apply_inlined &= ~2;
    if (d_adam()) scal[RSRGAN_ADAM_STEP_D] += 1;
    d_grads_ready = false;
  } else if (net == RSRGAN_NET_G) {
    if (!g_grads_ready) { set_error("apply(G) without gradients"); return RSRGAN_ERR_STATE; }
    if (!(apply_inlined & 1)) run_seg(seg_key(SEG_APPLY_G, 0, 0), s, [&]() { apply_body(RSRGAN_NET_G, s); });
    if (dfree_current) dfree_inside = true;
    apply_inlined &= ~1;
    scal[RSRGAN_ADAM_STEP] += 1;
    g_grads_ready = false;
    g_fwd_valid = false;
  } else {
    set_error("bad net %d", net);
    return RSRGAN_ERR_INVALID;
  }
  HIPC(hipGetLastError());
  return RSRGAN_OK;
}

}
```

Baseline: 1.330 million.

## Fuse weight transposes into optimizer apply and fold tick/total into sumsq

The Adam/SGD apply kernels now also write the transposed weight images through extra tiled blocks, so the separate transpose pass after each update can be skipped. The Adam tick and the G total-loss computation run on the first thread of the sumsq kernel, and the memset for a zero L2 loss is folded into the total kernel. This removes several small kernel launches and a full re-read of the weights per update. In exchange the apply kernel gains extra blocks and per-block table scans, and the image table must exactly cover each tensor or the path falls back to the old transposes.

```diff
diff --git a/include/rsrgan.h b/include/rsrgan.h
--- a/include/rsrgan.h
+++ b/include/rsrgan.h
@@ -226,6 +226,9 @@
 
 int rsrgan_op_chunks(const int64_t* tensors, int32_t n_tensors, int32_t* out, int64_t out_ints, int32_t* n_chunks);
 int rsrgan_op_update(int32_t op, const void* const* ptrs, const int64_t* dims, const float* fl, void* stream);
+int rsrgan_op_sumsq_riders(const void* const* ptrs, const int64_t* dims, const float* fl, void* stream);
+int rsrgan_op_update_images(int32_t op, const void* const* ptrs, const int64_t* dims, const int64_t* images, int32_t n_images,
+                            const void* const* dst, void* stream);
 int rsrgan_op_step_elem(int32_t op, const void* const* ptrs, const int64_t* dims, const float* fl, void* stream);
 int rsrgan_op_layout(int32_t op, const void* const* ptrs, const int64_t* dims, const float* fl, void* stream);
 
diff --git a/rsrgan_amd/_lib.py b/rsrgan_amd/_lib.py
--- a/rsrgan_amd/_lib.py
+++ b/rsrgan_amd/_lib.py
@@ -33,7 +33,7 @@
            "rsrgan_hist", "rsrgan_hist_limits", "rsrgan_d_logits", "rsrgan_d_logits_hist",
            "rsrgan_op_segan_sizes", "rsrgan_op_segan_conv2", "rsrgan_op_segan_conv1", "rsrgan_op_segan_colred", "rsrgan_op_segan_last_plan",
            "rsrgan_op_segan_vbn", "rsrgan_op_segan_elem", "rsrgan_op_segan_dhead",
-           "rsrgan_op_chunks", "rsrgan_op_update", "rsrgan_op_step_elem", "rsrgan_op_layout",
+           "rsrgan_op_chunks", "rsrgan_op_update", "rsrgan_op_update_images", "rsrgan_op_sumsq_riders", "rsrgan_op_step_elem", "rsrgan_op_layout",
            "rsrgan_segan_default_cfg", "rsrgan_segan_create", "rsrgan_segan_destroy", "rsrgan_segan_set_scalar",
            "rsrgan_segan_num_tensors", "rsrgan_segan_tensor_info", "rsrgan_segan_param_count", "rsrgan_segan_get_params",
            "rsrgan_segan_set_params", "rsrgan_segan_forward_g", "rsrgan_segan_d_backward", "rsrgan_segan_g_backward",
@@ -151,6 +151,8 @@
         f.argtypes = [i32, C.POINTER(vp), C.POINTER(i64), C.POINTER(C.c_float), vp]
     lib.rsrgan_op_segan_last_plan.argtypes = [C.POINTER(i32)]
     lib.rsrgan_op_chunks.argtypes = [C.POINTER(i64), i32, C.POINTER(i32), i64, C.POINTER(i32)]
+    lib.rsrgan_op_sumsq_riders.argtypes = [C.POINTER(vp), C.POINTER(i64), C.POINTER(C.c_float), vp]
+    lib.rsrgan_op_update_images.argtypes = [i32, C.POINTER(vp), C.POINTER(i64), C.POINTER(i64), i32, C.POINTER(vp), vp]
     lib.rsrgan_segan_default_cfg.argtypes = [C.POINTER(SeganCfg)]
     lib.rsrgan_segan_create.argtypes = [C.POINTER(SeganCfg), C.c_uint64, C.POINTER(vp)]
     lib.rsrgan_segan_destroy.argtypes = [vp]
diff --git a/rsrgan_amd/csrc/capi_ops.cpp b/rsrgan_amd/csrc/capi_ops.cpp
--- a/rsrgan_amd/csrc/capi_ops.cpp
+++ b/rsrgan_amd/csrc/capi_ops.cpp
@@ -744,9 +744,9 @@
 #undef WHO
 
 #define WHO "op_update"
-int rsrgan_op_update(int32_t op, const void* const* ptrs, const int64_t* dims, const float* fl, void* stream) {
-  (void)fl;
-  return guard(WHO, [&]() -> int {
+static int update_impl(int32_t op, const void* const* ptrs, const int64_t* dims, void* stream, const ImageTable* img, const SumsqRiders* riders = nullptr) {
+  {
+    const float* fl = nullptr;
     OP_TABLES(0);
     OP_REFUSE(op < 0 || op > 4, WHO ": op = %d outside 0 (sumsq), 1 (dw_reduce), 2 (l2), 3 (apply_sgd), 4 (apply_adam)", op);
     const int64_t* d = dims;
@@ -795,15 +795,82 @@
     ct.t_first = dev + 3 * nc; ct.t_count = dev + 3 * nc + nt; ct.t_l2 = dev + 3 * nc + 2 * nt;
     ct.n_chunks = nc; ct.n_tensors = (int)nt;
     switch (op) {
-      case 0: launch_sumsq(FP(0), ct, FP(1), s); break;
+      case 0: launch_sumsq(FP(0), ct, FP(1), s, riders); break;
       case 1: launch_dw_reduce(FP(0), (size_t)d[3], (int)d[4], dsrc, FP(1), ct, FP(2), s); break;
       case 2: launch_l2(FP(0), FP(1), ct, FP(2), FP(3), s); break;
-      case 3: launch_apply_sgd(FP(0), FP(1), FP(2), ct, FP(3), FP(4), s); break;
-      default: launch_apply_adam(FP(0), FP(1), FP(2), FP(3), FP(4), ct, FP(5), FP(6), s, (int)d[3]); break;
+      case 3: launch_apply_sgd(FP(0), FP(1), FP(2), ct, FP(3), FP(4), s, img); break;
+      default: launch_apply_adam(FP(0), FP(1), FP(2), FP(3), FP(4), ct, FP(5), FP(6), s, (int)d[3], img); break;
     }
     OP_LAUNCH_OK(WHO);
     HIPC(hipStreamSynchronize(s));
     return RSRGAN_OK;
+  }
+}
+int rsrgan_op_update(int32_t op, const void* const* ptrs, const int64_t* dims, const float* fl, void* stream) {
+  (void)fl;
+  return guard(WHO, [&]() -> int { return update_impl(op, ptrs, dims, stream, nullptr); });
+}
+#undef WHO
+
+#define WHO "op_sumsq_riders"
+int rsrgan_op_sumsq_riders(const void* const* ptrs, const int64_t* dims, const float* fl, void* stream) {
+  return guard(WHO, [&]() -> int {
+    OP_TABLES(0);
+    const bool tick = ptrs[2] || ptrs[3], total = ptrs[4] || ptrs[5];
+    OP_REFUSE(tick && !fl, WHO ": null table (fl: the betas)");
+    SumsqRiders r{};
+    if (tick) {
+      const int64_t* d = dims + 3;
+      const bool g = d[0] == DYN_G_LR && d[1] == DYN_ADAM_LRT, dd = d[0] == DYN_D_LR && d[1] == DYN_ADAM_LRT_D;
+      OP_REFUSE(!g && !dd, WHO ": slots (%lld, %lld) are neither (%d, %d) (G) nor (%d, %d) (D)", (long long)d[0], (long long)d[1], (int)DYN_G_LR,
+                (int)DYN_ADAM_LRT, (int)DYN_D_LR, (int)DYN_ADAM_LRT_D);
+      OP_REFUSE(!(fl[0] >= 0.f && fl[0] < 1.f) || !(fl[1] >= 0.f && fl[1] < 1.f), WHO ": beta1 = %g or beta2 = %g outside [0, 1)", (double)fl[0], (double)fl[1]);
+      OP_PTR("dyn", ptrs[2], 4); OP_PTR("t", ptrs[3], 4);
+      r.dyn = (float*)const_cast<void*>(ptrs[2]); r.t = (int*)const_cast<void*>(ptrs[3]);
+      r.b1 = (double)fl[0]; r.b2 = (double)fl[1]; r.lr_slot = (int)d[0]; r.lrt_slot = (int)d[1];
+    }
+    if (total) {
+      OP_PTR("l4", ptrs[4], 4); OP_PTR("lambda", ptrs[5], 4); OP_FLAG("zero_l2", dims[5]);
+      r.l4 = (float*)const_cast<void*>(ptrs[4]); r.lambda = (const float*)ptrs[5]; r.zero_l2 = (int)dims[5];
+    }
+    return update_impl(0, ptrs, dims, stream, nullptr, &r);
+  });
+}
+#undef WHO
+
+#define WHO "op_update_images"
+int rsrgan_op_update_images(int32_t op, const void* const* ptrs, const int64_t* dims, const int64_t* images, int32_t n_images,
+                            const void* const* dst, void* stream) {
+  return guard(WHO, [&]() -> int {
+    OP_REFUSE(op != 3 && op != 4, WHO ": op = %d is neither 3 (apply_sgd) nor 4 (apply_adam)", op);
+    OP_REFUSE(!dims, WHO ": null table (dims)");
+    OP_REFUSE(!images || !dst, WHO ": null table (images / dst)");
+    OP_REFUSE(n_images < 1 || n_images > IMG_MAX, WHO ": n_images = %d outside 1 .. %d", (int)n_images, (int)IMG_MAX);
+    const int64_t nt = dims[0];
+    if (int rc = up_tensors_ok(WHO, dims + 6, nt, dims[1])) return rc;
+    ImageTable it{};
+    std::vector<int64_t> covered((size_t)nt, 0);
+    for (int i = 0; i < n_images; ++i) {
+      const int64_t* e = images + 7 * i;
+      const int64_t t = e[0], off = e[1], R = e[2], Cc = e[3], lds = e[4], ldd = e[5], dfl = e[6];
+      OP_REFUSE(t < 0 || t >= nt, WHO ": tensor %lld of image %d outside 0 .. %lld", (long long)t, i, (long long)nt - 1);
+      OP_REFUSE(R < 1 || Cc < 1 || lds < Cc || ldd < R, WHO ": image %d: R = %lld, C = %lld, lds = %lld, ldd = %lld (needs R, C >= 1, lds >= C, ldd >= R)",
+                i, (long long)R, (long long)Cc, (long long)lds, (long long)ldd);
+      OP_REFUSE(R > (1 << 20) || lds > (1 << 20) || ldd > (1 << 20), WHO ": image %d above the entry's 2^20 rows / columns", i);
+      const int64_t t_off = dims[6 + 3 * t], t_fl = dims[6 + 3 * t + 1];
+      OP_REFUSE(off != t_off + covered[t], WHO ": image %d starts at %lld, not behind the %lld floats of tensor %lld the images before it cover", i,
+                (long long)off, (long long)covered[t], (long long)t);
+      covered[t] += R * lds;
+      OP_REFUSE(covered[t] > t_fl, WHO ": image %d ends beyond tensor %lld's %lld floats", i, (long long)t, (long long)t_fl);
+      OP_REFUSE(!dst[i] || ((uintptr_t)dst[i] & 3), WHO ": dst of image %d is null or not 4-byte aligned", i);
+      OP_REFUSE(dfl < (Cc - 1) * ldd + R, WHO ": dst of image %d: %lld floats below (C - 1) x ldd + R = %lld", i, (long long)dfl, (long long)((Cc - 1) * ldd + R));
+      it.e[it.n++] = ImageEntry{(int)t, (int)off, (int)R, (int)Cc, (int)lds, (int)ldd, 0, (float*)const_cast<void*>(dst[i])};
+    }
+    for (int64_t t = 0; t < nt; ++t)
+      OP_REFUSE(covered[t] && covered[t] != dims[6 + 3 * t + 1], WHO ": the images of tensor %lld cover %lld of its %lld floats", (long long)t,
+                (long long)covered[t], (long long)dims[6 + 3 * t + 1]);
+    image_table_plan(it);
+    return update_impl(op, ptrs, dims, stream, &it);
   });
 }
 #undef WHO
diff --git a/rsrgan_amd/csrc/kernels.h b/rsrgan_amd/csrc/kernels.h
--- a/rsrgan_amd/csrc/kernels.h
+++ b/rsrgan_amd/csrc/kernels.h
@@ -387,7 +387,7 @@
 void launch_slice_cols(const float* src, int lds, int off, float* dst, int ldd, int R, int C, hipStream_t s);
 void launch_mse(const float* y, const float* lab, int ld, float* dy, int rows, int D, const float* lambda,
                 bool accumulate, float* loss_out, float* scratch , hipStream_t s, int Bp = 0, int Bt = 0);
-void launch_g_total(float* l4 , const float* lambda, hipStream_t s);
+void launch_g_total(float* l4 , const float* lambda, hipStream_t s, bool zero_l2 = false);
 void launch_copy_f(const float* src, float* dst, int n, hipStream_t s);
 
 struct ChunkTable {
@@ -399,14 +399,19 @@
   const int* t_l2;
   int n_chunks, n_tensors;
 };
-void launch_sumsq(const float* g, const ChunkTable& ct, float* partial, hipStream_t s);
+struct SumsqRiders { float* dyn; int* t; double b1, b2; int lr_slot, lrt_slot; float* l4; const float* lambda; int zero_l2; };
+void launch_sumsq(const float* g, const ChunkTable& ct, float* partial, hipStream_t s, const SumsqRiders* riders = nullptr);
 void launch_dw_reduce(const float* ws, size_t stride, int ntiles, const long long* src, float* g, const ChunkTable& ct, float* partial, hipStream_t s);
 void launch_l2(const float* w, float* g, const ChunkTable& ct, const float* l2_scale, float* partial, hipStream_t s);
 void launch_l2_total(const float* partial, int n_chunks, const float* l2_scale, float* out, hipStream_t s);
+constexpr int IMG_MAX = 16, IMG_TILE = 64;
+struct ImageEntry { int tensor, off, R, C, lds, ldd, blk_base; float* dst; };
+struct ImageTable { int n, n_blocks; ImageEntry e[IMG_MAX]; };
+void image_table_plan(ImageTable& it);
 void launch_apply_sgd(float* w, const float* g, float* ema, const ChunkTable& ct, const float* partial,
-                      const float* dyn, hipStream_t s);
+                      const float* dyn, hipStream_t s, const ImageTable* img = nullptr);
 void launch_apply_adam(float* w, const float* g, float* m, float* v, float* ema, const ChunkTable& ct,
-                       const float* partial, const float* dyn, hipStream_t s, int lrt_slot = DYN_ADAM_LRT);
+                       const float* partial, const float* dyn, hipStream_t s, int lrt_slot = DYN_ADAM_LRT, const ImageTable* img = nullptr);
 void launch_adam_tick(float* dyn, int* t, double b1, double b2, hipStream_t s, int lr_slot = DYN_G_LR, int lrt_slot = DYN_ADAM_LRT);
 void launch_pad_copy(const float* dense, float* padded, int rows, int cols, int ld, bool to_padded, hipStream_t s);
 
diff --git a/rsrgan_amd/csrc/kernels.hip b/rsrgan_amd/csrc/kernels.hip
--- a/rsrgan_amd/csrc/kernels.hip
+++ b/rsrgan_amd/csrc/kernels.hip
@@ -1672,11 +1672,15 @@
   hipLaunchKernelGGL(k_mse2, dim3(1), dim3(64), 0, s, scratch, Bp > 0 ? rows / Bp * Bt : rows, loss_out);
 }
 
-__global__ void k_g_total(float* l4, const float* lambda) {
-  if (threadIdx.x == 0) l4[3] = l4[0] + (*lambda) * l4[1] + l4[2];
-}
-void launch_g_total(float* l4, const float* lambda, hipStream_t s) {
-  hipLaunchKernelGGL(k_g_total, dim3(1), dim3(64), 0, s, l4, lambda);
+__device__ __forceinline__ void g_total_body(float* l4, const float* lambda, int zero_l2) {
+  if (zero_l2) l4[2] = 0.f;
+  l4[3] = l4[0] + (*lambda) * l4[1] + (zero_l2 ? 0.f : l4[2]);
+}
+__global__ void k_g_total(float* l4, const float* lambda, int zero_l2) {
+  if (threadIdx.x == 0) g_total_body(l4, lambda, zero_l2);
+}
+void launch_g_total(float* l4, const float* lambda, hipStream_t s, bool zero_l2) {
+  hipLaunchKernelGGL(k_g_total, dim3(1), dim3(64), 0, s, l4, lambda, zero_l2 ? 1 : 0);
 }
 __global__ void k_copy_f(const float* src, float* dst, int n) {
   const int i = blockIdx.x * blockDim.x + threadIdx.x;
@@ -1687,9 +1691,19 @@
 }
 
 
-__global__ __launch_bounds__(256) void k_sumsq(const float* __restrict__ g, ChunkTable ct, float* __restrict__ partial) {
+__device__ __forceinline__ void adam_tick_body(float* dyn, int* t, double b1, double b2, int lr_slot, int lrt_slot) {
+  const int tt = *t + 1;
+  *t = tt;
+  dyn[lrt_slot] = (float)((double)dyn[lr_slot] * sqrt(1.0 - pow(b2, (double)tt)) / (1.0 - pow(b1, (double)tt)));
+}
+
+__global__ __launch_bounds__(256) void k_sumsq(const float* __restrict__ g, ChunkTable ct, float* __restrict__ partial, SumsqRiders r) {
   __shared__ float red[16];
   const int c = blockIdx.x;
+  if (c == 0 && threadIdx.x == 0) {
+    if (r.l4) g_total_body(r.l4, r.lambda, r.zero_l2);
+    if (r.t) adam_tick_body(r.dyn, r.t, r.b1, r.b2, r.lr_slot, r.lrt_slot);
+  }
   const float* p = g + ct.off[c];
   const int n = ct.len[c];
   float s = 0.f;
@@ -1700,8 +1714,8 @@
   s = block_sum_1024(s, red);
   if (threadIdx.x == 0) partial[c] = s;
 }
-void launch_sumsq(const float* g, const ChunkTable& ct, float* partial, hipStream_t s) {
-  hipLaunchKernelGGL(k_sumsq, dim3(ct.n_chunks), dim3(256), 0, s, g, ct, partial);
+void launch_sumsq(const float* g, const ChunkTable& ct, float* partial, hipStream_t s, const SumsqRiders* r) {
+  hipLaunchKernelGGL(k_sumsq, dim3(ct.n_chunks), dim3(256), 0, s, g, ct, partial, r ? *r : SumsqRiders{});
 }
 
 __global__ __launch_bounds__(256) void k_dw_reduce(const float* __restrict__ ws, size_t stride, int ntiles, const long long* __restrict__ src,
@@ -1768,8 +1782,7 @@
   hipLaunchKernelGGL(k_l2_total, dim3(1), dim3(1024), 0, s, partial, n, l2_scale, out);
 }
 
-__device__ __forceinline__ float tensor_clip_scale(const ChunkTable& ct, const float* partial, int c, float clip, float* red) {
-  const int t = ct.tensor[c];
+__device__ __forceinline__ float tensor_clip_scale(const ChunkTable& ct, const float* partial, int t, float clip, float* red) {
   const int first = ct.t_first[t], cnt = ct.t_count[t];
   float s = 0.f;
   for (int i = threadIdx.x; i < cnt; i += blockDim.x) s += partial[first + i];
@@ -1779,52 +1792,113 @@
   return clip * fminf(inv, 1.0f / clip);
 }
 
+struct SgdElem {
+  float* __restrict__ w; const float* __restrict__ g; float* __restrict__ ema;
+  float scale, lr, dec;
+  __device__ __forceinline__ float operator()(size_t i) const {
+#pragma clang fp contract(off)
+    const float nw = __builtin_fmaf(-lr, g[i] * scale, w[i]);
+    w[i] = nw;
+    if (ema) ema[i] = dec * ema[i] + (1.f - dec) * nw;
+    return nw;
+  }
+};
+struct AdamElem {
+  float* __restrict__ w; const float* __restrict__ g; float* __restrict__ m; float* __restrict__ v; float* __restrict__ ema;
+  float scale, b1, b2, eps, lrt, dec;
+  __device__ __forceinline__ float operator()(size_t i) const {
+#pragma clang fp contract(off)
+    const float gg = g[i] * scale;
+    const float mm = __builtin_fmaf(b1, m[i], (1.f - b1) * gg);
+    const float vv = __builtin_fmaf(b2, v[i], (1.f - b2) * gg * gg);
+    m[i] = mm; v[i] = vv;
+    const float nw = w[i] - lrt * mm / (sqrtf(vv) + eps);
+    w[i] = nw;
+    if (ema) ema[i] = dec * ema[i] + (1.f - dec) * nw;
+    return nw;
+  }
+};
+
+template <bool IMG, class Elem>
+__device__ __forceinline__ void apply_block(const ChunkTable& ct, const float* __restrict__ partial, float clip, const ImageTable& it,
+                                            Elem& el, float* red, float (*tile)[IMG_TILE + 1]) {
+  const int b = blockIdx.x;
+  if (b < ct.n_chunks) {
+    const int t = ct.tensor[b];
+    if (IMG)
+      for (int j = 0; j < it.n; ++j)
+        if (it.e[j].tensor == t) return;
+    el.scale = tensor_clip_scale(ct, partial, t, clip, red);
+    const int off = ct.off[b], n = ct.len[b];
+    for (int i = threadIdx.x; i < n; i += 256) el((size_t)(off + i));
+    return;
+  }
+  if (!IMG) return;
+  const int k = b - ct.n_chunks;
+  int j = 0;
+  while (j + 1 < it.n && k >= it.e[j + 1].blk_base) ++j;
+  const ImageEntry& E = it.e[j];
+  el.scale = tensor_clip_scale(ct, partial, E.tensor, clip, red);
+  const int lb = k - E.blk_base, nbc = (E.lds + IMG_TILE - 1) / IMG_TILE;
+  const int c0 = (lb % nbc) * IMG_TILE, r0 = (lb / nbc) * IMG_TILE;
+  const int tx = threadIdx.x & (IMG_TILE - 1), ty = threadIdx.x / IMG_TILE;
+  for (int i = ty; i < IMG_TILE; i += 256 / IMG_TILE) {
+    const int r = r0 + i, c = c0 + tx;
+    if (r < E.R && c < E.lds) tile[i][tx] = el((size_t)E.off + (size_t)r * E.lds + c);
+  }
+  __syncthreads();
+  for (int i = ty; i < IMG_TILE; i += 256 / IMG_TILE) {
+    const int c = c0 + i, r = r0 + tx;
+    if (c < E.C && r < E.R) E.dst[(size_t)c * E.ldd + r] = tile[tx][i];
+  }
+}
+
+void image_table_plan(ImageTable& it) {
+  int base = 0;
+  for (int i = 0; i < it.n; ++i) {
+    it.e[i].blk_base = base;
+    base += ((it.e[i].lds + IMG_TILE - 1) / IMG_TILE) * ((it.e[i].R + IMG_TILE - 1) / IMG_TILE);
+  }
+  it.n_blocks = base;
+}
+
+template <bool IMG>
 __global__ __launch_bounds__(256) void k_apply_sgd(float* __restrict__ w, const float* __restrict__ g, float* __restrict__ ema,
-                                                   ChunkTable ct, const float* __restrict__ partial, const float* __restrict__ dyn) {
+                                                   ChunkTable ct, const float* __restrict__ partial, const float* __restrict__ dyn,
+                                                   ImageTable it) {
   __shared__ float red[16];
-  const int c = blockIdx.x;
-  const float scale = tensor_clip_scale(ct, partial, c, dyn[DYN_CLIP], red);
-  const float lr = dyn[DYN_D_LR], dec = dyn[DYN_EMA];
-  const int off = ct.off[c], n = ct.len[c];
-  for (int i = threadIdx.x; i < n; i += 256) {
-    const float nw = w[off + i] - lr * (g[off + i] * scale);
-    w[off + i] = nw;
-    if (ema) ema[off + i] = dec * ema[off + i] + (1.f - dec) * nw;
-  }
-}
-void launch_apply_sgd(float* w, const float* g, float* ema, const ChunkTable& ct, const float* partial, const float* dyn, hipStream_t s) {
-  hipLaunchKernelGGL(k_apply_sgd, dim3(ct.n_chunks), dim3(256), 0, s, w, g, ema, ct, partial, dyn);
-}
-
+  __shared__ float tile[IMG ? IMG_TILE : 1][IMG_TILE + 1];
+  SgdElem el{w, g, ema, 1.f, dyn[DYN_D_LR], dyn[DYN_EMA]};
+  apply_block<IMG>(ct, partial, dyn[DYN_CLIP], it, el, red, tile);
+}
+void launch_apply_sgd(float* w, const float* g, float* ema, const ChunkTable& ct, const float* partial, const float* dyn, hipStream_t s,
+                      const ImageTable* img) {
+  if (img && img->n > 0)
+    hipLaunchKernelGGL(k_apply_sgd<true>, dim3(ct.n_chunks + img->n_blocks), dim3(256), 0, s, w, g, ema, ct, partial, dyn, *img);
+  else
+    hipLaunchKernelGGL(k_apply_sgd<false>, dim3(ct.n_chunks), dim3(256), 0, s, w, g, ema, ct, partial, dyn, ImageTable{});
+}
+
+template <bool IMG>
 __global__ __launch_bounds__(256) void k_apply_adam(float* __restrict__ w, const float* __restrict__ g, float* __restrict__ m,
                                                     float* __restrict__ v, float* __restrict__ ema, ChunkTable ct,
-                                                    const float* __restrict__ partial, const float* __restrict__ dyn, int lrt_slot) {
+                                                    const float* __restrict__ partial, const float* __restrict__ dyn, int lrt_slot,
+                                                    ImageTable it) {
   __shared__ float red[16];
-  const int c = blockIdx.x;
-  const float scale = tensor_clip_scale(ct, partial, c, dyn[DYN_CLIP], red);
-  const float b1 = dyn[DYN_B1], b2 = dyn[DYN_B2], eps = dyn[DYN_EPS], lrt = dyn[lrt_slot], dec = dyn[DYN_EMA];
-  const int off = ct.off[c], n = ct.len[c];
-  for (int i = threadIdx.x; i < n; i += 256) {
-    const float gg = g[off + i] * scale;
-    const float mm = b1 * m[off + i] + (1.f - b1) * gg;
-    const float vv = b2 * v[off + i] + (1.f - b2) * gg * gg;
-    m[off + i] = mm; v[off + i] = vv;
-    const float nw = w[off + i] - lrt * mm / (sqrtf(vv) + eps);
-    w[off + i] = nw;
-    if (ema) ema[off + i] = dec * ema[off + i] + (1.f - dec) * nw;
-  }
+  __shared__ float tile[IMG ? IMG_TILE : 1][IMG_TILE + 1];
+  AdamElem el{w, g, m, v, ema, 1.f, dyn[DYN_B1], dyn[DYN_B2], dyn[DYN_EPS], dyn[lrt_slot], dyn[DYN_EMA]};
+  apply_block<IMG>(ct, partial, dyn[DYN_CLIP], it, el, red, tile);
 }
 void launch_apply_adam(float* w, const float* g, float* m, float* v, float* ema, const ChunkTable& ct,
-                       const float* partial, const float* dyn, hipStream_t s, int lrt_slot) {
-  hipLaunchKernelGGL(k_apply_adam, dim3(ct.n_chunks), dim3(256), 0, s, w, g, m, v, ema, ct, partial, dyn, lrt_slot);
+                       const float* partial, const float* dyn, hipStream_t s, int lrt_slot, const ImageTable* img) {
+  if (img && img->n > 0)
+    hipLaunchKernelGGL(k_apply_adam<true>, dim3(ct.n_chunks + img->n_blocks), dim3(256), 0, s, w, g, m, v, ema, ct, partial, dyn, lrt_slot, *img);
+  else
+    hipLaunchKernelGGL(k_apply_adam<false>, dim3(ct.n_chunks), dim3(256), 0, s, w, g, m, v, ema, ct, partial, dyn, lrt_slot, ImageTable{});
 }
 
 __global__ void k_adam_tick(float* dyn, int* t, double b1, double b2, int lr_slot, int lrt_slot) {
-  if (threadIdx.x == 0) {
-    const int tt = *t + 1;
-    *t = tt;
-    dyn[lrt_slot] = (float)((double)dyn[lr_slot] * sqrt(1.0 - pow(b2, (double)tt)) / (1.0 - pow(b1, (double)tt)));
-  }
+  if (threadIdx.x == 0) adam_tick_body(dyn, t, b1, b2, lr_slot, lrt_slot);
 }
 void launch_adam_tick(float* dyn, int* t, double b1, double b2, hipStream_t s, int lr_slot, int lrt_slot) {
   hipLaunchKernelGGL(k_adam_tick, dim3(1), dim3(64), 0, s, dyn, t, b1, b2, lr_slot, lrt_slot);
diff --git a/rsrgan_amd/csrc/model.cpp b/rsrgan_amd/csrc/model.cpp
--- a/rsrgan_amd/csrc/model.cpp
+++ b/rsrgan_amd/csrc/model.cpp
@@ -17,16 +17,12 @@
 }
 const char* get_error() { return g_err; }
 
-void Model::refresh_transposes(int net, hipStream_t s) {
+void Model::transpose_jobs(int net, std::vector<TransposeJob>& jobs) const {
   const ParamSet& ps = net == RSRGAN_NET_G ? G : D;
   auto& layers = net == RSRGAN_NET_G ? gl : dl;
-  TransposeList tl{};
   auto add = [&](const float* src, int lds_, float* dst, int ldd, int R, int C) {
-    if (tl.n == 16) { launch_transpose_many(tl, s); tl.n = 0; }
-    tl.j[tl.n++] = TransposeJob{src, dst, lds_, ldd, R, C, 0};
+    jobs.push_back(TransposeJob{src, dst, lds_, ldd, R, C, 0});
   };
-  if (net == RSRGAN_NET_G && bnl_infer()) { bnl_refresh_fold(s); return; }
-  if (net == RSRGAN_NET_G && seq_bn_infer()) seq_bn_fold(s);
   for (auto& L : layers) {
     const float* K = ps.W(L.tK);
     const int H4 = 4 * L.H;
@@ -36,7 +32,50 @@
   }
   if (net == RSRGAN_NET_G && g_fc_out_wT && g_fc_out_w >= 0)
     add(G.W(g_fc_out_w), ldDout, g_fc_out_wT, pad4(gR), gR, Dout);
-  launch_transpose_many(tl, s);
+}
+
+void Model::build_image_tables() {
+  for (int net : {RSRGAN_NET_G, RSRGAN_NET_D}) {
+    const ParamSet& ps = net == RSRGAN_NET_G ? G : D;
+    ImageTable& it = img_tab[net];
+    it = ImageTable{};
+    img_on[net] = false;
+    if (!ps.w || infer()) continue;
+    std::vector<TransposeJob> jobs;
+    transpose_jobs(net, jobs);
+    if (jobs.empty() || jobs.size() > (size_t)IMG_MAX) continue;
+    bool ok = true;
+    std::vector<int64_t> covered(ps.t.size(), 0);
+    for (const TransposeJob& J : jobs) {
+      const int64_t o = J.src - ps.w;
+      int t = -1;
+      for (size_t i = 0; i < ps.t.size(); ++i)
+        if (o >= ps.t[i].off && o < ps.t[i].off + (int64_t)ps.t[i].rows * ps.t[i].ld) t = (int)i;
+      if (t < 0 || !J.dst || J.lds != ps.t[t].ld || J.C > J.lds || o != ps.t[t].off + covered[t]) { ok = false; break; }
+      covered[t] += (int64_t)J.R * J.lds;
+      it.e[it.n++] = ImageEntry{t, (int)o, J.R, J.C, J.lds, J.ldd, 0, J.dst};
+    }
+    for (size_t i = 0; ok && i < ps.t.size(); ++i)
+      if (covered[i] && covered[i] != (int64_t)ps.t[i].rows * ps.t[i].ld) ok = false;
+    if (!ok) { it = ImageTable{}; continue; }
+    image_table_plan(it);
+    img_on[net] = true;
+  }
+}
+
+void Model::refresh_transposes(int net, hipStream_t s, bool images_written) {
+  if (net == RSRGAN_NET_G && bnl_infer()) { bnl_refresh_fold(s); return; }
+  if (net == RSRGAN_NET_G && seq_bn_infer()) seq_bn_fold(s);
+  if (!images_written) {
+    std::vector<TransposeJob> jobs;
+    transpose_jobs(net, jobs);
+    TransposeList tl{};
+    for (const TransposeJob& J : jobs) {
+      if (tl.n == 16) { launch_transpose_many(tl, s); tl.n = 0; }
+      tl.j[tl.n++] = J;
+    }
+    launch_transpose_many(tl, s);
+  }
   if (!lazy_sw) refresh_swizzles(net, s);
   if (net == RSRGAN_NET_G)
     for (size_t l = 0; l < gconv.size(); ++l) {
diff --git a/rsrgan_amd/csrc/model.h b/rsrgan_amd/csrc/model.h
--- a/rsrgan_amd/csrc/model.h
+++ b/rsrgan_amd/csrc/model.h
@@ -390,7 +390,7 @@
   bool g_run_backward(const GRunPlan& p, bool g_head, hipStream_t s);
   bool g_run_bptt_fused(const GRunPlan& p, hipStream_t s);
   void g_run_bwd_rest(const GRunPlan& p, hipStream_t s);
-  void g_run_tail(const GRunPlan& p, hipStream_t s);
+  void g_run_tail(const GRunPlan& p, hipStream_t s, bool total_rides_update = false);
   int g_supervised_step(const float* x, const float* labels, const int32_t* lengths, int T, float* out_losses, bool want_grads, hipStream_t s);
   DRunPlan plan_d_run(int T, const float* nr, const float* nf, bool want_grads, hipStream_t s);
   void d_run_forward(const DRunPlan& p, hipStream_t s);
@@ -401,9 +401,13 @@
   int g_backward(const float* x, const float* labels, const int32_t* lengths, int T, const float* nf,
                  float* out_losses, bool want_grads, bool reuse, hipStream_t s);
   int apply(int net, hipStream_t s);
-  void apply_body(int net, hipStream_t s);
+  void apply_body(int net, hipStream_t s, int g_total = 0);
   int apply_inlined = 0;
-  void refresh_transposes(int net, hipStream_t s);
+  void refresh_transposes(int net, hipStream_t s, bool images_written = false);
+  void transpose_jobs(int net, std::vector<TransposeJob>& jobs) const;
+  void build_image_tables();
+  ImageTable img_tab[2] = {};
+  bool img_on[2] = {false, false};
   void refresh_swizzles(int net, hipStream_t s);
   bool lazy_sw = false;
 
diff --git a/rsrgan_amd/csrc/model_init.cpp b/rsrgan_amd/csrc/model_init.cpp
--- a/rsrgan_amd/csrc/model_init.cpp
+++ b/rsrgan_amd/csrc/model_init.cpp
@@ -670,6 +670,7 @@
   hdyn[DYN_EPS] = c.adam_eps; hdyn[DYN_EMA] = c.ema_decay;
   HIPC(hipMemcpy(dyn, hdyn, sizeof(hdyn), hipMemcpyHostToDevice));
   g_fc_in_unfolded = true;
+  build_image_tables();
   refresh_transposes(RSRGAN_NET_G, nullptr);
   if (!inf) {
     refresh_transposes(RSRGAN_NET_D, nullptr);
diff --git a/rsrgan_amd/csrc/model_step.cpp b/rsrgan_amd/csrc/model_step.cpp
--- a/rsrgan_amd/csrc/model_step.cpp
+++ b/rsrgan_amd/csrc/model_step.cpp
@@ -326,10 +326,8 @@
   if (l2) {
     launch_l2(G.w, G.g, G.ct, dyn + DYN_L2, G.partial, s);
     launch_l2_total(G.partial, G.ct.n_chunks, dyn + DYN_L2, losses + 5, s);
-  } else {
-    (void)hipMemsetAsync(losses + 5, 0, sizeof(float), s);
-  }
-  launch_g_total(losses + 3, dyn + DYN_LAMBDA, s);
+  }
+  launch_g_total(losses + 3, dyn + DYN_LAMBDA, s, !l2);
 }
 
 bool Model::g_forward_persist(int T, hipStream_t s) {
@@ -606,11 +604,16 @@
     }
     if (!p.fcs_inside) g_fc_out_wgrads(p.dy, p.R, s);
   }
-  if (p.inl) { g_run_tail(p, s); apply_body(RSRGAN_NET_G, s); }
-}
-
-void Model::g_run_tail(const GRunPlan& p, hipStream_t s) {
-  g_loss_tail(p.want_grads && p.l2_on, s);
+  if (p.inl) { g_run_tail(p, s, true); apply_body(RSRGAN_NET_G, s, p.want_grads && p.l2_on ? 1 : 2); }
+}
+
+void Model::g_run_tail(const GRunPlan& p, hipStream_t s, bool total_rides_update) {
+  const bool l2 = p.want_grads && p.l2_on;
+  if (!total_rides_update) g_loss_tail(l2, s);
+  else if (l2) {
+    launch_l2(G.w, G.g, G.ct, dyn + DYN_L2, G.partial, s);
+    launch_l2_total(G.partial, G.ct.n_chunks, dyn + DYN_L2, losses + 5, s);
+  }
   if (seq_bn() && p.want_grads && bn_training()) seq_bn_commit(2, s);
 }
 
@@ -645,7 +648,7 @@
     if (!g_run_forward(p, s)) g_run_d_forward(p, s);
     const bool g_head = g_run_loss_head(p, s);
     if (!g_run_backward(p, g_head, s)) return;
-    if (p.inl) { g_run_tail(p, s); apply_body(RSRGAN_NET_G, s); }
+    if (p.inl) { g_run_tail(p, s, true); apply_body(RSRGAN_NET_G, s, p.want_grads && p.l2_on ? 1 : 2); }
   });
   if (p.gsplit) {
     (void)hipEventRecord(ev_dfree, s);
@@ -733,22 +736,26 @@
   return RSRGAN_OK;
 }
 
-void Model::apply_body(int net, hipStream_t s) {
+void Model::apply_body(int net, hipStream_t s, int g_total) {
   if (net == RSRGAN_NET_D) {
     if (!d_partial_fresh) launch_sumsq(D.g, D.ct, D.partial, s);
     d_partial_fresh = false;
+    const ImageTable* img = img_on[RSRGAN_NET_D] ? &img_tab[RSRGAN_NET_D] : nullptr;
     if (d_adam()) {
       launch_adam_tick(dyn, adam_t_dev_d, (double)cfg.adam_beta1, (double)cfg.adam_beta2, s, DYN_D_LR, DYN_ADAM_LRT_D);
-      launch_apply_adam(D.w, D.g, D.m, D.v, D.ema, D.ct, D.partial, dyn, s, DYN_ADAM_LRT_D);
+      launch_apply_adam(D.w, D.g, D.m, D.v, D.ema, D.ct, D.partial, dyn, s, DYN_ADAM_LRT_D, img);
     } else {
-      launch_apply_sgd(D.w, D.g, D.ema, D.ct, D.partial, dyn, s);
-    }
-    refresh_transposes(RSRGAN_NET_D, s);
+      launch_apply_sgd(D.w, D.g, D.ema, D.ct, D.partial, dyn, s, img);
+    }
+    refresh_transposes(RSRGAN_NET_D, s, img != nullptr);
   } else {
-    launch_sumsq(G.g, G.ct, G.partial, s);
-    launch_adam_tick(dyn, adam_t_dev, (double)cfg.adam_beta1, (double)cfg.adam_beta2, s);
-    launch_apply_adam(G.w, G.g, G.m, G.v, G.ema, G.ct, G.partial, dyn, s);
-    refresh_transposes(RSRGAN_NET_G, s);
+    const ImageTable* img = img_on[RSRGAN_NET_G] ? &img_tab[RSRGAN_NET_G] : nullptr;
+    SumsqRiders r{};
+    r.dyn = dyn; r.t = adam_t_dev; r.b1 = (double)cfg.adam_beta1; r.b2 = (double)cfg.adam_beta2; r.lr_slot = DYN_G_LR; r.lrt_slot = DYN_ADAM_LRT;
+    if (g_total) { r.l4 = losses + 3; r.lambda = dyn + DYN_LAMBDA; r.zero_l2 = g_total == 2 ? 1 : 0; }
+    launch_sumsq(G.g, G.ct, G.partial, s, &r);
+    launch_apply_adam(G.w, G.g, G.m, G.v, G.ema, G.ct, G.partial, dyn, s, DYN_ADAM_LRT, img);
+    refresh_transposes(RSRGAN_NET_G, s, img != nullptr);
   }
 }
 
```

Measured after the change: 1.336 million, median of 5. No clear change (+0.5%).
